# hila-chefer/Transformer-MM-Explainability

Hardware: AMD Instinct MI355X
Metric: relevancy maps/sec (fwd+bwd+rollout), CLIP ViT-B/32 (higher is better)
Workload: dtype f32

## Files before the change

### include/mmx_relevancy.h

```cpp
#ifndef MMX_RELEVANCY_H
#define MMX_RELEVANCY_H

#include <stddef.h>
#include <stdint.h>

#ifdef __cplusplus
extern "C" {
#endif

#define MMX_ABI_VERSION 2
#define MMX_MAX_LAYERS 48

enum mmx_dtype { MMX_F32 = 0, MMX_F16 = 1, MMX_BF16 = 2 };
#define MMX_ATTN_MMA_BF16 0x100
#define MMX_ATTN_IO_BF16 0x200

enum mmx_status {
    MMX_OK = 0,
    MMX_EINVAL = -22,
    MMX_ENOTSUP = -95,
    MMX_EWORKSPACE = -105,
    MMX_EHIP = -1000
};

#define MMX_MM_NORMALIZE 1u
#define MMX_MM_SELF_IN_RULE10 2u
#define MMX_MM_NAN_TO_ZERO 4u

#define MMX_SCALE_Q_FIRST 0
#define MMX_SCALE_SCORES 1

int mmx_abi_version(void);
const char* mmx_last_error(void);
int mmx_set_option(const char* key, int value);

int mmx_avg_heads(const void* attn_dev, const void* grad_dev, void* out_dev,
                  int B, int H, int Nq, int Nk, int dtype, void* stream);
int mmx_avg_heads_ex(const void* attn_dev, const void* grad_dev, void* out_dev,
                     int B, int H, int Nq, int Nk, int dtype, int64_t attn_batch_stride, void* stream);

size_t mmx_self_chain_workspace_bytes(int n_layers, int B, int H, int N, int M, int dtype);
int mmx_relevancy_self_chain(const void* const* attn_layers, const void* const* grad_layers, int n_layers,
                             int B, int H, int N, int dtype,
                             const void* R_init_dev, void* R_out_dev,
                             const void* Rsq_init_dev, void* Rsq_out_dev, int M,
                             void* workspace_dev, size_t workspace_bytes, void* stream);

int mmx_relevancy_self_chain_ex(const void* const* attn_layers, const void* const* grad_layers, int n_layers,
                                int B, int H, int N, int dtype, int64_t attn_batch_stride,
                                const void* R_init_dev, void* R_out_dev,
                                const void* Rsq_init_dev, void* Rsq_out_dev, int M,
                                void* workspace_dev, size_t workspace_bytes, void* stream);

#define MMX_CHAIN_CAUSAL 1u
int mmx_relevancy_self_chain_flags(const void* const* attn_layers, const void* const* grad_layers, int n_layers,
                                   int B, int H, int N, int dtype, int64_t attn_batch_stride,
                                   const void* R_init_dev, void* R_out_dev,
                                   const void* Rsq_init_dev, void* Rsq_out_dev, int M, unsigned flags,
                                   void* workspace_dev, size_t workspace_bytes, void* stream);

int mmx_relevancy_self_chain_half(const void* const* attn_layers, const void* const* grad_layers, int n_layers,
                                  int B, int H, int N, int dtype, int64_t attn_batch_stride, void* R_out_dev,
                                  void* workspace_dev, size_t workspace_bytes, void* stream);

int mmx_bmm_f32(const void* A_dev, const void* B_dev, const void* Cin_dev, void* C_dev,
                int batch, int M, int N, int K, int trans_a,
                int64_t stride_a, int64_t stride_b, int64_t stride_c,
                int nan_to_zero, void* stream);

int mmx_linear_f32(const void* x_dev, const void* wt_dev, const void* bias_dev, void* out_dev, int M, int N, int K, void* stream);

int mmx_rows_to_dense(const void* vals_dev, const void* rows_dev, void* out_dev, int B, int N, int E, void* stream);
int mmx_rows_add(void* dense_dev, const void* rows_dev, const void* vals_dev, int B, int N, int E, void* stream);

int mmx_live_rows(const void* eot_dev, int B, int N, void* rows_dev, void* count_dev, void* stream);
int mmx_gemm_rows_f32(const void* a_dev, const void* w_dev, void* c_dev, const void* rows_dev, const void* count_dev,
                      int cap_rows, int N, int K, void* stream);
int mmx_quick_gelu_bwd_rows(const void* x_dev, const void* dy_dev, void* dx_dev, const void* rows_dev, const void* count_dev,
                            int cap_rows, int row_elems, void* stream);
int mmx_layernorm_bwd_add_rows(const void* dy_dev, const void* x_dev, const void* mean_dev, const void* rstd_dev,
                               const void* gamma_dev, const void* d_res_dev, void* dx_dev, const void* rows_dev,
                               const void* count_dev, int cap_rows, int E, void* stream);
int mmx_gemm_rows_bias_f32(const void* a_dev, const void* wt_dev, const void* bias_dev, void* c_dev, void* act_dev,
                           const void* rows_dev, const void* count_dev, int cap_rows, int N, int K, void* stream);
int mmx_add_layernorm_fwd_rows(const void* x_dev, const void* y_dev, const void* gamma_dev, const void* beta_dev,
                               void* sum_dev, void* h_dev, void* mean_dev, void* rstd_dev, const void* rows_dev,
                               const void* count_dev, int cap_rows, int E, float eps, void* stream);
int mmx_text_live_rows_fwd_enabled(void);

int mmx_chain_matvec(const void* A_dev, const void* y_dev, const void* base_dev, void* out_dev, int B, int N, void* stream);
size_t mmx_chain_vecmat_workspace_bytes(int B, int N);
int mmx_chain_vecmat(const void* A_dev, const void* x_dev, const void* base_dev, void* out_dev, int B, int N,
                     void* workspace_dev, size_t workspace_bytes, void* stream);

size_t mmx_avg_heads_vecmat_workspace_bytes(int B, int N);
int mmx_avg_heads_vecmat(const void* attn_dev, const void* grad_dev, const void* x_dev, const void* base_dev, void* out_dev,
                         int B, int H, int N, int dtype, int64_t attn_batch_stride, void* workspace_dev,
                         size_t workspace_bytes, void* stream);

int mmx_handle_residual(const void* R_dev, void* out_dev, int batch, int N, void* diag_min_dev, void* stream);

size_t mmx_mm_rules_workspace_bytes(int Ns, int Nq);
int mmx_mm_attention_rules(const void* R_ss_dev, const void* R_qq_dev, const void* R_qs_dev,
                           const void* cam_sq_dev, void* R_sq_add_dev, void* R_ss_add_dev,
                           int Ns, int Nq, unsigned flags, void* diag_min_dev,
                           void* workspace_dev, size_t workspace_bytes, void* stream);

size_t mmx_lxmert_schedule_workspace_bytes(int n_lang, int n_vis, int n_x, int B, int T, int I);
int mmx_lxmert_schedule(const void* const* lang_attn, const void* const* lang_grad, int n_lang,
                           const void* const* vis_attn, const void* const* vis_grad, int n_vis,
                           const void* const* x_lang_cross_attn, const void* const* x_lang_cross_grad,
                           const void* const* x_img_cross_attn, const void* const* x_img_cross_grad,
                           const void* const* x_lang_self_attn, const void* const* x_lang_self_grad,
                           const void* const* x_img_self_attn, const void* const* x_img_self_grad, int n_x,
                           int B, int H, int T, int I, unsigned flags, const void* text_len_dev,
                           void* R_tt_dev, void* R_ti_dev, void* R_ii_dev, void* R_it_dev,
                           void* diag_min_dev, void* workspace_dev, size_t workspace_bytes, void* stream);

size_t mmx_rollout_workspace_bytes(int B, int N);
int mmx_rollout_chain(const void* const* layers, int n_layers, int B, int N, int normalize,
                      void* out_dev, void* workspace_dev, size_t workspace_bytes, void* stream);

int mmx_heatmap_bilinear_minmax(const void* in_dev, void* out_dev, int B, int g, int S, void* stream);
int mmx_otsu_masks(const void* cam_dev, void* masks_dev, void* thresholds_dev, int K, int n, void* stream);

int mmx_attn_capture_fwd(const void* q_dev, const void* k_dev, const void* v_dev,
                         int64_t q_sb, int64_t q_sh, int64_t q_sn,
                         int64_t k_sb, int64_t k_sh, int64_t k_sn,
                         int64_t v_sb, int64_t v_sh, int64_t v_sn,
                         const void* mask_dev, int64_t mask_sb, int64_t mask_sq,
                         void* probs_dev, void* o_dev, int64_t o_sb, int64_t o_sh, int64_t o_sn,
                         int B, int H, int Nq, int Nk, int D, float scale, int scale_mode, void* stream);

size_t mmx_attn_capture_bwd_workspace_bytes(int B, int H, int Nq);
int mmx_attn_capture_bwd(const void* q_dev, const void* k_dev, const void* v_dev,
                         int64_t q_sb, int64_t q_sh, int64_t q_sn,
                         int64_t k_sb, int64_t k_sh, int64_t k_sn,
                         int64_t v_sb, int64_t v_sh, int64_t v_sn,
                         const void* probs_dev, int64_t probs_sb,
                         const void* do_dev, int64_t o_sb, int64_t o_sh, int64_t o_sn,
                         void* dprobs_dev,
                         void* dq_dev, void* dk_dev, void* dv_dev,
                         int64_t dq_sb, int64_t dq_sh, int64_t dq_sn,
                         int64_t dk_sb, int64_t dk_sh, int64_t dk_sn,
                         int64_t dv_sb, int64_t dv_sh, int64_t dv_sn,
                         int B, int H, int Nq, int Nk, int D, float scale, int scale_mode,
                         int need_dqkv, void* workspace_dev, size_t workspace_bytes, void* stream);

int mmx_attn_capture_fwd_ex(const void* q_dev, const void* k_dev, const void* v_dev,
                            int64_t q_sb, int64_t q_sh, int64_t q_sn,
                            int64_t k_sb, int64_t k_sh, int64_t k_sn,
                            int64_t v_sb, int64_t v_sh, int64_t v_sn,
                            const void* mask_dev, int64_t mask_sb, int64_t mask_sq,
                            void* probs_dev, int slab_dtype,
                            void* o_dev, int64_t o_sb, int64_t o_sh, int64_t o_sn,
                            int B, int H, int Nq, int Nk, int D, float scale, int scale_mode, void* stream);
int mmx_attn_capture_bwd_ex(const void* q_dev, const void* k_dev, const void* v_dev,
                            int64_t q_sb, int64_t q_sh, int64_t q_sn,
                            int64_t k_sb, int64_t k_sh, int64_t k_sn,
                            int64_t v_sb, int64_t v_sh, int64_t v_sn,
                            const void* probs_dev, int64_t probs_sb, int slab_dtype,
                            const void* do_dev, int64_t o_sb, int64_t o_sh, int64_t o_sn,
                            const void* fwd_o_dev, int64_t fo_sb, int64_t fo_sh, int64_t fo_sn,
                            void* dprobs_dev,
                            void* dq_dev, void* dk_dev, void* dv_dev,
                            int64_t dq_sb, int64_t dq_sh, int64_t dq_sn,
                            int64_t dk_sb, int64_t dk_sh, int64_t dk_sn,
                            int64_t dv_sb, int64_t dv_sh, int64_t dv_sn,
                            int B, int H, int Nq, int Nk, int D, float scale, int scale_mode,
                            int need_dqkv, void* workspace_dev, size_t workspace_bytes, void* stream);

int mmx_attn_fwd(const void* q_dev, const void* k_dev, const void* v_dev,
                 int64_t q_sb, int64_t q_sh, int64_t q_sn,
                 int64_t k_sb, int64_t k_sh, int64_t k_sn,
                 int64_t v_sb, int64_t v_sh, int64_t v_sn,
                 const void* mask_dev, int64_t mask_sb, int64_t mask_sq,
                 void* o_dev, int64_t o_sb, int64_t o_sh, int64_t o_sn,
                 int B, int H, int Nq, int Nk, int D, float scale, int scale_mode, void* stream);

int mmx_patch_ranks(const void* scores_dev, void* ranks_dev, int B, int P, void* stream);
int mmx_perturb_patches(const void* images_dev, const void* ranks_dev, const void* counts_dev, const void* fill_dev,
                        void* out_dev, int B, int C, int R, int patch, int S, void* stream);

size_t mmx_attn_capture_bwd_rowrel_workspace_bytes(int B, int H, int Nq, int Nk);
int mmx_attn_capture_bwd_rowrel(const void* q_dev, const void* k_dev, const void* v_dev,
                                int64_t q_sb, int64_t q_sh, int64_t q_sn,
                                int64_t k_sb, int64_t k_sh, int64_t k_sn,
                                int64_t v_sb, int64_t v_sh, int64_t v_sn,
                                const void* probs_dev, int64_t probs_sb, int slab_dtype,
                                const void* do_dev, int64_t o_sb, int64_t o_sh, int64_t o_sn,
                                const void* fwd_o_dev, int64_t fo_sb, int64_t fo_sh, int64_t fo_sn,
                                void* dprobs_dev,
                                void* dq_dev, void* dk_dev, void* dv_dev,
                                int64_t dq_sb, int64_t dq_sh, int64_t dq_sn,
                                int64_t dk_sb, int64_t dk_sh, int64_t dk_sn,
                                int64_t dv_sb, int64_t dv_sh, int64_t dv_sn,
                                int B, int H, int Nq, int Nk, int D, float scale, int scale_mode,
                                int need_dqkv, const void* rel_in_dev, void* rel_out_dev,
                                void* workspace_dev, size_t workspace_bytes, void* stream);

size_t mmx_attn_capture_bwd_rowrel_f32_workspace_bytes(int B, int H, int Nq, int Nk);
int mmx_attn_capture_bwd_rowrel_f32(const void* q_dev, const void* k_dev, const void* v_dev,
                                    int64_t q_sb, int64_t q_sh, int64_t q_sn,
                                    int64_t k_sb, int64_t k_sh, int64_t k_sn,
                                    int64_t v_sb, int64_t v_sh, int64_t v_sn,
                                    const void* probs_dev, int64_t probs_sb, int slab_dtype,
                                    const void* do_dev, int64_t o_sb, int64_t o_sh, int64_t o_sn,
                                    const void* fwd_o_dev, int64_t fo_sb, int64_t fo_sh, int64_t fo_sn,
                                    void* dprobs_dev,
                                    void* dq_dev, void* dk_dev, void* dv_dev,
                                    int64_t dq_sb, int64_t dq_sh, int64_t dq_sn,
                                    int64_t dk_sb, int64_t dk_sh, int64_t dk_sn,
                                    int64_t dv_sb, int64_t dv_sh, int64_t dv_sn,
                                    int B, int H, int Nq, int Nk, int D, float scale, int scale_mode,
                                    int need_dqkv, const void* rel_in_dev, void* rel_out_dev,
                                    void* workspace_dev, size_t workspace_bytes, void* stream);

size_t mmx_attn_capture_bwd_rowrel_f32_grouped_workspace_bytes(int B, int H, int Nq, int Nk);
int mmx_attn_capture_bwd_rowrel_f32_grouped(const void* q_dev, const void* k_dev, const void* v_dev,
                                            int64_t q_sb, int64_t q_sh, int64_t q_sn,
                                            int64_t k_sb, int64_t k_sh, int64_t k_sn,
                                            int64_t v_sb, int64_t v_sh, int64_t v_sn,
                                            const void* probs_dev, int64_t probs_sb, int slab_dtype,
                                            const void* do_dev, int64_t o_sb, int64_t o_sh, int64_t o_sn,
                                            const void* fwd_o_dev, int64_t fo_sb, int64_t fo_sh, int64_t fo_sn,
                                            void* dprobs_dev,
                                            void* dq_dev, void* dk_dev, void* dv_dev,
                                            int64_t dq_sb, int64_t dq_sh, int64_t dq_sn,
                                            int64_t dk_sb, int64_t dk_sh, int64_t dk_sn,
                                            int64_t dv_sb, int64_t dv_sh, int64_t dv_sn,
                                            int B, int H, int Nq, int Nk, int D, float scale, int scale_mode,
                                            int need_dqkv, const void* rel_in_dev, void* rel_out_dev, int n_images,
                                            void* workspace_dev, size_t workspace_bytes, void* stream);

size_t mmx_detr_decoder_rows_workspace_bytes(int n_layers, int K, int Q, int Ni);
int mmx_detr_decoder_rows(const void* const* self_attn, const void* const* self_grad, const void* const* cross_attn,
                          const void* const* cross_grad, int n_layers, int K, int H, int Q, int Ni,
                          int64_t self_attn_bstride, int64_t cross_attn_bstride, const void* targets_dev,
                          void* s_out_dev, void* diag_min_dev, void* workspace_dev, size_t workspace_bytes, void* stream);

int mmx_attn_relprop(const void* q_dev, const void* k_dev, const void* v_dev, const void* o_dev, const void* cam_o_dev,
                     int64_t q_sb, int64_t q_sh, int64_t q_sn, int64_t k_sb, int64_t k_sh, int64_t k_sn,
                     int64_t v_sb, int64_t v_sh, int64_t v_sn, int64_t o_sb, int64_t o_sh, int64_t o_sn,
                     int64_t co_sb, int64_t co_sh, int64_t co_sn,
                     const void* probs_dev, void* cam_probs_dev, void* cam_q_dev, void* cam_k_dev, void* cam_v_dev,
                     int64_t cq_sb, int64_t cq_sh, int64_t cq_sn, int64_t ck_sb, int64_t ck_sh, int64_t ck_sn,
                     int64_t cv_sb, int64_t cv_sh, int64_t cv_sn,
                     int B, int H, int Nq, int Nk, int D, float scale, int scale_mode, void* stream);

#define MMX_LRP_VALUES 1
#define MMX_LRP_SCORES 2
int mmx_attn_relprop_phase(const void* q_dev, const void* k_dev, const void* v_dev, const void* o_dev, const void* cam_o_dev,
                           int64_t q_sb, int64_t q_sh, int64_t q_sn, int64_t k_sb, int64_t k_sh, int64_t k_sn,
                           int64_t v_sb, int64_t v_sh, int64_t v_sn, int64_t o_sb, int64_t o_sh, int64_t o_sn,
                           int64_t co_sb, int64_t co_sh, int64_t co_sn,
                           const void* probs_dev, void* cam_probs_dev, void* cam_q_dev, void* cam_k_dev, void* cam_v_dev,
                           int64_t cq_sb, int64_t cq_sh, int64_t cq_sn, int64_t ck_sb, int64_t ck_sh, int64_t ck_sn,
                           int64_t cv_sb, int64_t cv_sh, int64_t cv_sn,
                           int B, int H, int Nq, int Nk, int D, float scale, int scale_mode,
                           const void* cam_scores_dev, int phase, void* stream);

size_t mmx_lrp_workspace_bytes(void);
int mmx_lrp_split_signs(const void* x_dev, void* out_dev, int64_t rows, int n, void* stream);
int mmx_lrp_safe_divide(const void* a_dev, const void* b_dev, void* out_dev, int64_t n, void* stream);
int mmx_lrp_linear_combine(const void* xx_dev, const void* y_dev, void* out_dev, int64_t rows, int n,
                           const void* r_dev, int64_t r_numel, void* workspace_dev, void* stream);
int mmx_lrp_add_relprop(const void* r_dev, const void* a_dev, const void* b_dev, void* ra_dev, void* rb_dev,
                        int batch, int64_t per, void* workspace_dev, void* stream);
int mmx_lrp_clone_relprop(const void* const* r_list, int n_r, const void* x_dev, void* out_dev, int64_t n, void* stream);
int mmx_lrp_mha_rescale(const void* v_pre_dev, int64_t n_vpre, const void* v_post_dev, int64_t n_vpost, void* cam_k_dev,
                        int64_t n_k, void* cam_q_dev, int64_t n_q, const void* cam_o_dev, int64_t n_o,
                        void* workspace_dev, void* stream);


int mmx_quick_gelu_fwd(const void* x_dev, void* y_dev, int64_t n, void* stream);
int mmx_quick_gelu_fwd_bf16(const void* x_dev, void* y_dev, int64_t n, void* stream);
int mmx_quick_gelu_bwd(const void* x_dev, const void* dy_dev, void* dx_dev, int64_t n, void* stream);
int mmx_quick_gelu_bwd_bcast_bf16(const void* x_dev, const void* dy_dev, void* dx_dev, int64_t n, int64_t x_n, void* stream);
int mmx_layernorm_bwd_add_bf16(const void* dy_dev, const void* x_dev, const void* mean_dev, const void* rstd_dev,
                               const void* gamma_dev, const void* d_res_dev, void* dx_dev, void* dx_bf16_dev,
                               int64_t rows, int x_rows, int E, void* stream);
int mmx_quick_gelu_bwd_bcast(const void* x_dev, const void* dy_dev, void* dx_dev, int64_t n, int64_t x_n, void* stream);

int mmx_layernorm_bwd_add(const void* dy_dev, const void* x_dev, const void* mean_dev, const void* rstd_dev,
                          const void* gamma_dev, const void* d_res_dev, void* dx_dev, int64_t rows, int x_rows, int E,
                          void* stream);

int mmx_add_layernorm_fwd(const void* x_dev, const void* y_dev, const void* gamma_dev, const void* beta_dev,
                          void* sum_dev, void* h_dev, void* mean_dev, void* rstd_dev, int64_t rows, int E, float eps,
                          void* stream);
int mmx_add_layernorm_fwd_ex(const void* x_dev, const void* y_dev, const void* gamma_dev, const void* beta_dev,
                             void* sum_dev, void* h_dev, void* mean_dev, void* rstd_dev, int64_t rows, int E,
                             float eps, int h_dtype, void* stream);

int mmx_event_create(void** event_out);
int mmx_event_destroy(void* event);
int mmx_event_record(void* event, void* stream);
int mmx_event_elapsed_ms(void* start, void* stop, float* ms_out);

#ifdef __cplusplus
}
#endif
#endif
```

### transformer-mm-explainability_amd/_lib.py

```python
from __future__ import annotations

import ctypes as C
import os
import re

_HERE = os.path.dirname(os.path.abspath(__file__))
LIB_PATH = os.environ.get("MMX_LIB_PATH") or os.path.join(_HERE, "csrc", "libmmx_hip.so")
HEADER_PATH = os.path.join(os.path.dirname(_HERE), "include", "mmx_relevancy.h")

ABI_VERSION = 2
MMX_F32, MMX_F16, MMX_BF16 = 0, 1, 2
MMX_ENOTSUP = -95
MMX_ATTN_IO_BF16 = 0x200
MMX_ATTN_MMA_BF16 = 0x100
MM_NORMALIZE, MM_SELF_IN_RULE10, MM_NAN_TO_ZERO = 1, 2, 4
CHAIN_CAUSAL = 1
SCALE_Q_FIRST, SCALE_SCORES = 0, 1
LRP_VALUES, LRP_SCORES = 1, 2
MAX_LAYERS = 48

_vp, _i, _i64, _sz, _f, _u = C.c_void_p, C.c_int, C.c_int64, C.c_size_t, C.c_float, C.c_uint
_vpp = C.POINTER(C.c_void_p)

_PROTOTYPES = {
    "mmx_abi_version": (_i, []),
    "mmx_last_error": (C.c_char_p, []),
    "mmx_set_option": (_i, [C.c_char_p, _i]),
    "mmx_avg_heads": (_i, [_vp, _vp, _vp, _i, _i, _i, _i, _i, _vp]),
    "mmx_avg_heads_ex": (_i, [_vp, _vp, _vp, _i, _i, _i, _i, _i, _i64, _vp]),
    "mmx_self_chain_workspace_bytes": (_sz, [_i, _i, _i, _i, _i, _i]),
    "mmx_relevancy_self_chain": (_i, [_vpp, _vpp, _i, _i, _i, _i, _i, _vp, _vp, _vp, _vp, _i, _vp, _sz, _vp]),
    "mmx_relevancy_self_chain_ex": (_i, [_vpp, _vpp, _i, _i, _i, _i, _i, _i64, _vp, _vp, _vp, _vp, _i, _vp, _sz, _vp]),
    "mmx_relevancy_self_chain_flags": (_i, [_vpp, _vpp, _i, _i, _i, _i, _i, _i64, _vp, _vp, _vp, _vp, _i, _u, _vp, _sz, _vp]),
    "mmx_relevancy_self_chain_half": (_i, [_vpp, _vpp, _i, _i, _i, _i, _i, _i64, _vp, _vp, _sz, _vp]),
    "mmx_bmm_f32": (_i, [_vp, _vp, _vp, _vp, _i, _i, _i, _i, _i, _i64, _i64, _i64, _i, _vp]),
    "mmx_handle_residual": (_i, [_vp, _vp, _i, _i, _vp, _vp]),
    "mmx_mm_rules_workspace_bytes": (_sz, [_i, _i]),
    "mmx_mm_attention_rules": (_i, [_vp, _vp, _vp, _vp, _vp, _vp, _i, _i, _u, _vp, _vp, _sz, _vp]),
    "mmx_lxmert_schedule_workspace_bytes": (_sz, [_i, _i, _i, _i, _i, _i]),
    "mmx_lxmert_schedule": (_i, [_vpp, _vpp, _i, _vpp, _vpp, _i] + [_vpp] * 8 + [_i, _i, _i, _i, _i, _u, _vp,
                                    _vp, _vp, _vp, _vp, _vp, _vp, _sz, _vp]),
    "mmx_lrp_workspace_bytes": (_sz, []),
    "mmx_lrp_split_signs": (_i, [_vp, _vp, _i64, _i, _vp]),
    "mmx_lrp_safe_divide": (_i, [_vp, _vp, _vp, _i64, _vp]),
    "mmx_lrp_linear_combine": (_i, [_vp, _vp, _vp, _i64, _i, _vp, _i64, _vp, _vp]),
    "mmx_lrp_add_relprop": (_i, [_vp, _vp, _vp, _vp, _vp, _i, _i64, _vp, _vp]),
    "mmx_lrp_clone_relprop": (_i, [_vpp, _i, _vp, _vp, _i64, _vp]),
    "mmx_lrp_mha_rescale": (_i, [_vp, _i64, _vp, _i64, _vp, _i64, _vp, _i64, _vp, _i64, _vp, _vp]),
    "mmx_heatmap_bilinear_minmax": (_i, [_vp, _vp, _i, _i, _i, _vp]),
    "mmx_otsu_masks": (_i, [_vp, _vp, _vp, _i, _i, _vp]),
    "mmx_rollout_workspace_bytes": (_sz, [_i, _i]),
    "mmx_rollout_chain": (_i, [_vpp, _i, _i, _i, _i, _vp, _vp, _sz, _vp]),
    "mmx_attn_capture_fwd": (_i, [_vp, _vp, _vp] + [_i64] * 9 + [_vp, _i64, _i64, _vp, _vp, _i64, _i64, _i64,
                                  _i, _i, _i, _i, _i, _f, _i, _vp]),
    "mmx_attn_capture_fwd_ex": (_i, [_vp, _vp, _vp] + [_i64] * 9 + [_vp, _i64, _i64, _vp, _i, _vp, _i64, _i64, _i64,
                                     _i, _i, _i, _i, _i, _f, _i, _vp]),
    "mmx_attn_fwd": (_i, [_vp, _vp, _vp] + [_i64] * 9 + [_vp, _i64, _i64, _vp, _i64, _i64, _i64, _i, _i, _i, _i, _i, _f, _i, _vp]),
    "mmx_patch_ranks": (_i, [_vp, _vp, _i, _i, _vp]),
    "mmx_perturb_patches": (_i, [_vp, _vp, _vp, _vp, _vp, _i, _i, _i, _i, _i, _vp]),
    "mmx_attn_capture_bwd_ex": (_i, [_vp, _vp, _vp] + [_i64] * 9 + [_vp, _i64, _i, _vp, _i64, _i64, _i64, _vp, _i64, _i64, _i64,
                                     _vp, _vp, _vp, _vp]
                                + [_i64] * 9 + [_i, _i, _i, _i, _i, _f, _i, _i, _vp, _sz, _vp]),
    "mmx_attn_capture_bwd_rowrel": (_i, [_vp, _vp, _vp] + [_i64] * 9 + [_vp, _i64, _i, _vp, _i64, _i64, _i64, _vp, _i64, _i64,
                                         _i64, _vp, _vp, _vp, _vp]
                                    + [_i64] * 9 + [_i, _i, _i, _i, _i, _f, _i, _i, _vp, _vp, _vp, _sz, _vp]),
    "mmx_attn_capture_bwd_rowrel_workspace_bytes": (_sz, [_i, _i, _i, _i]),
    "mmx_attn_capture_bwd_rowrel_f32": (_i, [_vp, _vp, _vp] + [_i64] * 9 + [_vp, _i64, _i, _vp, _i64, _i64, _i64, _vp, _i64,
                                             _i64, _i64, _vp, _vp, _vp, _vp]
                                        + [_i64] * 9 + [_i, _i, _i, _i, _i, _f, _i, _i, _vp, _vp, _vp, _sz, _vp]),
    "mmx_attn_capture_bwd_rowrel_f32_workspace_bytes": (_sz, [_i, _i, _i, _i]),
    "mmx_attn_capture_bwd_rowrel_f32_grouped": (_i, [_vp, _vp, _vp] + [_i64] * 9 + [_vp, _i64, _i, _vp, _i64, _i64, _i64, _vp,
                                                     _i64, _i64, _i64, _vp, _vp, _vp, _vp]
                                                + [_i64] * 9 + [_i, _i, _i, _i, _i, _f, _i, _i, _vp, _vp, _i, _vp, _sz, _vp]),
    "mmx_attn_capture_bwd_rowrel_f32_grouped_workspace_bytes": (_sz, [_i, _i, _i, _i]),
    "mmx_attn_capture_bwd_workspace_bytes": (_sz, [_i, _i, _i]),
    "mmx_attn_capture_bwd": (_i, [_vp, _vp, _vp] + [_i64] * 9 + [_vp, _i64, _vp, _i64, _i64, _i64, _vp, _vp, _vp, _vp]
                             + [_i64] * 9 + [_i, _i, _i, _i, _i, _f, _i, _i, _vp, _sz, _vp]),
    "mmx_attn_relprop": (_i, [_vp] * 5 + [_i64] * 15 + [_vp] * 5 + [_i64] * 9 + [_i, _i, _i, _i, _i, _f, _i, _vp]),
    "mmx_attn_relprop_phase": (_i, [_vp] * 5 + [_i64] * 15 + [_vp] * 5 + [_i64] * 9 + [_i, _i, _i, _i, _i, _f, _i, _vp, _i, _vp]),
    "mmx_detr_decoder_rows_workspace_bytes": (_sz, [_i, _i, _i, _i]),
    "mmx_detr_decoder_rows": (_i, [_vpp] * 4 + [_i] * 5 + [_i64, _i64, _vp, _vp, _vp, _vp, _sz, _vp]),
    "mmx_linear_f32": (_i, [_vp, _vp, _vp, _vp, _i, _i, _i, _vp]),
    "mmx_rows_to_dense": (_i, [_vp, _vp, _vp, _i, _i, _i, _vp]),
    "mmx_rows_add": (_i, [_vp, _vp, _vp, _i, _i, _i, _vp]),
    "mmx_live_rows": (_i, [_vp, _i, _i, _vp, _vp, _vp]),
    "mmx_gemm_rows_f32": (_i, [_vp, _vp, _vp, _vp, _vp, _i, _i, _i, _vp]),
    "mmx_quick_gelu_bwd_rows": (_i, [_vp, _vp, _vp, _vp, _vp, _i, _i, _vp]),
    "mmx_layernorm_bwd_add_rows": (_i, [_vp, _vp, _vp, _vp, _vp, _vp, _vp, _vp, _vp, _i, _i, _vp]),
    "mmx_gemm_rows_bias_f32": (_i, [_vp, _vp, _vp, _vp, _vp, _vp, _vp, _i, _i, _i, _vp]),
    "mmx_add_layernorm_fwd_rows": (_i, [_vp, _vp, _vp, _vp, _vp, _vp, _vp, _vp, _vp, _vp, _i, _i, _f, _vp]),
    "mmx_text_live_rows_fwd_enabled": (_i, []),
    "mmx_chain_matvec": (_i, [_vp, _vp, _vp, _vp, _i, _i, _vp]),
    "mmx_chain_vecmat_workspace_bytes": (_sz, [_i, _i]),
    "mmx_chain_vecmat": (_i, [_vp, _vp, _vp, _vp, _i, _i, _vp, _sz, _vp]),
    "mmx_avg_heads_vecmat_workspace_bytes": (_sz, [_i, _i]),
    "mmx_avg_heads_vecmat": (_i, [_vp, _vp, _vp, _vp, _vp, _i, _i, _i, _i, _i64, _vp, _sz, _vp]),
    "mmx_quick_gelu_fwd": (_i, [_vp, _vp, _i64, _vp]),
    "mmx_quick_gelu_fwd_bf16": (_i, [_vp, _vp, _i64, _vp]),
    "mmx_quick_gelu_bwd": (_i, [_vp, _vp, _vp, _i64, _vp]),
    "mmx_quick_gelu_bwd_bcast": (_i, [_vp, _vp, _vp, _i64, _i64, _vp]),
    "mmx_quick_gelu_bwd_bcast_bf16": (_i, [_vp, _vp, _vp, _i64, _i64, _vp]),
    "mmx_layernorm_bwd_add_bf16": (_i, [_vp, _vp, _vp, _vp, _vp, _vp, _vp, _vp, _i64, _i, _i, _vp]),
    "mmx_layernorm_bwd_add": (_i, [_vp, _vp, _vp, _vp, _vp, _vp, _vp, _i64, _i, _i, _vp]),
    "mmx_add_layernorm_fwd": (_i, [_vp, _vp, _vp, _vp, _vp, _vp, _vp, _vp, _i64, _i, _f, _vp]),
    "mmx_add_layernorm_fwd_ex": (_i, [_vp, _vp, _vp, _vp, _vp, _vp, _vp, _vp, _i64, _i, _f, _i, _vp]),
    "mmx_event_create": (_i, [_vpp]),
    "mmx_event_destroy": (_i, [_vp]),
    "mmx_event_record": (_i, [_vp, _vp]),
    "mmx_event_elapsed_ms": (_i, [_vp, _vp, C.POINTER(C.c_float)]),
}


class MMXError(RuntimeError):
    pass


_lib = None


def header_symbols():
    with open(HEADER_PATH) as f:
        text = re.sub(r"/\*.*?\*/", "", f.read(), flags=re.S)
    return sorted(set(re.findall(r"\b(mmx_[a-z0-9_]+)\s*\(", text)))


def lib():
    global _lib
    if _lib is None:
        if not os.path.exists(LIB_PATH):
            raise MMXError(
                "libmmx_hip.so is not built (%s). Run `python -c 'import __graft_entry__ as g; g.build()'` "
                "or `make -C transformer-mm-explainability_amd/csrc`. There is no CPU fallback." % LIB_PATH)
        handle = C.CDLL(LIB_PATH)
        for name, (res, args) in _PROTOTYPES.items():
            fn = getattr(handle, name)
            fn.restype, fn.argtypes = res, args
        if handle.mmx_abi_version() != ABI_VERSION:
            raise MMXError("libmmx_hip.so ABI version %d != %d (stale build? `make -C transformer-mm-explainability_amd/csrc`)"
                           % (handle.mmx_abi_version(), ABI_VERSION))
        _lib = handle
    return _lib


def check(rc, what):
    if rc != 0:
        msg = lib().mmx_last_error().decode("utf-8", "replace")
        raise MMXError("%s failed (rc=%d): %s" % (what, rc, msg))


def ptr_table(ptrs):
    arr = (C.c_void_p * len(ptrs))(*ptrs)
    return C.cast(arr, _vpp), arr
```

### transformer-mm-explainability_amd/clip_model.py

```python
from __future__ import annotations

from collections import OrderedDict

import numpy as np
import torch
import torch.nn as nn
import torch.nn.functional as F

from . import _lib, ops
from .capture import CaptureBuffers, attention_capture_packed


class QuickGELU(nn.Module):
    def forward(self, x):
        if x.is_cuda and x.dtype == torch.float32:
            return ops.quick_gelu(x)
        return x * torch.sigmoid(1.702 * x)


class _OutProj(nn.Linear):
    """``attn.out_proj`` (name kept for state-dict compatibility)."""


class CapturedSelfAttention(nn.Module):

    def __init__(self, embed_dim, num_heads):
        super().__init__()
        if embed_dim % num_heads:
            raise ValueError("embed_dim must be divisible by num_heads")
        self.embed_dim, self.num_heads, self.head_dim = embed_dim, num_heads, embed_dim // num_heads
        self.in_proj_weight = nn.Parameter(torch.empty(3 * embed_dim, embed_dim))
        self.in_proj_bias = nn.Parameter(torch.zeros(3 * embed_dim))
        self.out_proj = _OutProj(embed_dim, embed_dim)
        nn.init.xavier_uniform_(self.in_proj_weight)
        nn.init.zeros_(self.out_proj.bias)

    def forward(self, x, probs_slab, grads_slab, mask=None, need_dqkv=True, grad_hook=None):
        B, N, E = x.shape
        qkv = F.linear(x, self.in_proj_weight, self.in_proj_bias).view(B, N, 3, self.num_heads, self.head_dim)
        o = attention_capture_packed(qkv, probs_slab, grads_slab, self.head_dim ** -0.5, mask=mask,
                                     scale_mode=_lib.SCALE_Q_FIRST, need_dqkv=need_dqkv, grad_hook=grad_hook)
        return self.out_proj(o.view(B, N, E))


class ResidualAttentionBlock(nn.Module):

    def __init__(self, d_model, n_head, attn_mask=None):
        super().__init__()
        self.attn = CapturedSelfAttention(d_model, n_head)
        self.ln_1 = nn.LayerNorm(d_model)
        self.mlp = nn.Sequential(OrderedDict([
            ("c_fc", nn.Linear(d_model, d_model * 4)),
            ("gelu", QuickGELU()),
            ("c_proj", nn.Linear(d_model * 4, d_model)),
        ]))
        self.ln_2 = nn.LayerNorm(d_model)
        self.attn_mask = attn_mask
        self.attn_probs = None
        self.attn_grad = None

    def _slab_view(self, name):
        owner = self.__dict__.get("_probs_owner")
        if owner is not None:
            owner[0].complete_attn_probs()
        return self.__dict__.get(name)

    @property
    def attn_probs(self):
        return self._slab_view("_attn_probs")

    @attn_probs.setter
    def attn_probs(self, value):
        self.__dict__["_attn_probs"] = value

    @property
    def attn_grad(self):
        return self._slab_view("_attn_grad")

    @attn_grad.setter
    def attn_grad(self, value):
        self.__dict__["_attn_grad"] = value

    def set_attn_probs(self, attn_probs):
        self.attn_probs = attn_probs

    def set_attn_grad(self, attn_grad):
        self.attn_grad = attn_grad

    def forward(self, x, buffers, layer, need_dqkv=True):
        if self.attn_mask is not None and (self.attn_mask.device != x.device):
            self.attn_mask = self.attn_mask.to(device=x.device, dtype=torch.float32)
        probs, grads = buffers.probs[layer], buffers.grads[layer]
        self.attn_probs = buffers.layer_probs(layer)
        self.attn_grad = buffers.layer_grads(layer)
        mask = self.attn_mask
        if mask is not None and mask.shape[-1] != x.shape[1]:
            mask = mask[: x.shape[1], : x.shape[1]].contiguous()
        x = x + self.attn(self.ln_1(x), probs, grads, mask=mask, need_dqkv=need_dqkv)
        x = x + self.mlp(self.ln_2(x))
        return x


class Transformer(nn.Module):
    def __init__(self, width, layers, heads, attn_mask=None):
        super().__init__()
        self.width, self.layers, self.heads = width, layers, heads
        self.resblocks = nn.Sequential(*[ResidualAttentionBlock(width, heads, attn_mask) for _ in range(layers)])
        self.buffers = None
        self.capture_dtype = torch.float32
        self.backward_gemm_dtype = torch.float32
        self.forward_gemm_dtype = torch.float32
        self.attention_mma_bf16 = False
        self._long_sequence_slabs_follow_body = attn_mask is None
        self._probs_pending = None

    def set_body_dtype(self, dtype):
        if dtype not in (torch.float32, torch.bfloat16, torch.float16):
            raise ValueError("body dtype must be torch.float32, torch.bfloat16 or torch.float16")
        half = dtype == torch.bfloat16
        self.backward_gemm_dtype = self.forward_gemm_dtype = dtype
        self.attention_mma_bf16 = half
        self.half_chain = dtype == torch.float16
        if self._long_sequence_slabs_follow_body:
            self.capture_dtype = dtype
            self.buffers = None

    def _linear(self, x, lin_weight, lin_bias):
        return ops.linear(x, lin_weight, lin_bias, getattr(self, "forward_gemm_dtype", torch.float32))

    def _gemm(self, x, weight):
        return ops.backward_gemm(x, weight, getattr(self, "backward_gemm_dtype", torch.float32))

    def _ensure_buffers(self, batch, n_tokens, device, shared_probs=False, grads=True):
        if self.buffers is None or not self.buffers.matches(self.layers, batch, self.heads, n_tokens, n_tokens, device,
                                                            shared_probs, self.capture_dtype, grads):
            self.buffers = CaptureBuffers(self.layers, batch, self.heads, n_tokens, n_tokens, device=device,
                                          shared_probs=shared_probs, dtype=self.capture_dtype, grads=grads)
        return self.buffers

    def _mask_for(self, blk, n_tokens, device):
        mask = blk.attn_mask
        if mask is None:
            return None
        if mask.device != device:
            blk.attn_mask = mask = mask.to(device=device, dtype=torch.float32)
        if mask.shape[-1] != n_tokens:
            mask = mask[:n_tokens, :n_tokens].contiguous()
        return mask

    def is_causal(self):
        masks = [getattr(blk, "attn_mask", None) for blk in self.resblocks]
        if not masks or any(m is None for m in masks):
            return False
        key = tuple(id(m) for m in masks)
        cached = self.__dict__.get("_causal_mask_check")
        if cached is None or cached[0] != key:
            ok = True
            for m in {id(m): m for m in masks}.values():
                n = m.shape[-1]
                upper = torch.ones(n, n, dtype=torch.bool, device=m.device).triu_(1)
                ok = ok and m.dim() == 2 and m.shape[0] == n and bool(torch.isneginf(m[upper]).all())
            self.__dict__["_causal_mask_check"] = cached = (key, ok)
        return cached[1]

    def _row_gemm_weights_ok(self):
        for blk in self.resblocks:
            if not ops.gemm_rows_eligible(blk.mlp.c_proj.weight, blk.mlp.c_fc.weight, blk.attn.out_proj.weight, blk.attn.in_proj_weight):
                return False
        return True

    def live_rows_for_forward(self, x, out_rows):
        if out_rows is None or x.dim() != 3 or x.dtype != torch.float32 or x.shape[-1] % 4 or not x.is_cuda:
            return None
        for what in ("forward_gemm_dtype", "backward_gemm_dtype", "capture_dtype"):
            if getattr(self, what, torch.float32) != torch.float32:
                return None
        if self.layers < 1 or not ops.live_rows_forward_enabled() or not self.is_causal() or not self._row_gemm_weights_ok():
            return None
        if x.shape[1] < self.resblocks[0].attn_mask.shape[-1]:
            return None
        for blk in self.resblocks:
            for bias in (blk.attn.in_proj_bias, blk.attn.out_proj.bias, blk.mlp.c_fc.bias, blk.mlp.c_proj.bias):
                if bias is None or bias.dtype != torch.float32:
                    return None
        return ops.live_rows(out_rows, x.shape[1])

    @torch.no_grad()
    def complete_attn_probs(self):
        pending = self.__dict__.get("_probs_pending")
        if pending is None:
            return
        if torch.cuda.is_current_stream_capturing():
            raise _lib.MMXError("attn_probs / attn_grad: the slabs of a row-list forward cannot be completed inside a stream capture "
                                "(read them outside it, or set option text_live_rows_fwd to 0)")
        self._probs_pending = None
        keep, self.buffers = self.buffers, pending["buffers"]
        try:
            _, tape = self.forward_tape(pending["x"], first_grad_layer=pending["first_grad_layer"],
                                        grads=pending["buffers"].grads is not None, out_rows=pending["out_rows"])
            if pending["dy_row_values"] is not None:
                self.backward_tape(tape, None, pending["backward_first_grad_layer"], dy_rows=pending["out_rows"],
                                   dy_row_values=pending["dy_row_values"])
        finally:
            self.buffers = keep

    def _live_rows_route(self, tape, B, N, E, first_grad_layer, dy_rows, dy_row_values, rel_row, grouped):
        top = self.layers - 1
        if dy_rows is None or dy_row_values is None or rel_row is not None or grouped or top <= first_grad_layer:
            return None
        if getattr(self, "backward_gemm_dtype", torch.float32) != torch.float32 or dy_row_values.dtype != torch.float32:
            return None
        if tape[top][0].shape[0] != B or E % 4 or not self.is_causal() or not self._row_gemm_weights_ok():
            return None
        return ops.live_rows(dy_rows, N)

    @torch.no_grad()
    def forward_tape(self, x, batch=None, first_grad_layer=0, grads=True, out_rows=None, live=None):
        if not x.is_cuda:
            raise _lib.MMXError("the CLIP body runs its attention on the HIP capture op: move the model and "
                                "inputs to the MI355X (there is no CPU attention path)")
        Bx, N, E = x.shape
        batch = Bx if batch is None else batch
        shared = Bx == 1 and batch > 1
        if not shared and Bx != batch:
            raise ValueError("forward_tape: %d inputs for %d upstream gradients (only a single input can be shared)" % (Bx, batch))
        buffers = self._ensure_buffers(batch, N, x.device, shared_probs=shared, grads=grads)
        blocks = list(self.resblocks)
        mask = self._mask_for(blocks[0], N, x.device) if blocks else None
        tape = []
        self._probs_pending = None
        if live is not None:
            if out_rows is None or shared or live.cap != Bx * N:
                raise ValueError("forward_tape: the row-list forward needs out_rows, one input per gradient and a list over %d rows"
                                 % (Bx * N))
            self._probs_pending = {"x": x, "buffers": buffers, "live": live, "out_rows": out_rows, "first_grad_layer": first_grad_layer,
                                   "dy_row_values": None, "backward_first_grad_layer": None}
            for blk in blocks:
                blk.__dict__["_probs_owner"] = (self,)

        def ln(res, y, norm):
            if live is not None:
                return ops.add_layernorm_rows(res, y, norm.weight, norm.bias, norm.eps, live)
            return ops.add_layernorm(res, y, norm.weight, norm.bias, norm.eps, h_dtype=hd)
        mma = bool(getattr(self, "attention_mma_bf16", False)) and N > 128
        first = blocks[0].ln_1
        hd = torch.bfloat16 if getattr(self, "forward_gemm_dtype", torch.float32) == torch.bfloat16 else torch.float32
        _, h1, mean1, rstd1 = ln(x, None, first)
        for l, blk in enumerate(blocks):
            at = blk.attn
            if live is not None:
                qkv = ops.linear_rows(h1, at.in_proj_weight, at.in_proj_bias, live,
                                      out=torch.zeros(Bx, N, 3 * E, dtype=torch.float32, device=x.device))
            else:
                qkv = self._linear(h1, at.in_proj_weight, at.in_proj_bias)
            qkv = qkv.view(Bx, N, 3, at.num_heads, at.head_dim)
            o = ops.attn_capture_fwd(qkv[:, :, 0], qkv[:, :, 1], qkv[:, :, 2], buffers.probs[l], at.head_dim ** -0.5,
                                     _lib.SCALE_Q_FIRST, mask, layout="bnhd", mma_bf16=mma)
            if out_rows is not None and l + 1 == len(blocks):
                ar = torch.arange(Bx, device=x.device)
                x1, h2, mean2, rstd2 = ops.add_layernorm(
                    x[ar, out_rows], self._linear(o.view(Bx, N, E)[ar, out_rows], at.out_proj.weight, at.out_proj.bias),
                    blk.ln_2.weight, blk.ln_2.bias, blk.ln_2.eps, h_dtype=hd)
                m = self._linear(h2, blk.mlp.c_fc.weight, blk.mlp.c_fc.bias)
                mlp_out = self._linear(ops.quick_gelu_fwd(m, hd), blk.mlp.c_proj.weight, blk.mlp.c_proj.bias)
                tape.append((x, mean1, rstd1, qkv, x1, mean2, rstd2, m, o, out_rows) if l >= first_grad_layer else None)
                blk.attn_probs, blk.attn_grad = buffers.layer_probs(l), buffers.layer_grads(l)
                return x1 + mlp_out, tape
            if live is not None:
                x1, h2, mean2, rstd2 = ln(x, ops.linear_rows(o.view(Bx, N, E), at.out_proj.weight, at.out_proj.bias, live), blk.ln_2)
                m, act = ops.linear_rows(h2, blk.mlp.c_fc.weight, blk.mlp.c_fc.bias, live, gelu=True)
                mlp_out = ops.linear_rows(act, blk.mlp.c_proj.weight, blk.mlp.c_proj.bias, live)
            else:
                x1, h2, mean2, rstd2 = ln(x, self._linear(o.view(Bx, N, E), at.out_proj.weight, at.out_proj.bias), blk.ln_2)
                m = self._linear(h2, blk.mlp.c_fc.weight, blk.mlp.c_fc.bias)
                mlp_out = self._linear(ops.quick_gelu_fwd(m, hd), blk.mlp.c_proj.weight, blk.mlp.c_proj.bias)
            tape.append((x, mean1, rstd1, qkv, x1, mean2, rstd2, m, o) if l >= first_grad_layer else None)
            blk.attn_probs, blk.attn_grad = buffers.layer_probs(l), buffers.layer_grads(l)
            if l + 1 < len(blocks):
                x, h1, mean1, rstd1 = ln(x1, mlp_out, blocks[l + 1].ln_1)
            else:
                x = x1 + mlp_out
        return x, tape

    @torch.no_grad()
    def forward_nocapture(self, x, out_rows=None):
        for what in ("forward_gemm_dtype", "capture_dtype"):
            dt = getattr(self, what, torch.float32)
            if dt != torch.float32:
                raise _lib.MMXError("forward_nocapture: fp32 bodies only (the no-capture attention is exact fp32); this tower's "
                                    "%s is %s" % (what, str(dt).replace("torch.", "")))
        if x.dtype != torch.float32:
            raise _lib.MMXError("forward_nocapture: fp32 bodies only; the input is %s" % str(x.dtype).replace("torch.", ""))
        if not x.is_cuda:
            raise _lib.MMXError("the CLIP body runs its attention on the HIP kernels: move the model and inputs to the GPU")
        B, N, E = x.shape
        blocks = list(self.resblocks)
        mask = self._mask_for(blocks[0], N, x.device) if blocks else None
        first = blocks[0].ln_1
        _, h1, _, _ = ops.add_layernorm(x, None, first.weight, first.bias, first.eps)
        for l, blk in enumerate(blocks):
            at = blk.attn
            top = out_rows is not None and l + 1 == len(blocks)
            one = top and isinstance(out_rows, int)
            qkv = self._linear(h1, at.in_proj_weight, at.in_proj_bias).view(B, N, 3, at.num_heads, at.head_dim)
            q = qkv[:, out_rows:out_rows + 1, 0] if one else qkv[:, :, 0]
            m_l = mask[out_rows:out_rows + 1] if (one and mask is not None) else mask
            o = ops.attn_fwd(q, qkv[:, :, 1], qkv[:, :, 2], at.head_dim ** -0.5, _lib.SCALE_Q_FIRST, m_l, layout="bnhd")
            if one:
                xr, orows = x[:, out_rows], o.view(B, E)
            elif top:
                ar = torch.arange(B, device=x.device)
                xr, orows = x[ar, out_rows], o.view(B, N, E)[ar, out_rows]
            else:
                xr, orows = x, o.view(B, N, E)
            x1, h2, _, _ = ops.add_layernorm(xr, self._linear(orows, at.out_proj.weight, at.out_proj.bias), blk.ln_2.weight,
                                             blk.ln_2.bias, blk.ln_2.eps)
            mlp_out = self._linear(ops.quick_gelu_fwd(self._linear(h2, blk.mlp.c_fc.weight, blk.mlp.c_fc.bias)),
                                   blk.mlp.c_proj.weight, blk.mlp.c_proj.bias)
            if l + 1 < len(blocks):
                nxt = blocks[l + 1].ln_1
                x, h1, _, _ = ops.add_layernorm(x1, mlp_out, nxt.weight, nxt.bias, nxt.eps)
            else:
                x = x1 + mlp_out
        return x

    def forward_shared(self, x, batch):
        if x.shape[0] != 1:
            raise ValueError("forward_shared takes the single shared sample")
        return self.forward_tape(x, batch)

    @torch.no_grad()
    def backward_tape(self, tape, dy, first_grad_layer=0, dy_rows=None, rel_row=None, dy_row_values=None, targets_per_image=1,
                      live=None):
        if dy is None:
            if dy_rows is None or dy_row_values is None:
                raise ValueError("backward_tape: dy=None needs dy_rows and dy_row_values")
            if self.layers - 1 < first_grad_layer:
                return rel_row
            B, N, E = dy_row_values.shape[0], tape[-1][0].shape[1], dy_row_values.shape[1]
        else:
            B, N, E = dy.shape
        buffers = self.buffers
        top = self.layers - 1
        dx = dy
        top_rows = None
        mma = bool(getattr(self, "attention_mma_bf16", False)) and N > 128
        grouped = int(targets_per_image) > 1
        stream16 = getattr(self, "backward_gemm_dtype", torch.float32) == torch.bfloat16
        head = self.resblocks[0].attn
        att16 = stream16 and (mma or (self.capture_dtype == torch.float32 and
                                      ops.head_kernel_shape(N, N, head.head_dim) and head.head_dim % 8 == 0))
        if grouped and (rel_row is None or stream16 or mma or B % int(targets_per_image)):
            raise ValueError("backward_tape: targets_per_image=%d needs an fp32 body in the row mode and a multiple of it "
                             "upstream gradients (got %d)" % (int(targets_per_image), B))
        dx_h = None
        if live is None:
            live = self._live_rows_route(tape, B, N, E, first_grad_layer, dy_rows, dy_row_values, rel_row, grouped)
        elif dy_rows is None or dy_row_values is None or rel_row is not None or grouped or live.cap != B * N:
            raise ValueError("backward_tape: the tape of a row-list forward needs the row-list backward (dy_rows and dy_row_values, "
                             "no rel_row, one target per sample)")
        else:
            pending = self.__dict__.get("_probs_pending")
            if pending is not None and pending["live"] is live:
                pending["dy_row_values"], pending["backward_first_grad_layer"] = dy_row_values, first_grad_layer
        d_o_dense = None
        for l in range(top, first_grad_layer - 1, -1):
            blk = self.resblocks[l]
            at = blk.attn
            x, mean1, rstd1, qkv, x1, mean2, rstd2, m, o_fwd = tape[l][:9]
            shared = x.shape[0] != B and not grouped
            if grouped and x.shape[0] * int(targets_per_image) != B:
                raise ValueError("backward_tape: %d upstream gradients for %d samples x %d targets"
                                 % (B, x.shape[0], int(targets_per_image)))
            if len(tape[l]) > 9 and (l != top or dy_rows is None):
                raise ValueError("backward_tape: the forward kept only the output rows of the top block (out_rows): "
                                 "pass the same rows as dy_rows")
            if l == top and dy_rows is not None:
                g = dy_row_values if dy_row_values is not None else dy[torch.arange(B, device=dy_rows.device), dy_rows]
                d_x1_r, d_o = self._top_block_rows(blk, tape[l], g, dy_rows, shared, N, x.shape[0] if grouped else None)
                d_x1, top_rows = None, (dy_rows, d_x1_r)
                d_o_dense = d_o
                if att16:
                    d_o = d_o.to(torch.bfloat16)
            elif live is not None:
                d_a = ops.gemm_rows(dx, blk.mlp.c_proj.weight, live)
                d_m = ops.quick_gelu_bwd_rows(m, d_a, live)
                d_h2 = ops.gemm_rows(d_m, blk.mlp.c_fc.weight, live)
                d_x1 = ops.layernorm_bwd_add_rows(d_h2, x1, mean2, rstd2, blk.ln_2.weight, dx, live)
                d_o = ops.gemm_rows(d_x1, at.out_proj.weight, live, out=d_o_dense)
            elif stream16:
                if dx_h is None:
                    dx_h = dx.to(torch.bfloat16)
                d_a = ops.backward_gemm_bf16(dx_h, blk.mlp.c_proj.weight)
                d_m = ops.quick_gelu_bwd(m, d_a)
                d_h2 = ops.backward_gemm_bf16(d_m, blk.mlp.c_fc.weight)
                d_x1, d_x1_h = ops.layernorm_bwd_add_bf16(d_h2, x1, mean2, rstd2, blk.ln_2.weight, dx)
                d_o = ops.backward_gemm_bf16(d_x1_h, at.out_proj.weight)
            else:
                d_a = self._gemm(dx, blk.mlp.c_proj.weight)
                d_m = ops.quick_gelu_bwd(m, d_a)
                d_h2 = self._gemm(d_m, blk.mlp.c_fc.weight)
                d_x1 = ops.layernorm_bwd_add(d_h2, x1, mean2, rstd2, blk.ln_2.weight, dx)
                d_o = self._gemm(d_x1, at.out_proj.weight)
            if stream16 and not att16 and d_o.dtype != torch.float32:
                d_o = d_o.float()
            d_o = d_o.view(B, N, at.num_heads, at.head_dim)
            need = l > first_grad_layer
            dqkv = torch.empty(B, N, 3, at.num_heads, at.head_dim, dtype=d_o.dtype, device=d_o.device) if need else None
            out = (dqkv[:, :, 0], dqkv[:, :, 1], dqkv[:, :, 2]) if need else None
            res = ops.attn_capture_bwd(qkv[:, :, 0], qkv[:, :, 1], qkv[:, :, 2], buffers.probs[l], d_o,
                                       buffers.grads[l] if buffers.grads is not None else None,
                                       at.head_dim ** -0.5, _lib.SCALE_Q_FIRST, need_dqkv=need, layout="bnhd", out=out,
                                       batch=B if shared else None, o=o_fwd, mma_bf16=mma, rel_row=rel_row,
                                       images=x.shape[0] if grouped else None)
            if rel_row is not None:
                rel_row = res[3]
            if not need:
                break
            if stream16:
                dq_in = dqkv.view(B, N, 3 * E)
                d_h1 = ops.backward_gemm_bf16(dq_in if att16 else dq_in.to(torch.bfloat16), at.in_proj_weight)
                dx, dx_h = ops.layernorm_bwd_add_bf16(d_h1, x, mean1, rstd1, blk.ln_1.weight, d_x1)
            elif live is not None:
                d_h1 = ops.gemm_rows(dqkv.view(B, N, 3 * E), at.in_proj_weight, live)
                dx = ops.layernorm_bwd_add_rows(d_h1, x, mean1, rstd1, blk.ln_1.weight, d_x1, live)
            else:
                d_h1 = self._gemm(dqkv.view(B, N, 3 * E), at.in_proj_weight)
                dx = ops.layernorm_bwd_add(d_h1, x, mean1, rstd1, blk.ln_1.weight, d_x1)
            if l == top and top_rows is not None:
                ops.rows_add_(dx, *top_rows)
                if stream16:
                    dx_h = dx.to(torch.bfloat16)
        return rel_row

    def _top_block_rows(self, blk, entry, g, rows, shared, N, images=None):
        x, mean1, rstd1, qkv, x1, mean2, rstd2, m, o_fwd = entry[:9]
        B = g.shape[0]
        ar = torch.arange(B, device=g.device)
        src = torch.zeros_like(rows) if shared else ar
        if images is not None:
            src = ar % images
        if len(entry) > 9:
            m_r, x1_r, mean2_r, rstd2_r = m[src], x1[src], mean2.reshape(-1)[src], rstd2.reshape(-1)[src]
        else:
            flat = src * N + rows
            m_r, x1_r, mean2_r, rstd2_r = m[src, rows], x1[src, rows], mean2.reshape(-1)[flat], rstd2.reshape(-1)[flat]
        d_a = self._gemm(g, blk.mlp.c_proj.weight)
        d_m = ops.quick_gelu_bwd(m_r, d_a) if d_a.dtype == torch.float32 and m_r.numel() % 4 == 0 else \
            d_a * (torch.sigmoid(1.702 * m_r) * (1 + 1.702 * m_r * (1 - torch.sigmoid(1.702 * m_r))))
        d_h2 = self._gemm(d_m, blk.mlp.c_fc.weight)
        d_x1_r = ops.layernorm_bwd_add(d_h2, x1_r, mean2_r, rstd2_r, blk.ln_2.weight, g)
        return d_x1_r, ops.rows_to_dense(self._gemm(d_x1_r, blk.attn.out_proj.weight), rows, N)

    def backward_shared(self, tape, dy, first_grad_layer=0):
        return self.backward_tape(tape, dy, first_grad_layer)

    def forward(self, x, capture_only=False, first_grad_layer=0):
        if not x.is_cuda:
            raise _lib.MMXError("the CLIP body runs its attention on the HIP capture op: move the model and "
                                "inputs to the MI355X (there is no CPU attention path)")
        buffers = self._ensure_buffers(x.shape[0], x.shape[1], x.device)
        self._probs_pending = None
        if not capture_only:
            for l, blk in enumerate(self.resblocks):
                x = blk(x, buffers, l)
            return x
        with torch.no_grad():
            for l in range(first_grad_layer):
                x = self.resblocks[l](x, buffers, l)
        x = x.detach().requires_grad_(True)
        for l in range(first_grad_layer, self.layers):
            x = self.resblocks[l](x, buffers, l, need_dqkv=(l != first_grad_layer))
        return x


class VisualTransformer(nn.Module):

    def __init__(self, input_resolution, patch_size, width, layers, heads, output_dim):
        super().__init__()
        self.input_resolution, self.output_dim = input_resolution, output_dim
        self.conv1 = nn.Conv2d(3, width, kernel_size=patch_size, stride=patch_size, bias=False)
        scale = width ** -0.5
        self.class_embedding = nn.Parameter(scale * torch.randn(width))
        self.positional_embedding = nn.Parameter(scale * torch.randn((input_resolution // patch_size) ** 2 + 1, width))
        self.ln_pre = nn.LayerNorm(width)
        self.transformer = Transformer(width, layers, heads)
        self.ln_post = nn.LayerNorm(width)
        self.proj = nn.Parameter(scale * torch.randn(width, output_dim))

    def _patchify(self, x):
        B, C, Hh, Ww = x.shape
        p = self.conv1.kernel_size[0]
        gh, gw = Hh // p, Ww // p
        patches = x.reshape(B, C, gh, p, gw, p).permute(0, 2, 4, 1, 3, 5).reshape(B, gh * gw, C * p * p)
        return F.linear(patches, self.conv1.weight.reshape(self.conv1.out_channels, -1))

    def _embed(self, x):
        x = self._patchify(x)
        cls = self.class_embedding.to(x.dtype).expand(x.shape[0], 1, -1)
        return self.ln_pre(torch.cat([cls, x], dim=1) + self.positional_embedding.to(x.dtype))

    def forward(self, x, capture_only=False, first_grad_layer=0):
        x = self.transformer(self._embed(x), capture_only=capture_only, first_grad_layer=first_grad_layer)
        x = self.ln_post(x[:, 0, :])
        return x @ self.proj if self.proj is not None else x

    def row_relevancy_ok(self):
        t = self.transformer
        n_tokens = self.positional_embedding.shape[0]
        return bool(getattr(t, "attention_mma_bf16", False)) and n_tokens > 128

    @torch.no_grad()
    def forward_tape(self, image, batch=None, first_grad_layer=0, grads=True):
        x = self._embed(image)
        y, tape = self.transformer.forward_tape(x, batch, first_grad_layer, grads=grads,
                                                out_rows=torch.zeros(x.shape[0], dtype=torch.long, device=x.device))
        cls = y
        _, f, mean, rstd = ops.add_layernorm(cls, None, self.ln_post.weight, self.ln_post.bias, self.ln_post.eps)
        return f @ self.proj, (tape, x.shape, cls, mean, rstd)

    def forward_shared(self, image, batch):
        return self.forward_tape(image, batch)

    @torch.no_grad()
    def encode_nocapture(self, images=None, tokens=None):
        if (images is None) == (tokens is None):
            raise ValueError("encode_nocapture takes images or tokens (exactly one of them)")
        if self.conv1.weight.dtype != torch.float32:
            raise _lib.MMXError("encode_nocapture: fp32 bodies only; the parameters are %s"
                                % str(self.conv1.weight.dtype).replace("torch.", ""))
        x = self._embed(images) if tokens is None else tokens
        cls = self.transformer.forward_nocapture(x, out_rows=0)
        _, f, _, _ = ops.add_layernorm(cls, None, self.ln_post.weight, self.ln_post.bias, self.ln_post.eps)
        return f @ self.proj

    @torch.no_grad()
    def backward_tape(self, state, d_features, first_grad_layer=0, cls_row=False, targets_per_image=1):
        tape, y_shape, cls, mean, rstd = state
        B = d_features.shape[0]
        if int(targets_per_image) > 1 and not cls_row:
            raise ValueError("backward_tape: targets_per_image needs cls_row=True (the grouped mode is a row mode)")
        d_f = torch.matmul(d_features, self.proj.t())
        d_cls = ops.layernorm_bwd_add(d_f, cls, mean, rstd, self.ln_post.weight)
        rel_row = None
        if cls_row:
            rel_row = torch.zeros(B, y_shape[1], dtype=torch.float32, device=d_f.device)
            rel_row[:, 0] = 1.0
        return self.transformer.backward_tape(tape, None, first_grad_layer,
                                              dy_rows=torch.zeros(B, dtype=torch.long, device=d_f.device), rel_row=rel_row,
                                              dy_row_values=d_cls, targets_per_image=targets_per_image)

    def backward_shared(self, state, d_features, first_grad_layer=0):
        return self.backward_tape(state, d_features, first_grad_layer)


class CLIP(nn.Module):

    def __init__(self, embed_dim, image_resolution, vision_layers, vision_width, vision_patch_size,
                 context_length, vocab_size, transformer_width, transformer_heads, transformer_layers):
        super().__init__()
        if isinstance(vision_layers, (tuple, list)):
            raise NotImplementedError("ModifiedResNet towers have no attention stack; use a ViT config")
        self.context_length = context_length
        self.visual = VisualTransformer(image_resolution, vision_patch_size, vision_width, vision_layers,
                                        vision_width // 64, embed_dim)
        self.transformer = Transformer(transformer_width, transformer_layers, transformer_heads,
                                       attn_mask=self.build_attention_mask())
        self.vocab_size = vocab_size
        self.token_embedding = nn.Embedding(vocab_size, transformer_width)
        self.positional_embedding = nn.Parameter(torch.empty(context_length, transformer_width))
        self.ln_final = nn.LayerNorm(transformer_width)
        self.text_projection = nn.Parameter(torch.empty(transformer_width, embed_dim))
        self.logit_scale = nn.Parameter(torch.ones([]) * np.log(1 / 0.07))
        self.capture_only = False
        self.first_grad_layers = (0, 0)
        self.initialize_parameters()

    def initialize_parameters(self):
        nn.init.normal_(self.token_embedding.weight, std=0.02)
        nn.init.normal_(self.positional_embedding, std=0.01)
        w, n = self.transformer.width, self.transformer.layers
        proj_std, attn_std, fc_std = (w ** -0.5) * ((2 * n) ** -0.5), w ** -0.5, (2 * w) ** -0.5
        for blk in self.transformer.resblocks:
            nn.init.normal_(blk.attn.in_proj_weight, std=attn_std)
            nn.init.normal_(blk.attn.out_proj.weight, std=proj_std)
            nn.init.normal_(blk.mlp.c_fc.weight, std=fc_std)
            nn.init.normal_(blk.mlp.c_proj.weight, std=proj_std)
        nn.init.normal_(self.text_projection, std=w ** -0.5)

    def set_body_dtype(self, dtype):
        self.visual.transformer.set_body_dtype(dtype)
        self.transformer.set_body_dtype(dtype)

    def build_attention_mask(self):
        return torch.full((self.context_length, self.context_length), float("-inf")).triu_(1)

    @property
    def dtype(self):
        return self.visual.conv1.weight.dtype

    def encode_image(self, image):
        return self.visual(image.type(self.dtype), capture_only=self.capture_only,
                           first_grad_layer=self.first_grad_layers[0])

    def encode_text(self, text, n_tokens=None):
        if n_tokens is not None and n_tokens < text.shape[1]:
            text = text[:, :n_tokens]
        n = text.shape[1]
        x = self.token_embedding(text).type(self.dtype) + self.positional_embedding[:n].type(self.dtype)
        x = self.transformer(x, capture_only=self.capture_only, first_grad_layer=self.first_grad_layers[1])
        x = self.ln_final(x)
        return x[torch.arange(x.shape[0], device=x.device), text.argmax(dim=-1)] @ self.text_projection

    @torch.no_grad()
    def encode_text_tape(self, text, n_tokens=None, first_grad_layer=0):
        if n_tokens is not None and n_tokens < text.shape[1]:
            text = text[:, :n_tokens]
        n = text.shape[1]
        x = self.token_embedding(text).type(self.dtype) + self.positional_embedding[:n].type(self.dtype)
        eot = text.argmax(dim=-1)
        live = self.transformer.live_rows_for_forward(x, eot)
        rows, tape = self.transformer.forward_tape(x, first_grad_layer=first_grad_layer, out_rows=eot, live=live)
        _, f, mean, rstd = ops.add_layernorm(rows, None, self.ln_final.weight, self.ln_final.bias, self.ln_final.eps)
        return f @ self.text_projection, (tape, x.shape, rows, mean, rstd, eot, live)

    @torch.no_grad()
    def encode_text_nocapture(self, text):
        x = self.token_embedding(text).type(self.dtype) + self.positional_embedding[:text.shape[1]].type(self.dtype)
        rows = self.transformer.forward_nocapture(x, out_rows=text.argmax(dim=-1))
        _, f, _, _ = ops.add_layernorm(rows, None, self.ln_final.weight, self.ln_final.bias, self.ln_final.eps)
        return f @ self.text_projection

    @torch.no_grad()
    def backward_text_tape(self, state, d_features, first_grad_layer=0):
        tape, y_shape, rows, mean, rstd, eot, live = state
        d_f = torch.matmul(d_features, self.text_projection.t())
        d_rows = ops.layernorm_bwd_add(d_f, rows, mean, rstd, self.ln_final.weight)
        self.transformer.backward_tape(tape, None, first_grad_layer, dy_rows=eot, dy_row_values=d_rows,
                                       live=live)

    def forward(self, image, text):
        return self.logits(self.encode_image(image), self.encode_text(text))

    def logits(self, image_features, text_features):
        image_features = image_features / image_features.norm(dim=-1, keepdim=True)
        text_features = text_features / text_features.norm(dim=-1, keepdim=True)
        logit_scale = self.logit_scale.exp()
        logits_per_image = logit_scale * image_features @ text_features.t()
        logits_per_text = logit_scale * text_features @ image_features.t()
        return logits_per_image, logits_per_text


def build_model(state_dict):
    if "visual.proj" not in state_dict:
        raise NotImplementedError("only ViT CLIP checkpoints carry an attention stack to explain")
    vision_width = state_dict["visual.conv1.weight"].shape[0]
    vision_layers = len([k for k in state_dict if k.startswith("visual.") and k.endswith(".attn.in_proj_weight")])
    vision_patch_size = state_dict["visual.conv1.weight"].shape[-1]
    grid_size = round((state_dict["visual.positional_embedding"].shape[0] - 1) ** 0.5)
    embed_dim = state_dict["text_projection"].shape[1]
    context_length = state_dict["positional_embedding"].shape[0]
    vocab_size = state_dict["token_embedding.weight"].shape[0]
    transformer_width = state_dict["ln_final.weight"].shape[0]
    transformer_layers = len({k.split(".")[2] for k in state_dict if k.startswith("transformer.resblocks")})
    model = CLIP(embed_dim, vision_patch_size * grid_size, vision_layers, vision_width, vision_patch_size,
                 context_length, vocab_size, transformer_width, transformer_width // 64, transformer_layers)
    sd = {k: v.float() for k, v in state_dict.items() if k not in ("input_resolution", "context_length", "vocab_size")}
    model.load_state_dict(sd)
    return model.eval()


CONFIGS = {
    "ViT-B/32": (512, 224, 12, 768, 32, 77, 49408, 512, 8, 12),
    "ViT-B/16": (512, 224, 12, 768, 16, 77, 49408, 512, 8, 12),
    "ViT-L/14@336": (768, 336, 24, 1024, 14, 77, 49408, 768, 12, 12),
}


def random_init(name="ViT-B/32", seed=0):
    torch.manual_seed(seed)
    return CLIP(*CONFIGS[name]).float().eval()
```

### transformer-mm-explainability_amd/csrc/elementwise_kernels.hip

```cpp
#include "mmx_common.h"

namespace mmx {

typedef unsigned u32x2 __attribute__((ext_vector_type(2)));
__device__ __forceinline__ unsigned bf_pack(float a, float b) {
    typedef __bf16 bf2 __attribute__((ext_vector_type(2)));
    bf2 r;
    r[0] = static_cast<__bf16>(a);
    r[1] = static_cast<__bf16>(b);
    return __builtin_bit_cast(unsigned, r);
}

__global__ __launch_bounds__(256) void quick_gelu_fwd_kernel(const f32x4* __restrict__ x, f32x4* __restrict__ y, int64_t n4,
                                                             const float* xt, float* yt, int tail) {
    for (int64_t i = static_cast<int64_t>(blockIdx.x) * 256 + threadIdx.x; i < n4; i += static_cast<int64_t>(gridDim.x) * 256) {
        const f32x4 v = x[i];
        f32x4 o;
#pragma unroll
        for (int e = 0; e < 4; ++e) o[e] = quick_gelu_f(v[e]);
        y[i] = o;
    }
    if (blockIdx.x == 0 && threadIdx.x < tail) yt[threadIdx.x] = quick_gelu_f(xt[threadIdx.x]);
}

__global__ __launch_bounds__(256) void quick_gelu_fwd_bf16_kernel(const f32x4* __restrict__ x, u32x2* __restrict__ y, int64_t n4) {
    for (int64_t i = static_cast<int64_t>(blockIdx.x) * 256 + threadIdx.x; i < n4; i += static_cast<int64_t>(gridDim.x) * 256) {
        const f32x4 v = x[i];
        f32x4 o;
#pragma unroll
        for (int e = 0; e < 4; ++e) o[e] = quick_gelu_f(v[e]);
        y[i] = u32x2{bf_pack(o[0], o[1]), bf_pack(o[2], o[3])};
    }
}

template <bool ROWS>
__global__ __launch_bounds__(256) void quick_gelu_bwd_kernel(const f32x4* __restrict__ x, const f32x4* __restrict__ dy,
                                                             f32x4* __restrict__ dx, int64_t n4, int64_t x_n4, const float* xt,
                                                             const float* dyt, float* dxt, int tail, const int* __restrict__ rows,
                                                             const int* __restrict__ count, int row4) {
    const int64_t cap = ROWS ? n4 / row4 : 0;
    const int64_t total = ROWS ? (*count < cap ? *count : cap) * row4 : n4;
    for (int64_t j = static_cast<int64_t>(blockIdx.x) * 256 + threadIdx.x; j < total; j += static_cast<int64_t>(gridDim.x) * 256) {
        int64_t i = j;
        if constexpr (ROWS) {
            const int64_t r = rows[j / row4];
            if (r < 0 || r >= cap) continue;
            i = r * row4 + j % row4;
        }
        const f32x4 v = x[x_n4 == n4 ? i : i % x_n4];
        const f32x4 g = dy[i];
        f32x4 o;
#pragma unroll
        for (int e = 0; e < 4; ++e) {
            const float s = sigmoid_f(1.702f * v[e]);
            o[e] = g[e] * (s + 1.702f * v[e] * s * (1.f - s));
        }
        dx[i] = o;
    }
    if (!ROWS && blockIdx.x == 0 && threadIdx.x < tail) {
        const float v = xt[threadIdx.x], s = sigmoid_f(1.702f * v);
        dxt[threadIdx.x] = dyt[threadIdx.x] * (s + 1.702f * v * s * (1.f - s));
    }
}

}

using namespace mmx;

static int gelu_grid(int64_t n4) {
    const int64_t blocks = (n4 + 255) / 256;
    return static_cast<int>(blocks < 1 ? 1 : (blocks > 4096 ? 4096 : blocks));
}

extern "C" int mmx_quick_gelu_fwd(const void* x_dev, void* y_dev, int64_t n, void* stream) {
    MMX_CHECK_ARG(x_dev && y_dev && n > 0, "mmx_quick_gelu_fwd: bad argument");
    MMX_CHECK_ARG(((reinterpret_cast<uintptr_t>(x_dev) | reinterpret_cast<uintptr_t>(y_dev)) & 15u) == 0,
                  "mmx_quick_gelu_fwd: pointers must be 16-byte aligned");
    const int64_t n4 = n / 4;
    const float* x = static_cast<const float*>(x_dev);
    float* y = static_cast<float*>(y_dev);
    quick_gelu_fwd_kernel<<<gelu_grid(n4), 256, 0, static_cast<hipStream_t>(stream)>>>(
        reinterpret_cast<const f32x4*>(x), reinterpret_cast<f32x4*>(y), n4, x + n4 * 4, y + n4 * 4, static_cast<int>(n - n4 * 4));
    MMX_LAUNCH_CHECK("quick_gelu_fwd_kernel");
    return MMX_OK;
}

extern "C" int mmx_quick_gelu_bwd_bcast(const void* x_dev, const void* dy_dev, void* dx_dev, int64_t n, int64_t x_n,
                                        void* stream) {
    MMX_CHECK_ARG(x_dev && dy_dev && dx_dev && n > 0 && x_n > 0, "mmx_quick_gelu_bwd_bcast: bad argument");
    MMX_CHECK_ARG(n % x_n == 0 && x_n % 4 == 0, "mmx_quick_gelu_bwd_bcast: n=%ld must be a multiple of x_n=%ld, x_n %% 4 == 0",
                  static_cast<long>(n), static_cast<long>(x_n));
    MMX_CHECK_ARG(((reinterpret_cast<uintptr_t>(x_dev) | reinterpret_cast<uintptr_t>(dy_dev) |
                    reinterpret_cast<uintptr_t>(dx_dev)) & 15u) == 0, "mmx_quick_gelu_bwd_bcast: pointers must be 16-byte aligned");
    const int64_t n4 = n / 4;
    quick_gelu_bwd_kernel<false><<<gelu_grid(n4), 256, 0, static_cast<hipStream_t>(stream)>>>(
        static_cast<const f32x4*>(x_dev), static_cast<const f32x4*>(dy_dev), static_cast<f32x4*>(dx_dev), n4, x_n / 4, nullptr,
        nullptr, nullptr, 0, nullptr, nullptr, 1);
    MMX_LAUNCH_CHECK("quick_gelu_bwd_kernel");
    return MMX_OK;
}

extern "C" int mmx_quick_gelu_bwd(const void* x_dev, const void* dy_dev, void* dx_dev, int64_t n, void* stream) {
    MMX_CHECK_ARG(x_dev && dy_dev && dx_dev && n > 0, "mmx_quick_gelu_bwd: bad argument");
    MMX_CHECK_ARG(((reinterpret_cast<uintptr_t>(x_dev) | reinterpret_cast<uintptr_t>(dy_dev) |
                    reinterpret_cast<uintptr_t>(dx_dev)) & 15u) == 0, "mmx_quick_gelu_bwd: pointers must be 16-byte aligned");
    const int64_t n4 = n / 4;
    const float* x = static_cast<const float*>(x_dev);
    const float* dy = static_cast<const float*>(dy_dev);
    float* dx = static_cast<float*>(dx_dev);
    quick_gelu_bwd_kernel<false><<<gelu_grid(n4), 256, 0, static_cast<hipStream_t>(stream)>>>(
        reinterpret_cast<const f32x4*>(x), reinterpret_cast<const f32x4*>(dy), reinterpret_cast<f32x4*>(dx), n4, n4, x + n4 * 4,
        dy + n4 * 4, dx + n4 * 4, static_cast<int>(n - n4 * 4), nullptr, nullptr, 1);
    MMX_LAUNCH_CHECK("quick_gelu_bwd_kernel");
    return MMX_OK;
}

extern "C" int mmx_quick_gelu_bwd_rows(const void* x_dev, const void* dy_dev, void* dx_dev, const void* rows_dev, const void* count_dev,
                                       int cap_rows, int row_elems, void* stream) {
    MMX_CHECK_ARG(x_dev && dy_dev && dx_dev && rows_dev && count_dev, "mmx_quick_gelu_bwd_rows: null pointer");
    MMX_CHECK_ARG(cap_rows > 0 && row_elems > 0 && row_elems % 4 == 0, "mmx_quick_gelu_bwd_rows: cap_rows=%d row_elems=%d (%% 4 must be 0)",
                  cap_rows, row_elems);
    MMX_CHECK_ARG(((reinterpret_cast<uintptr_t>(x_dev) | reinterpret_cast<uintptr_t>(dy_dev) |
                    reinterpret_cast<uintptr_t>(dx_dev)) & 15u) == 0, "mmx_quick_gelu_bwd_rows: pointers must be 16-byte aligned");
    const int64_t n4 = static_cast<int64_t>(cap_rows) * (row_elems / 4);
    quick_gelu_bwd_kernel<true><<<gelu_grid(n4), 256, 0, static_cast<hipStream_t>(stream)>>>(
        static_cast<const f32x4*>(x_dev), static_cast<const f32x4*>(dy_dev), static_cast<f32x4*>(dx_dev), n4, n4, nullptr, nullptr,
        nullptr, 0, static_cast<const int*>(rows_dev), static_cast<const int*>(count_dev), row_elems / 4);
    MMX_LAUNCH_CHECK("quick_gelu_bwd_kernel<rows>");
    return MMX_OK;
}

namespace mmx {

template <bool ROWS>
__global__ __launch_bounds__(256) void layernorm_bwd_add_kernel(const float* __restrict__ dy, const float* __restrict__ x,
                                                                const float* __restrict__ mean, const float* __restrict__ rstd,
                                                                const float* __restrict__ gamma, const float* d_res,
                                                                float* __restrict__ dx, int64_t rows, int x_rows, int E,
                                                                const int* __restrict__ list, const int* __restrict__ count) {
    int64_t r = static_cast<int64_t>(blockIdx.x) * 4 + (threadIdx.x >> 6);
    if (r >= rows) return;
    if constexpr (ROWS) {
        if (r >= *count) return;
        r = list[r];
        if (r < 0 || r >= rows) return;
    }
    const int lane = threadIdx.x & 63;
    const int m = static_cast<int>(r % x_rows);
    const f32x4* dyr = reinterpret_cast<const f32x4*>(dy + r * E);
    const f32x4* xr = reinterpret_cast<const f32x4*>(x + static_cast<int64_t>(m) * E);
    const f32x4* gm = reinterpret_cast<const f32x4*>(gamma);
    const float mu = mean[m], rs = rstd[m];
    const int n4 = E >> 2;
    float a = 0.f, b = 0.f;
    for (int i = lane; i < n4; i += 64) {
        const f32x4 g = dyr[i] * gm[i];
        const f32x4 xh = (xr[i] - mu) * rs;
        a += g[0] + g[1] + g[2] + g[3];
        b += g[0] * xh[0] + g[1] * xh[1] + g[2] * xh[2] + g[3] * xh[3];
    }
#pragma unroll
    for (int off = 32; off > 0; off >>= 1) { a += __shfl_xor(a, off); b += __shfl_xor(b, off); }
    a /= static_cast<float>(E);
    b /= static_cast<float>(E);
    const f32x4* dr = d_res ? reinterpret_cast<const f32x4*>(d_res + r * E) : nullptr;
    f32x4* out = reinterpret_cast<f32x4*>(dx + r * E);
    for (int i = lane; i < n4; i += 64) {
        const f32x4 g = dyr[i] * gm[i];
        const f32x4 xh = (xr[i] - mu) * rs;
        f32x4 o = (g - a - xh * b) * rs;
        if (dr) o = o + dr[i];
        out[i] = o;
    }
}

}

extern "C" int mmx_layernorm_bwd_add(const void* dy_dev, const void* x_dev, const void* mean_dev, const void* rstd_dev,
                                     const void* gamma_dev, const void* d_res_dev, void* dx_dev, int64_t rows, int x_rows,
                                     int E, void* stream) {
    MMX_CHECK_ARG(dy_dev && x_dev && mean_dev && rstd_dev && gamma_dev && dx_dev, "mmx_layernorm_bwd_add: null pointer");
    MMX_CHECK_ARG(rows > 0 && x_rows > 0 && E > 0 && E % 4 == 0, "mmx_layernorm_bwd_add: rows=%ld x_rows=%d E=%d (E %% 4 must be 0)",
                  static_cast<long>(rows), x_rows, E);
    mmx::layernorm_bwd_add_kernel<false><<<static_cast<unsigned>((rows + 3) / 4), 256, 0, static_cast<hipStream_t>(stream)>>>(
        static_cast<const float*>(dy_dev), static_cast<const float*>(x_dev), static_cast<const float*>(mean_dev),
        static_cast<const float*>(rstd_dev), static_cast<const float*>(gamma_dev), static_cast<const float*>(d_res_dev),
        static_cast<float*>(dx_dev), rows, x_rows, E, nullptr, nullptr);
    MMX_LAUNCH_CHECK("layernorm_bwd_add_kernel");
    return MMX_OK;
}

extern "C" int mmx_layernorm_bwd_add_rows(const void* dy_dev, const void* x_dev, const void* mean_dev, const void* rstd_dev,
                                          const void* gamma_dev, const void* d_res_dev, void* dx_dev, const void* rows_dev,
                                          const void* count_dev, int cap_rows, int E, void* stream) {
    MMX_CHECK_ARG(dy_dev && x_dev && mean_dev && rstd_dev && gamma_dev && dx_dev && rows_dev && count_dev,
                  "mmx_layernorm_bwd_add_rows: null pointer");
    MMX_CHECK_ARG(cap_rows > 0 && E > 0 && E % 4 == 0, "mmx_layernorm_bwd_add_rows: cap_rows=%d E=%d (E %% 4 must be 0)", cap_rows, E);
    mmx::layernorm_bwd_add_kernel<true><<<static_cast<unsigned>((cap_rows + 3) / 4), 256, 0, static_cast<hipStream_t>(stream)>>>(
        static_cast<const float*>(dy_dev), static_cast<const float*>(x_dev), static_cast<const float*>(mean_dev),
        static_cast<const float*>(rstd_dev), static_cast<const float*>(gamma_dev), static_cast<const float*>(d_res_dev),
        static_cast<float*>(dx_dev), cap_rows, cap_rows, E, static_cast<const int*>(rows_dev), static_cast<const int*>(count_dev));
    MMX_LAUNCH_CHECK("layernorm_bwd_add_kernel<rows>");
    return MMX_OK;
}

namespace mmx {

template <int NV, bool ROWS>
__global__ __launch_bounds__(256) void add_layernorm_fwd_kernel(const float* __restrict__ x, const float* __restrict__ y,
                                                                const float* __restrict__ gamma, const float* __restrict__ beta,
                                                                float* __restrict__ sum_out, float* __restrict__ h_out,
                                                                float* __restrict__ mean_out, float* __restrict__ rstd_out,
                                                                int64_t rows, int E, float eps, unsigned short* __restrict__ h_bf16,
                                                                const int* __restrict__ list, const int* __restrict__ count) {
    int64_t r = static_cast<int64_t>(blockIdx.x) * 4 + (threadIdx.x >> 6);
    if (r >= rows) return;
    if constexpr (ROWS) {
        if (r >= *count) return;
        r = list[r];
        if (r < 0 || r >= rows) return;
    }
    const int lane = threadIdx.x & 63, n4 = E >> 2;
    const f32x4* xr = reinterpret_cast<const f32x4*>(x + r * E);
    const f32x4* yr = y ? reinterpret_cast<const f32x4*>(y + r * E) : nullptr;
    f32x4 v[NV];
    float s = 0.f;
#pragma unroll
    for (int j = 0; j < NV; ++j) {
        const int i = lane + 64 * j;
        v[j] = f32x4{0.f, 0.f, 0.f, 0.f};
        if (i < n4) {
            v[j] = xr[i];
            if (yr) v[j] = v[j] + yr[i];
            s += v[j][0] + v[j][1] + v[j][2] + v[j][3];
        }
    }
#pragma unroll
    for (int off = 32; off > 0; off >>= 1) s += __shfl_xor(s, off);
    const float mu = s / static_cast<float>(E);
    float q = 0.f;
#pragma unroll
    for (int j = 0; j < NV; ++j)
        if (lane + 64 * j < n4) {
            const f32x4 d = v[j] - mu;
            q += d[0] * d[0] + d[1] * d[1] + d[2] * d[2] + d[3] * d[3];
        }
#pragma unroll
    for (int off = 32; off > 0; off >>= 1) q += __shfl_xor(q, off);
    const float rs = rsqrtf(q / static_cast<float>(E) + eps);
    if (lane == 0) {
        mean_out[r] = mu;
        rstd_out[r] = rs;
    }
    const f32x4* gm = reinterpret_cast<const f32x4*>(gamma);
    const f32x4* bt = reinterpret_cast<const f32x4*>(beta);
    f32x4* so = (sum_out && yr) ? reinterpret_cast<f32x4*>(sum_out + r * E) : nullptr;
    f32x4* ho = h_bf16 ? nullptr : reinterpret_cast<f32x4*>(h_out + r * E);
    u32x2* hb = h_bf16 ? reinterpret_cast<u32x2*>(h_bf16 + r * E) : nullptr;
#pragma unroll
    for (int j = 0; j < NV; ++j) {
        const int i = lane + 64 * j;
        if (i < n4) {
            if (so) so[i] = v[j];
            const f32x4 h = (v[j] - mu) * rs * gm[i] + bt[i];
            if (hb) hb[i] = u32x2{bf_pack(h[0], h[1]), bf_pack(h[2], h[3])};
            else ho[i] = h;
        }
    }
}

}

extern "C" int mmx_add_layernorm_fwd_ex(const void* x_dev, const void* y_dev, const void* gamma_dev, const void* beta_dev,
                                        void* sum_dev, void* h_dev, void* mean_dev, void* rstd_dev, int64_t rows, int E,
                                        float eps, int h_dtype, void* stream) {
    MMX_CHECK_ARG(x_dev && gamma_dev && beta_dev && h_dev && mean_dev && rstd_dev, "mmx_add_layernorm_fwd: null pointer");
    MMX_CHECK_ARG(!y_dev || sum_dev, "mmx_add_layernorm_fwd: the sum x + y needs an output buffer");
    MMX_CHECK_ARG(rows > 0 && E > 0 && E % 4 == 0 && E <= 4096, "mmx_add_layernorm_fwd: rows=%ld E=%d (E %% 4 == 0, E <= 4096)",
                  static_cast<long>(rows), E);
    MMX_CHECK_ARG(h_dtype == MMX_F32 || h_dtype == MMX_BF16, "mmx_add_layernorm_fwd: h is fp32 or bf16");
    const unsigned grid = static_cast<unsigned>((rows + 3) / 4);
    hipStream_t s = static_cast<hipStream_t>(stream);
    const float *x = static_cast<const float*>(x_dev), *y = static_cast<const float*>(y_dev);
    const float *g = static_cast<const float*>(gamma_dev), *b = static_cast<const float*>(beta_dev);
    float *so = static_cast<float*>(sum_dev), *ho = h_dtype == MMX_F32 ? static_cast<float*>(h_dev) : nullptr;
    unsigned short* hb = h_dtype == MMX_BF16 ? static_cast<unsigned short*>(h_dev) : nullptr;
    float *mo = static_cast<float*>(mean_dev), *ro = static_cast<float*>(rstd_dev);
    if (E <= 256) mmx::add_layernorm_fwd_kernel<1, false><<<grid, 256, 0, s>>>(x, y, g, b, so, ho, mo, ro, rows, E, eps, hb, nullptr, nullptr);
    else if (E <= 512) mmx::add_layernorm_fwd_kernel<2, false><<<grid, 256, 0, s>>>(x, y, g, b, so, ho, mo, ro, rows, E, eps, hb, nullptr, nullptr);
    else if (E <= 1024) mmx::add_layernorm_fwd_kernel<4, false><<<grid, 256, 0, s>>>(x, y, g, b, so, ho, mo, ro, rows, E, eps, hb, nullptr, nullptr);
    else if (E <= 2048) mmx::add_layernorm_fwd_kernel<8, false><<<grid, 256, 0, s>>>(x, y, g, b, so, ho, mo, ro, rows, E, eps, hb, nullptr, nullptr);
    else mmx::add_layernorm_fwd_kernel<16, false><<<grid, 256, 0, s>>>(x, y, g, b, so, ho, mo, ro, rows, E, eps, hb, nullptr, nullptr);
    MMX_LAUNCH_CHECK("add_layernorm_fwd_kernel");
    return MMX_OK;
}

extern "C" int mmx_add_layernorm_fwd_rows(const void* x_dev, const void* y_dev, const void* gamma_dev, const void* beta_dev,
                                          void* sum_dev, void* h_dev, void* mean_dev, void* rstd_dev, const void* rows_dev,
                                          const void* count_dev, int cap_rows, int E, float eps, void* stream) {
    MMX_CHECK_ARG(x_dev && gamma_dev && beta_dev && h_dev && mean_dev && rstd_dev && rows_dev && count_dev,
                  "mmx_add_layernorm_fwd_rows: null pointer");
    MMX_CHECK_ARG(!y_dev || sum_dev, "mmx_add_layernorm_fwd_rows: the sum x + y needs an output buffer");
    MMX_CHECK_ARG(cap_rows > 0 && E > 0 && E % 4 == 0 && E <= 4096, "mmx_add_layernorm_fwd_rows: cap_rows=%d E=%d (E %% 4 == 0, E <= 4096)",
                  cap_rows, E);
    const unsigned grid = static_cast<unsigned>((cap_rows + 3) / 4);
    hipStream_t s = static_cast<hipStream_t>(stream);
    const float *x = static_cast<const float*>(x_dev), *y = static_cast<const float*>(y_dev);
    const float *g = static_cast<const float*>(gamma_dev), *b = static_cast<const float*>(beta_dev);
    float *so = static_cast<float*>(sum_dev), *ho = static_cast<float*>(h_dev);
    float *mo = static_cast<float*>(mean_dev), *ro = static_cast<float*>(rstd_dev);
    const int *list = static_cast<const int*>(rows_dev), *count = static_cast<const int*>(count_dev);
    if (E <= 256) mmx::add_layernorm_fwd_kernel<1, true><<<grid, 256, 0, s>>>(x, y, g, b, so, ho, mo, ro, cap_rows, E, eps, nullptr, list, count);
    else if (E <= 512) mmx::add_layernorm_fwd_kernel<2, true><<<grid, 256, 0, s>>>(x, y, g, b, so, ho, mo, ro, cap_rows, E, eps, nullptr, list, count);
    else if (E <= 1024) mmx::add_layernorm_fwd_kernel<4, true><<<grid, 256, 0, s>>>(x, y, g, b, so, ho, mo, ro, cap_rows, E, eps, nullptr, list, count);
    else if (E <= 2048) mmx::add_layernorm_fwd_kernel<8, true><<<grid, 256, 0, s>>>(x, y, g, b, so, ho, mo, ro, cap_rows, E, eps, nullptr, list, count);
    else mmx::add_layernorm_fwd_kernel<16, true><<<grid, 256, 0, s>>>(x, y, g, b, so, ho, mo, ro, cap_rows, E, eps, nullptr, list, count);
    MMX_LAUNCH_CHECK("add_layernorm_fwd_kernel<rows>");
    return MMX_OK;
}

extern "C" int mmx_add_layernorm_fwd(const void* x_dev, const void* y_dev, const void* gamma_dev, const void* beta_dev,
                                     void* sum_dev, void* h_dev, void* mean_dev, void* rstd_dev, int64_t rows, int E,
                                     float eps, void* stream) {
    return mmx_add_layernorm_fwd_ex(x_dev, y_dev, gamma_dev, beta_dev, sum_dev, h_dev, mean_dev, rstd_dev, rows, E, eps, MMX_F32,
                                    stream);
}

extern "C" int mmx_quick_gelu_fwd_bf16(const void* x_dev, void* y_dev, int64_t n, void* stream) {
    MMX_CHECK_ARG(x_dev && y_dev && n > 0 && n % 4 == 0, "mmx_quick_gelu_fwd_bf16: bad argument (n %% 4 == 0)");
    MMX_CHECK_ARG((reinterpret_cast<uintptr_t>(x_dev) & 15u) == 0 && (reinterpret_cast<uintptr_t>(y_dev) & 7u) == 0,
                  "mmx_quick_gelu_fwd_bf16: x must be 16-byte, y 8-byte aligned");
    mmx::quick_gelu_fwd_bf16_kernel<<<gelu_grid(n / 4), 256, 0, static_cast<hipStream_t>(stream)>>>(
        static_cast<const mmx::f32x4*>(x_dev), static_cast<mmx::u32x2*>(y_dev), n / 4);
    MMX_LAUNCH_CHECK("quick_gelu_fwd_bf16_kernel");
    return MMX_OK;
}

namespace mmx {

typedef unsigned u32x4 __attribute__((ext_vector_type(4)));


__device__ __forceinline__ float bf_lo(unsigned u) { return __uint_as_float(u << 16); }
__device__ __forceinline__ float bf_hi(unsigned u) { return __uint_as_float(u & 0xffff0000u); }

__global__ __launch_bounds__(256) void quick_gelu_bwd_bf16_kernel(const f32x4* __restrict__ x, const u32x4* __restrict__ dy,
                                                                  u32x4* __restrict__ dx, int64_t n8, int64_t x_n8) {
    for (int64_t i = static_cast<int64_t>(blockIdx.x) * 256 + threadIdx.x; i < n8; i += static_cast<int64_t>(gridDim.x) * 256) {
        const int64_t xi = (x_n8 == n8 ? i : i % x_n8) * 2;
        const f32x4 v0 = x[xi], v1 = x[xi + 1];
        const u32x4 g = dy[i];
        float gv[8], xv[8] = {v0[0], v0[1], v0[2], v0[3], v1[0], v1[1], v1[2], v1[3]};
#pragma unroll
        for (int e = 0; e < 4; ++e) { gv[2 * e] = bf_lo(g[e]); gv[2 * e + 1] = bf_hi(g[e]); }
        float o[8];
#pragma unroll
        for (int e = 0; e < 8; ++e) {
            const float sg = sigmoid_f(1.702f * xv[e]);
            o[e] = gv[e] * (sg + 1.702f * xv[e] * sg * (1.f - sg));
        }
        dx[i] = u32x4{bf_pack(o[0], o[1]), bf_pack(o[2], o[3]), bf_pack(o[4], o[5]), bf_pack(o[6], o[7])};
    }
}

__global__ __launch_bounds__(256) void quick_gelu_bwd_bf16_sweep_kernel(const f32x4* __restrict__ x, const u32x4* __restrict__ dy,
                                                                        u32x4* __restrict__ dx, int64_t x_n8, int batch, int per) {
    const int64_t p = static_cast<int64_t>(blockIdx.x) * 256 + threadIdx.x;
    if (p >= x_n8) return;
    const f32x4 v0 = x[2 * p], v1 = x[2 * p + 1];
    const float xv[8] = {v0[0], v0[1], v0[2], v0[3], v1[0], v1[1], v1[2], v1[3]};
    float d[8];
#pragma unroll
    for (int e = 0; e < 8; ++e) {
        const float sg = sigmoid_f(1.702f * xv[e]);
        d[e] = sg + 1.702f * xv[e] * sg * (1.f - sg);
    }
    const int b0 = blockIdx.y * per, b1 = min(batch, b0 + per);
    const u32x4* src = dy + static_cast<int64_t>(b0) * x_n8 + p;
    u32x4* dst = dx + static_cast<int64_t>(b0) * x_n8 + p;
    int b = b0;
    for (; b + 4 <= b1; b += 4) {
        u32x4 g[4];
#pragma unroll
        for (int u = 0; u < 4; ++u) g[u] = __builtin_nontemporal_load(src + u * x_n8);
#pragma unroll
        for (int u = 0; u < 4; ++u) {
            u32x4 o;
#pragma unroll
            for (int e = 0; e < 4; ++e) o[e] = bf_pack(bf_lo(g[u][e]) * d[2 * e], bf_hi(g[u][e]) * d[2 * e + 1]);
            __builtin_nontemporal_store(o, dst + u * x_n8);
        }
        src += 4 * x_n8;
        dst += 4 * x_n8;
    }
    for (; b < b1; ++b) {
        const u32x4 g = *src;
        u32x4 o;
#pragma unroll
        for (int e = 0; e < 4; ++e) o[e] = bf_pack(bf_lo(g[e]) * d[2 * e], bf_hi(g[e]) * d[2 * e + 1]);
        *dst = o;
        src += x_n8;
        dst += x_n8;
    }
}

template <int ITER>
__global__ __launch_bounds__(256) void layernorm_bwd_add_bf16_row_kernel(const unsigned short* __restrict__ dy,
                                                                         const float* __restrict__ x, const float* __restrict__ mean,
                                                                         const float* __restrict__ rstd, const float* __restrict__ gamma,
                                                                         const float* d_res, float* __restrict__ dx,
                                                                         unsigned short* __restrict__ dx_h, int64_t rows, int x_rows) {
    constexpr int E = 256 * ITER;
    const int64_t r = static_cast<int64_t>(blockIdx.x) * 4 + (threadIdx.x >> 6);
    if (r >= rows) return;
    const int lane = threadIdx.x & 63;
    const int m = static_cast<int>(r % x_rows);
    const u32x2* dyr = reinterpret_cast<const u32x2*>(dy + r * E);
    const f32x4* xr = reinterpret_cast<const f32x4*>(x + static_cast<int64_t>(m) * E);
    const f32x4* gm = reinterpret_cast<const f32x4*>(gamma);
    const f32x4* dr = d_res ? reinterpret_cast<const f32x4*>(d_res + r * E) : nullptr;
    u32x2 raw[ITER];
    f32x4 xh[ITER], res[ITER], g[ITER];
#pragma unroll
    for (int k = 0; k < ITER; ++k) raw[k] = __builtin_nontemporal_load(dyr + lane + 64 * k);
#pragma unroll
    for (int k = 0; k < ITER; ++k) xh[k] = xr[lane + 64 * k];
    if (dr) {
#pragma unroll
        for (int k = 0; k < ITER; ++k) res[k] = __builtin_nontemporal_load(dr + lane + 64 * k);
    }
    const float mu = mean[m], rs = rstd[m];
    float a = 0.f, b = 0.f;
#pragma unroll
    for (int k = 0; k < ITER; ++k) {
        g[k] = f32x4{bf_lo(raw[k][0]), bf_hi(raw[k][0]), bf_lo(raw[k][1]), bf_hi(raw[k][1])} * gm[lane + 64 * k];
        xh[k] = (xh[k] - mu) * rs;
        a += g[k][0] + g[k][1] + g[k][2] + g[k][3];
        b += g[k][0] * xh[k][0] + g[k][1] * xh[k][1] + g[k][2] * xh[k][2] + g[k][3] * xh[k][3];
    }
#pragma unroll
    for (int off = 32; off > 0; off >>= 1) { a += __shfl_xor(a, off); b += __shfl_xor(b, off); }
    a /= static_cast<float>(E);
    b /= static_cast<float>(E);
    f32x4* out = dx ? reinterpret_cast<f32x4*>(dx + r * E) : nullptr;
    u32x2* out_h = dx_h ? reinterpret_cast<u32x2*>(dx_h + r * E) : nullptr;
#pragma unroll
    for (int k = 0; k < ITER; ++k) {
        f32x4 o = (g[k] - a - xh[k] * b) * rs;
        if (dr) o = o + res[k];
        if (out) out[lane + 64 * k] = o;
        if (out_h) out_h[lane + 64 * k] = u32x2{bf_pack(o[0], o[1]), bf_pack(o[2], o[3])};
    }
}

__global__ __launch_bounds__(256) void layernorm_bwd_add_bf16_kernel(const unsigned short* __restrict__ dy,
                                                                     const float* __restrict__ x, const float* __restrict__ mean,
                                                                     const float* __restrict__ rstd, const float* __restrict__ gamma,
                                                                     const float* d_res, float* __restrict__ dx,
                                                                     unsigned short* __restrict__ dx_h, int64_t rows, int x_rows,
                                                                     int E) {
    const int64_t r = static_cast<int64_t>(blockIdx.x) * 4 + (threadIdx.x >> 6);
    if (r >= rows) return;
    const int lane = threadIdx.x & 63;
    const int m = static_cast<int>(r % x_rows);
    const u32x2* dyr = reinterpret_cast<const u32x2*>(dy + r * E);
    const f32x4* xr = reinterpret_cast<const f32x4*>(x + static_cast<int64_t>(m) * E);
    const f32x4* gm = reinterpret_cast<const f32x4*>(gamma);
    const float mu = mean[m], rs = rstd[m];
    const int n4 = E >> 2;
    float a = 0.f, b = 0.f;
    for (int i = lane; i < n4; i += 64) {
        const u32x2 raw = dyr[i];
        const f32x4 g = f32x4{bf_lo(raw[0]), bf_hi(raw[0]), bf_lo(raw[1]), bf_hi(raw[1])} * gm[i];
        const f32x4 xh = (xr[i] - mu) * rs;
        a += g[0] + g[1] + g[2] + g[3];
        b += g[0] * xh[0] + g[1] * xh[1] + g[2] * xh[2] + g[3] * xh[3];
    }
#pragma unroll
    for (int off = 32; off > 0; off >>= 1) { a += __shfl_xor(a, off); b += __shfl_xor(b, off); }
    a /= static_cast<float>(E);
    b /= static_cast<float>(E);
    const f32x4* dr = d_res ? reinterpret_cast<const f32x4*>(d_res + r * E) : nullptr;
    f32x4* out = dx ? reinterpret_cast<f32x4*>(dx + r * E) : nullptr;
    u32x2* out_h = dx_h ? reinterpret_cast<u32x2*>(dx_h + r * E) : nullptr;
    for (int i = lane; i < n4; i += 64) {
        const u32x2 raw = dyr[i];
        const f32x4 g = f32x4{bf_lo(raw[0]), bf_hi(raw[0]), bf_lo(raw[1]), bf_hi(raw[1])} * gm[i];
        const f32x4 xh = (xr[i] - mu) * rs;
        f32x4 o = (g - a - xh * b) * rs;
        if (dr) o = o + dr[i];
        if (out) out[i] = o;
        if (out_h) out_h[i] = u32x2{bf_pack(o[0], o[1]), bf_pack(o[2], o[3])};
    }
}

__global__ __launch_bounds__(256) void rows_to_dense_kernel(const f32x4* __restrict__ vals, const long long* __restrict__ rows,
                                                            f32x4* __restrict__ out, int N, int E4) {
    const int b = blockIdx.y;
    const long long row = rows[b];
    const int64_t per = static_cast<int64_t>(N) * E4;
    for (int64_t i = static_cast<int64_t>(blockIdx.x) * 256 + threadIdx.x; i < per; i += static_cast<int64_t>(gridDim.x) * 256) {
        const int n = static_cast<int>(i / E4), e = static_cast<int>(i - static_cast<int64_t>(n) * E4);
        out[b * per + i] = n == row ? vals[static_cast<int64_t>(b) * E4 + e] : f32x4{0.f, 0.f, 0.f, 0.f};
    }
}

__global__ __launch_bounds__(256) void rows_add_kernel(f32x4* __restrict__ dense, const long long* __restrict__ rows,
                                                       const f32x4* __restrict__ vals, int N, int E4) {
    const int b = blockIdx.y;
    const long long row = rows[b];
    if (row < 0 || row >= N) return;
    f32x4* dst = dense + (static_cast<int64_t>(b) * N + row) * E4;
    for (int e = blockIdx.x * 256 + threadIdx.x; e < E4; e += gridDim.x * 256) dst[e] = dst[e] + vals[static_cast<int64_t>(b) * E4 + e];
}

}

extern "C" int mmx_rows_to_dense(const void* vals_dev, const void* rows_dev, void* out_dev, int B, int N, int E, void* stream) {
    MMX_CHECK_ARG(vals_dev && rows_dev && out_dev && B > 0 && N > 0 && E > 0 && E % 4 == 0 && B <= 65535,
                  "mmx_rows_to_dense: bad argument (B=%d N=%d E=%d, E %% 4 must be 0)", B, N, E);
    const int64_t per = static_cast<int64_t>(N) * (E / 4);
    const dim3 grid(static_cast<unsigned>(per / 256 + 1 > 64 ? 64 : per / 256 + 1), B);
    mmx::rows_to_dense_kernel<<<grid, 256, 0, static_cast<hipStream_t>(stream)>>>(
        static_cast<const f32x4*>(vals_dev), static_cast<const long long*>(rows_dev), static_cast<f32x4*>(out_dev), N, E / 4);
    MMX_LAUNCH_CHECK("rows_to_dense_kernel");
    return MMX_OK;
}

extern "C" int mmx_rows_add(void* dense_dev, const void* rows_dev, const void* vals_dev, int B, int N, int E, void* stream) {
    MMX_CHECK_ARG(dense_dev && rows_dev && vals_dev && B > 0 && N > 0 && E > 0 && E % 4 == 0 && B <= 65535,
                  "mmx_rows_add: bad argument (B=%d N=%d E=%d, E %% 4 must be 0)", B, N, E);
    mmx::rows_add_kernel<<<dim3((E / 4 + 255) / 256, B), 256, 0, static_cast<hipStream_t>(stream)>>>(
        static_cast<f32x4*>(dense_dev), static_cast<const long long*>(rows_dev), static_cast<const f32x4*>(vals_dev), N, E / 4);
    MMX_LAUNCH_CHECK("rows_add_kernel");
    return MMX_OK;
}

extern "C" int mmx_quick_gelu_bwd_bcast_bf16(const void* x_dev, const void* dy_dev, void* dx_dev, int64_t n, int64_t x_n,
                                             void* stream) {
    MMX_CHECK_ARG(x_dev && dy_dev && dx_dev && n > 0 && x_n > 0, "mmx_quick_gelu_bwd_bcast_bf16: bad argument");
    MMX_CHECK_ARG(n % x_n == 0 && x_n % 8 == 0, "mmx_quick_gelu_bwd_bcast_bf16: n=%ld must be a multiple of x_n=%ld, x_n %% 8 == 0",
                  static_cast<long>(n), static_cast<long>(x_n));
    MMX_CHECK_ARG(((reinterpret_cast<uintptr_t>(x_dev) | reinterpret_cast<uintptr_t>(dy_dev) |
                    reinterpret_cast<uintptr_t>(dx_dev)) & 15u) == 0, "mmx_quick_gelu_bwd_bcast_bf16: pointers must be 16-byte aligned");
    const int64_t n8 = n / 8;
    if (n / x_n >= 4 && n / x_n <= 65535 * 8) {
        const int batch = static_cast<int>(n / x_n), per = 8;
        const dim3 grid(static_cast<unsigned>((x_n / 8 + 255) / 256), static_cast<unsigned>((batch + per - 1) / per));
        quick_gelu_bwd_bf16_sweep_kernel<<<grid, 256, 0, static_cast<hipStream_t>(stream)>>>(
            static_cast<const f32x4*>(x_dev), static_cast<const u32x4*>(dy_dev), static_cast<u32x4*>(dx_dev), x_n / 8, batch, per);
        MMX_LAUNCH_CHECK("quick_gelu_bwd_bf16_sweep_kernel");
        return MMX_OK;
    }
    quick_gelu_bwd_bf16_kernel<<<gelu_grid(n8), 256, 0, static_cast<hipStream_t>(stream)>>>(
        static_cast<const f32x4*>(x_dev), static_cast<const u32x4*>(dy_dev), static_cast<u32x4*>(dx_dev), n8, x_n / 8);
    MMX_LAUNCH_CHECK("quick_gelu_bwd_bf16_kernel");
    return MMX_OK;
}

extern "C" int mmx_layernorm_bwd_add_bf16(const void* dy_dev, const void* x_dev, const void* mean_dev, const void* rstd_dev,
                                          const void* gamma_dev, const void* d_res_dev, void* dx_dev, void* dx_bf16_dev,
                                          int64_t rows, int x_rows, int E, void* stream) {
    MMX_CHECK_ARG(dy_dev && x_dev && mean_dev && rstd_dev && gamma_dev && (dx_dev || dx_bf16_dev),
                  "mmx_layernorm_bwd_add_bf16: null pointer");
    MMX_CHECK_ARG(rows > 0 && x_rows > 0 && E > 0 && E % 4 == 0, "mmx_layernorm_bwd_add_bf16: rows=%ld x_rows=%d E=%d (E %% 4 must be 0)",
                  static_cast<long>(rows), x_rows, E);
    const bool aligned = ((reinterpret_cast<uintptr_t>(dy_dev) | reinterpret_cast<uintptr_t>(x_dev) | reinterpret_cast<uintptr_t>(gamma_dev) |
                           reinterpret_cast<uintptr_t>(d_res_dev) | reinterpret_cast<uintptr_t>(dx_dev) |
                           reinterpret_cast<uintptr_t>(dx_bf16_dev)) & 15u) == 0;
#define MMX_LN_ROW(ITER)                                                                                                          \
    if (aligned && E == 256 * ITER) {                                                                                            \
        mmx::layernorm_bwd_add_bf16_row_kernel<ITER><<<static_cast<unsigned>((rows + 3) / 4), 256, 0,                             \
                                                       static_cast<hipStream_t>(stream)>>>(                                      \
            static_cast<const unsigned short*>(dy_dev), static_cast<const float*>(x_dev), static_cast<const float*>(mean_dev),   \
            static_cast<const float*>(rstd_dev), static_cast<const float*>(gamma_dev), static_cast<const float*>(d_res_dev),     \
            static_cast<float*>(dx_dev), static_cast<unsigned short*>(dx_bf16_dev), rows, x_rows);                               \
        MMX_LAUNCH_CHECK("layernorm_bwd_add_bf16_row_kernel");                                                                   \
        return MMX_OK;                                                                                                           \
    }
    MMX_LN_ROW(2) MMX_LN_ROW(3) MMX_LN_ROW(4) MMX_LN_ROW(5)
#undef MMX_LN_ROW
    mmx::layernorm_bwd_add_bf16_kernel<<<static_cast<unsigned>((rows + 3) / 4), 256, 0, static_cast<hipStream_t>(stream)>>>(
        static_cast<const unsigned short*>(dy_dev), static_cast<const float*>(x_dev), static_cast<const float*>(mean_dev),
        static_cast<const float*>(rstd_dev), static_cast<const float*>(gamma_dev), static_cast<const float*>(d_res_dev),
        static_cast<float*>(dx_dev), static_cast<unsigned short*>(dx_bf16_dev), rows, x_rows, E);
    MMX_LAUNCH_CHECK("layernorm_bwd_add_bf16_kernel");
    return MMX_OK;
}
```

### transformer-mm-explainability_amd/csrc/gemm_rows_f32.hip

```cpp
#include "mmx_common.h"

namespace mmx {

typedef float f32x16 __attribute__((ext_vector_type(16)));

static int g_text_live_rows = 1;
static int g_gemm_rows_tm = 32;
static int g_gemm_rows_tn = 0;
static int g_text_live_rows_fwd = 1;
bool text_live_rows_option(const char* key, int value) {
    if (strcmp(key, "text_live_rows") == 0 && value >= 0 && value <= 1) { g_text_live_rows = value; return true; }
    if (strcmp(key, "text_live_rows_fwd") == 0 && value >= 0 && value <= 1) { g_text_live_rows_fwd = value; return true; }
    if (strcmp(key, "gemm_rows_tm") == 0 && (value == 32 || value == 64)) { g_gemm_rows_tm = value; return true; }
    if (strcmp(key, "gemm_rows_tn") == 0 && (value == 0 || value == 32 || value == 64)) { g_gemm_rows_tn = value; return true; }
    return false;
}

__global__ __launch_bounds__(256) void live_rows_kernel(const long long* __restrict__ eot, int B, int N, int* __restrict__ rows,
                                                        int* __restrict__ count) {
    __shared__ int len[256], off[256];
    __shared__ int base;
    if (threadIdx.x == 0) base = 0;
    for (int b0 = 0; b0 < B; b0 += 256) {
        const int b = b0 + threadIdx.x;
        if (b < B) {
            const long long e = eot[b];
            len[threadIdx.x] = static_cast<int>(e < 0 ? 0 : (e > N - 1 ? N - 1 : e)) + 1;
        }
        __syncthreads();
        if (threadIdx.x == 0) {
            int run = base;
            const int n = min(256, B - b0);
            for (int i = 0; i < n; ++i) { off[i] = run; run += len[i]; }
            base = run;
        }
        __syncthreads();
        const int n = min(256, B - b0);
        for (int i = 0; i < n; ++i)
            for (int p = threadIdx.x; p < len[i]; p += 256) rows[off[i] + p] = (b0 + i) * N + p;
        __syncthreads();
    }
    if (threadIdx.x == 0) *count = base;
}

template <int TM, int TN, int BK, int PF, int EPI>
__global__ __launch_bounds__(256, 2) void gemm_rows_f32_kernel(const float* __restrict__ A, const float* __restrict__ W,
                                                               float* __restrict__ C, const int* __restrict__ rows,
                                                               const int* __restrict__ count, int cap, int N, int K,
                                                               const float* __restrict__ bias, float* __restrict__ C2) {
    constexpr int WR = TM / 32, WC = TN / 32;
    constexpr int WK = 4 / (WR * WC);
    constexpr int NG = BK / 8 / WK;
    constexpr int LA = BK + 4;
    constexpr int LB = TN + 4;
    constexpr int CA = TM * BK / 1024, CB = BK * TN / 1024;
    constexpr int RA = 1024 / BK, RB = 1024 / TN;
    static_assert(WR * WC * WK == 4 && NG >= 2 && NG % 2 == 0 && CA >= 1 && CB >= 1 && PF >= 2, "tile shape");
    __shared__ __attribute__((aligned(16))) float As[2][TM * LA];
    __shared__ __attribute__((aligned(16))) float Bs[2][BK * LB];
    __shared__ __attribute__((aligned(16))) float red[WK > 1 ? (WK - 1) * WR * WC * 16 * 64 : 4];
    __shared__ int rid[TM];

    const int tid = threadIdx.x, lane = tid & 63, wave = tid >> 6;
    const int wc = wave % WC, wr = (wave / WC) % WR, wk = wave / (WC * WR);
    const int M = min(*count, cap);
    const int tiles_n = (N + TN - 1) / TN;
    const int bx = blockIdx.x % tiles_n, by = blockIdx.x / tiles_n;
    const int m0 = by * TM, n0 = bx * TN;
    if (m0 >= M) return;

    auto dense_row = [&](int gm) {
        const int r = gm < M ? rows[gm] : -1;
        return static_cast<unsigned>(r) < static_cast<unsigned>(cap) ? r : -1;
    };
    if (tid < TM) rid[tid] = dense_row(m0 + tid);

    f32x16 acc;
#pragma unroll
    for (int v = 0; v < 16; ++v) acc[v] = 0.f;

    const int ar = tid / (BK / 4), ka = (tid % (BK / 4)) * 4;
    bool oka[CA];
    const float* pa[CA];
#pragma unroll
    for (int i = 0; i < CA; ++i) {
        const int arow = dense_row(m0 + ar + i * RA);
        oka[i] = arow >= 0;
        pa[i] = A + static_cast<int64_t>(oka[i] ? arow : 0) * K;
    }
    const int kb = tid / (TN / 4), nbl = (tid % (TN / 4)) * 4;
    const bool okb = n0 + nbl < N;
    const float* pb = W + (okb ? n0 + nbl : 0);
    struct Slab { f32x4 a[CA], b[CB]; };
    Slab ring[PF];
    auto fetch = [&](int t, Slab& x) {
        const int k0 = t * BK;
#pragma unroll
        for (int i = 0; i < CA; ++i) x.a[i] = ldg4_u(pa[i] + min(k0 + ka, K - 4));
#pragma unroll
        for (int i = 0; i < CB; ++i) x.b[i] = ldg4_u(pb + static_cast<int64_t>(min(k0 + kb + i * RB, K - 1)) * N);
    };
    auto stash = [&](int stage, int t, const Slab& x) {
        const f32x4 z = {0.f, 0.f, 0.f, 0.f};
        const int k0 = t * BK;
#pragma unroll
        for (int i = 0; i < CA; ++i)
            *reinterpret_cast<f32x4*>(&As[stage][(ar + i * RA) * LA + ka]) = (oka[i] && k0 + ka < K) ? x.a[i] : z;
#pragma unroll
        for (int i = 0; i < CB; ++i)
            *reinterpret_cast<f32x4*>(&Bs[stage][(kb + i * RB) * LB + nbl]) = (okb && k0 + kb + i * RB < K) ? x.b[i] : z;
    };

    const int li = lane & 31, lg = lane >> 5;
    struct Frag { f32x4 a[NG]; float b[NG][4]; };
    auto read_frag = [&](Frag& f, int stage) {
        const float* Asl = &As[stage][(wr * 32 + li) * LA + 4 * lg];
        const float* Bsl = &Bs[stage][(4 * lg) * LB + wc * 32 + li];
#pragma unroll
        for (int g = 0; g < NG; ++g) {
            const int jj = wk + g * WK;
            f.a[g] = *reinterpret_cast<const f32x4*>(Asl + 8 * jj);
#pragma unroll
            for (int t = 0; t < 4; ++t) f.b[g][t] = Bsl[(8 * jj + t) * LB];
        }
    };
    auto mfma_half = [&](const Frag& f, int h) {
#pragma unroll
        for (int g = h * (NG / 2); g < (h + 1) * (NG / 2); ++g)
#pragma unroll
            for (int t = 0; t < 4; ++t) acc = __builtin_amdgcn_mfma_f32_32x32x2f32(f.a[g][t], f.b[g][t], acc, 0, 0, 0);
    };

    const int nslab = (K + BK - 1) / BK;
    fetch(0, ring[0]);
    stash(0, 0, ring[0]);
#pragma unroll
    for (int j = 1; j <= PF; ++j) fetch(j, ring[j % PF]);
    lds_barrier();
    Frag cur;
    read_frag(cur, 0);
    auto step = [&](int s, Slab& x, bool refill) {
        stash((s + 1) & 1, s + 1, x);
        if (refill) fetch(s + 1 + PF, x);
        mfma_half(cur, 0);
        lds_barrier();
        Frag nxt;
        read_frag(nxt, (s + 1) & 1);
        mfma_half(cur, 1);
        cur = nxt;
    };
    int s = 0;
    for (; s + PF < nslab; s += PF)
#pragma unroll
        for (int j = 0; j < PF; ++j) step(s + j, ring[(j + 1) % PF], true);
#pragma unroll
    for (int j = 0; j < PF - 1; ++j) {
        if (s + j + 1 >= nslab) break;
        step(s + j, ring[(j + 1) % PF], false);
    }
    mfma_half(cur, 0);
    mfma_half(cur, 1);
    if constexpr (WK > 1) {
        const int tile = wr * WC + wc;
        if (wk > 0)
#pragma unroll
            for (int v = 0; v < 16; ++v) red[(((wk - 1) * WR * WC + tile) * 16 + v) * 64 + lane] = acc[v];
        lds_barrier();
        if (wk > 0) return;
#pragma unroll
        for (int q = 0; q < WK - 1; ++q)
#pragma unroll
            for (int v = 0; v < 16; ++v) acc[v] += red[((q * WR * WC + tile) * 16 + v) * 64 + lane];
    }
    const int gn = n0 + wc * 32 + li;
    if (m0 + wr * 32 >= M || gn >= N) return;
    float bv = 0.f;
    if constexpr (EPI != 0) bv = bias[gn];
#pragma unroll
    for (int v = 0; v < 16; ++v) {
        const int r = rid[wr * 32 + (v >> 2) * 8 + lg * 4 + (v & 3)];
        if (r < 0) continue;
        if constexpr (EPI == 0) {
            C[static_cast<int64_t>(r) * N + gn] = acc[v];
        } else {
            const float m = acc[v] + bv;
            C[static_cast<int64_t>(r) * N + gn] = m;
            if constexpr (EPI == 2) C2[static_cast<int64_t>(r) * N + gn] = quick_gelu_f(m);
        }
    }
}

struct RowsTile { int tm, tn; };
static RowsTile rows_tile(int N, int K) {
    if (g_gemm_rows_tm == 64) return {64, 64};
    const int tn = g_gemm_rows_tn ? g_gemm_rows_tn : 64;
    return {32, tn};
}
static int64_t rows_grid(RowsTile t, int cap_rows, int N) {
    return static_cast<int64_t>((N + t.tn - 1) / t.tn) * ((cap_rows + t.tm - 1) / t.tm);
}

template <int EPI>
static void launch_gemm_rows(RowsTile t, int64_t wgs, hipStream_t s, const float* A, const float* W, float* C, const int* rows,
                             const int* count, int cap_rows, int N, int K, const float* bias, float* C2) {
    const unsigned g = static_cast<unsigned>(wgs);
    if (t.tm == 64)
        gemm_rows_f32_kernel<64, 64, 32, 3, EPI><<<g, 256, 0, s>>>(A, W, C, rows, count, cap_rows, N, K, bias, C2);
    else if (t.tn == 32)
        gemm_rows_f32_kernel<32, 32, 64, 3, EPI><<<g, 256, 0, s>>>(A, W, C, rows, count, cap_rows, N, K, bias, C2);
    else
        gemm_rows_f32_kernel<32, 64, 32, 3, EPI><<<g, 256, 0, s>>>(A, W, C, rows, count, cap_rows, N, K, bias, C2);
}

}

using namespace mmx;

extern "C" int mmx_live_rows(const void* eot_dev, int B, int N, void* rows_dev, void* count_dev, void* stream) {
    MMX_CHECK_ARG(eot_dev && rows_dev && count_dev, "mmx_live_rows: null pointer");
    MMX_CHECK_ARG(B > 0 && N > 0 && static_cast<int64_t>(B) * N < (1ll << 31), "mmx_live_rows: B=%d N=%d (B * N must fit an int)", B, N);
    if (!g_text_live_rows) {
        set_error("mmx_live_rows: the row-list route is switched off (option text_live_rows = 0)");
        return MMX_ENOTSUP;
    }
    live_rows_kernel<<<1, 256, 0, static_cast<hipStream_t>(stream)>>>(static_cast<const long long*>(eot_dev), B, N,
                                                                      static_cast<int*>(rows_dev), static_cast<int*>(count_dev));
    MMX_LAUNCH_CHECK("live_rows_kernel");
    return MMX_OK;
}

extern "C" int mmx_gemm_rows_f32(const void* a_dev, const void* w_dev, void* c_dev, const void* rows_dev, const void* count_dev,
                                 int cap_rows, int N, int K, void* stream) {
    MMX_CHECK_ARG(a_dev && w_dev && c_dev && rows_dev && count_dev, "mmx_gemm_rows_f32: null pointer");
    MMX_CHECK_ARG(cap_rows > 0 && N > 0 && K > 0, "mmx_gemm_rows_f32: cap_rows=%d N=%d K=%d", cap_rows, N, K);
    if (N % 4 || K % 4 ||
        ((reinterpret_cast<uintptr_t>(a_dev) | reinterpret_cast<uintptr_t>(w_dev) | reinterpret_cast<uintptr_t>(c_dev)) & 15u)) {
        set_error("mmx_gemm_rows_f32: N=%d and K=%d must be multiples of 4 and the operands 16-byte aligned", N, K);
        return MMX_ENOTSUP;
    }
    const RowsTile tm = rows_tile(N, K);
    const int64_t wgs = rows_grid(tm, cap_rows, N);
    MMX_CHECK_ARG(wgs < (1ll << 31), "mmx_gemm_rows_f32: cap_rows=%d x N=%d is too large a grid", cap_rows, N);
    launch_gemm_rows<0>(tm, wgs, static_cast<hipStream_t>(stream), static_cast<const float*>(a_dev), static_cast<const float*>(w_dev),
                        static_cast<float*>(c_dev), static_cast<const int*>(rows_dev), static_cast<const int*>(count_dev), cap_rows, N, K,
                        nullptr, nullptr);
    MMX_LAUNCH_CHECK("gemm_rows_f32_kernel");
    return MMX_OK;
}

extern "C" int mmx_text_live_rows_fwd_enabled(void) { return g_text_live_rows && g_text_live_rows_fwd; }

extern "C" int mmx_gemm_rows_bias_f32(const void* a_dev, const void* wt_dev, const void* bias_dev, void* c_dev, void* act_dev,
                                      const void* rows_dev, const void* count_dev, int cap_rows, int N, int K, void* stream) {
    MMX_CHECK_ARG(a_dev && wt_dev && bias_dev && c_dev && rows_dev && count_dev, "mmx_gemm_rows_bias_f32: null pointer");
    MMX_CHECK_ARG(cap_rows > 0 && N > 0 && K > 0, "mmx_gemm_rows_bias_f32: cap_rows=%d N=%d K=%d", cap_rows, N, K);
    MMX_CHECK_ARG(act_dev != c_dev, "mmx_gemm_rows_bias_f32: the activation needs a buffer of its own");
    if (N % 4 || K % 4 ||
        ((reinterpret_cast<uintptr_t>(a_dev) | reinterpret_cast<uintptr_t>(wt_dev) | reinterpret_cast<uintptr_t>(c_dev)) & 15u)) {
        set_error("mmx_gemm_rows_bias_f32: N=%d and K=%d must be multiples of 4 and the operands 16-byte aligned", N, K);
        return MMX_ENOTSUP;
    }
    const RowsTile tm = rows_tile(N, K);
    const int64_t wgs = rows_grid(tm, cap_rows, N);
    MMX_CHECK_ARG(wgs < (1ll << 31), "mmx_gemm_rows_bias_f32: cap_rows=%d x N=%d is too large a grid", cap_rows, N);
    const float *A = static_cast<const float*>(a_dev), *W = static_cast<const float*>(wt_dev), *bias = static_cast<const float*>(bias_dev);
    const int *rows = static_cast<const int*>(rows_dev), *count = static_cast<const int*>(count_dev);
    hipStream_t s = static_cast<hipStream_t>(stream);
    if (act_dev)
        launch_gemm_rows<2>(tm, wgs, s, A, W, static_cast<float*>(c_dev), rows, count, cap_rows, N, K, bias, static_cast<float*>(act_dev));
    else
        launch_gemm_rows<1>(tm, wgs, s, A, W, static_cast<float*>(c_dev), rows, count, cap_rows, N, K, bias, nullptr);
    MMX_LAUNCH_CHECK("gemm_rows_f32_kernel<bias>");
    return MMX_OK;
}
```

### transformer-mm-explainability_amd/csrc/mmx_common.h

```cpp
#pragma once
#include <hip/hip_runtime.h>
#include <hip/hip_bf16.h>
#include <hip/hip_fp16.h>
#include <stdint.h>
#include <stdio.h>
#include <string.h>

#include "../../include/mmx_relevancy.h"

namespace mmx {

typedef float f32x4 __attribute__((ext_vector_type(4)));
typedef float f32x2 __attribute__((ext_vector_type(2)));

struct __attribute__((packed, aligned(4))) f32x4_u { f32x4 v; };
__device__ __forceinline__ f32x4 ldg4_u(const float* p) { return reinterpret_cast<const f32x4_u*>(p)->v; }

__device__ __forceinline__ const char* sgpr_ptr(const void* p) {
    const uint64_t u = reinterpret_cast<uint64_t>(p);
    const uint32_t lo = __builtin_amdgcn_readfirstlane(static_cast<uint32_t>(u));
    const uint32_t hi = __builtin_amdgcn_readfirstlane(static_cast<uint32_t>(u >> 32));
    return reinterpret_cast<const char*>((static_cast<uint64_t>(hi) << 32) | lo);
}
typedef unsigned u32x4 __attribute__((ext_vector_type(4)));
constexpr int kRawBufferFlags = 0x00020000;

struct __attribute__((packed, aligned(2))) u16x4_u { unsigned short v[4]; };

__device__ __forceinline__ float bf16_bits_to_f32(unsigned short b) {
    return __uint_as_float(static_cast<unsigned int>(b) << 16);
}
__device__ __forceinline__ float f16_bits_to_f32(unsigned short b) {
    return __half2float(__ushort_as_half(b));
}

template <int DT>
__device__ __forceinline__ f32x4 load4_as_f32(const void* base, int64_t idx);
template <>
__device__ __forceinline__ f32x4 load4_as_f32<MMX_F32>(const void* base, int64_t idx) {
    return ldg4_u(static_cast<const float*>(base) + idx);
}
template <>
__device__ __forceinline__ f32x4 load4_as_f32<MMX_BF16>(const void* base, int64_t idx) {
    u16x4_u r = *reinterpret_cast<const u16x4_u*>(static_cast<const unsigned short*>(base) + idx);
    f32x4 o;
    o[0] = bf16_bits_to_f32(r.v[0]); o[1] = bf16_bits_to_f32(r.v[1]);
    o[2] = bf16_bits_to_f32(r.v[2]); o[3] = bf16_bits_to_f32(r.v[3]);
    return o;
}
template <>
__device__ __forceinline__ f32x4 load4_as_f32<MMX_F16>(const void* base, int64_t idx) {
    u16x4_u r = *reinterpret_cast<const u16x4_u*>(static_cast<const unsigned short*>(base) + idx);
    f32x4 o;
    o[0] = f16_bits_to_f32(r.v[0]); o[1] = f16_bits_to_f32(r.v[1]);
    o[2] = f16_bits_to_f32(r.v[2]); o[3] = f16_bits_to_f32(r.v[3]);
    return o;
}
typedef unsigned u32x3 __attribute__((ext_vector_type(3)));
struct __attribute__((packed, aligned(4))) u32x3_u { u32x3 v; };
template <int DT> struct stream_raw { u32x3 v; };
template <> struct stream_raw<MMX_F32> { f32x4 v; };
template <int DT>
__device__ __forceinline__ stream_raw<DT> load4_stream_raw(const void* base, int64_t idx) {
    stream_raw<DT> r;
    if constexpr (DT == MMX_F32) {
        r.v = ldg4_u(static_cast<const float*>(base) + idx);
    } else {
        const unsigned short* p = static_cast<const unsigned short*>(base) + (idx & ~static_cast<int64_t>(1));
        r.v = reinterpret_cast<const u32x3_u*>(p)->v;
    }
    return r;
}
template <int DT>
__device__ __forceinline__ f32x4 stream_cvt(const stream_raw<DT>& r, int64_t idx) {
    if constexpr (DT == MMX_F32) {
        return r.v;
    } else {
        const unsigned sh = (idx & 1) ? 2u : 0u;
        const unsigned lo = __builtin_amdgcn_alignbyte(r.v[1], r.v[0], sh);
        const unsigned hi = __builtin_amdgcn_alignbyte(r.v[2], r.v[1], sh);
        f32x4 o;
        if constexpr (DT == MMX_BF16) {
            o[0] = __uint_as_float(lo << 16); o[1] = __uint_as_float(lo & 0xffff0000u);
            o[2] = __uint_as_float(hi << 16); o[3] = __uint_as_float(hi & 0xffff0000u);
        } else {
            o[0] = f16_bits_to_f32(static_cast<unsigned short>(lo)); o[1] = f16_bits_to_f32(static_cast<unsigned short>(lo >> 16));
            o[2] = f16_bits_to_f32(static_cast<unsigned short>(hi)); o[3] = f16_bits_to_f32(static_cast<unsigned short>(hi >> 16));
        }
        return o;
    }
}
template <int DT>
__device__ __forceinline__ f32x4 load4_stream(const void* base, int64_t idx) {
    return stream_cvt<DT>(load4_stream_raw<DT>(base, idx), idx);
}

template <int DT>
__device__ __forceinline__ float load1_as_f32(const void* base, int64_t idx);
template <>
__device__ __forceinline__ float load1_as_f32<MMX_F32>(const void* base, int64_t idx) {
    return static_cast<const float*>(base)[idx];
}
template <>
__device__ __forceinline__ float load1_as_f32<MMX_BF16>(const void* base, int64_t idx) {
    return bf16_bits_to_f32(static_cast<const unsigned short*>(base)[idx]);
}
template <>
__device__ __forceinline__ float load1_as_f32<MMX_F16>(const void* base, int64_t idx) {
    return f16_bits_to_f32(static_cast<const unsigned short*>(base)[idx]);
}

template <int DT> struct slab_elem { typedef unsigned short type; };
template <> struct slab_elem<MMX_F32> { typedef float type; };
template <int DT>
__device__ __forceinline__ float slab_load(const typename slab_elem<DT>::type* p) {
    if constexpr (DT == MMX_F32) return *p;
    else if constexpr (DT == MMX_BF16) return bf16_bits_to_f32(*p);
    else return f16_bits_to_f32(*p);
}
template <int DT>
__device__ __forceinline__ void slab_store(typename slab_elem<DT>::type* p, float v) {
    if constexpr (DT == MMX_F32) {
        *p = v;
    } else if constexpr (DT == MMX_BF16) {
        const unsigned u = __float_as_uint(v);
        *p = (v != v) ? static_cast<unsigned short>(0x7FC0)
                      : static_cast<unsigned short>((u + 0x7FFFu + ((u >> 16) & 1u)) >> 16);
    } else {
        *p = __half_as_ushort(__float2half(v));
    }
}

__device__ __forceinline__ float relu_nan(float x) { return (x < 0.0f) ? 0.0f : x; }

__device__ __forceinline__ float sigmoid_f(float z) { return 1.f / (1.f + expf(-z)); }
__device__ __forceinline__ float quick_gelu_f(float v) { return v * sigmoid_f(1.702f * v); }

__device__ __forceinline__ f32x4 mfma16x16x4(float a, float b, f32x4 acc) {
    return __builtin_amdgcn_mfma_f32_16x16x4f32(a, b, acc, 0, 0, 0);
}

typedef __bf16 bf16x8 __attribute__((ext_vector_type(8)));
__device__ __forceinline__ bf16x8 pack_bf16(f32x4 lo, f32x4 hi) {
    bf16x8 r;
    r[0] = static_cast<__bf16>(lo[0]); r[1] = static_cast<__bf16>(lo[1]); r[2] = static_cast<__bf16>(lo[2]);
    r[3] = static_cast<__bf16>(lo[3]); r[4] = static_cast<__bf16>(hi[0]); r[5] = static_cast<__bf16>(hi[1]);
    r[6] = static_cast<__bf16>(hi[2]); r[7] = static_cast<__bf16>(hi[3]);
    return r;
}
__device__ __forceinline__ f32x4 mfma16x16x32_bf16(bf16x8 a, bf16x8 b, f32x4 acc) {
    return __builtin_amdgcn_mfma_f32_16x16x32_bf16(a, b, acc, 0, 0, 0);
}

__device__ __forceinline__ void lds_barrier() { asm volatile("s_waitcnt lgkmcnt(0)\n\ts_barrier" ::: "memory"); }

template <int CTRL>
__device__ __forceinline__ float dpp_row(float x) {
    return __int_as_float(__builtin_amdgcn_update_dpp(0, __float_as_int(x), CTRL, 0xF, 0xF, false));
}
__device__ __forceinline__ float group16_max(float x) {
    x = fmaxf(x, dpp_row<0x128>(x)); x = fmaxf(x, dpp_row<0x124>(x));
    x = fmaxf(x, dpp_row<0x122>(x)); x = fmaxf(x, dpp_row<0x121>(x));
    return x;
}
__device__ __forceinline__ float group16_sum(float x) {
    x += dpp_row<0x128>(x); x += dpp_row<0x124>(x); x += dpp_row<0x122>(x); x += dpp_row<0x121>(x);
    return x;
}

__device__ __forceinline__ int xcd_contiguous_id(int w, int total) {
    constexpr int X = 8;
    const int xcd = w % X, local = w / X, per = total / X, rem = total % X;
    return xcd < rem ? xcd * (per + 1) + local : rem * (per + 1) + (xcd - rem) * per + local;
}

inline size_t dtype_size(int dt) { return dt == MMX_F32 ? 4 : 2; }

void set_error(const char* fmt, ...);
void attn_head_enable(int on);
void attn_head_tile_skip(int on);
bool self_chain_cols_applies(int n_layers, int B, int H, int N);
int self_chain_cols_launch(const void* const* attn_layers, const void* const* grad_layers, int n_layers, int B, int H, int N,
                           int64_t attn_bstride, const void* R_init, void* R_out, int nt_policy, int debug, hipStream_t s);
void chain_cols_options(int c, int nb);
bool self_chain_groups_applies(int n_layers, int G, int H, int N);
int self_chain_groups_launch(const void* const* attn_layers, const void* const* grad_layers, int n_layers, int B, int H, int N, int G,
                             int64_t attn_bstride, const void* R_init, void* R_out, unsigned* counters, float* parts, int nt_policy,
                             int debug, hipStream_t s);
void attn_stream_enable(int on);
void attn_fwd_split_enable(int on);
void attn_bf16_v2_enable(int on);
void attn_bf16_v3_enable(int mode);
int hip_fail(hipError_t e, const char* what);
int zero_async(void* dst, size_t bytes, hipStream_t s);
bool chain_rows_layer_applies(int N);
int chain_rows_layer_launch(const void* attn, const void* grad, const float* R_in, float* R_out, int B, int H, int N, int dtype,
                            int64_t attn_bstride, hipStream_t s, int debug = 0);
bool bmm_f32_tiles_try(const float* A, const float* B, const float* Cin, float* C, int batch, int M, int N, int K, int trans_a,
                       int64_t sa, int64_t sb, int64_t sc, int nan_to_zero, int cin_is_row, hipStream_t s);
bool text_live_rows_option(const char* key, int value);
int device_cu_count();
int identity_async(float* R, int batch, int N, hipStream_t s);

}

#define MMX_CHECK_ARG(cond, ...)            \
    do {                                    \
        if (!(cond)) {                      \
            mmx::set_error(__VA_ARGS__);    \
            return MMX_EINVAL;              \
        }                                   \
    } while (0)

#define MMX_LAUNCH_CHECK(what)                                  \
    do {                                                        \
        hipError_t e__ = hipGetLastError();                     \
        if (e__ != hipSuccess) return mmx::hip_fail(e__, what); \
    } while (0)
```

### transformer-mm-explainability_amd/ops.py

```python
from __future__ import annotations

import contextlib
import threading
import ctypes as C
import gc
import os
import weakref

import torch

from . import _lib
from ._lib import MMXError, check, lib

_DTYPES = {torch.float32: _lib.MMX_F32, torch.float16: _lib.MMX_F16, torch.bfloat16: _lib.MMX_BF16}


def _stream():
    return C.c_void_p(torch.cuda.current_stream().cuda_stream)


def _dev(*tensors):
    for t in tensors:
        if t is not None and not t.is_cuda:
            raise MMXError("mmx ops need HIP-device tensors (got %s); there is no CPU path" % t.device)
# ... 212 lines not shown
    x, dy = _f32c(x), _f32c(dy)
    dx = torch.empty_like(dy)
    if x.shape == dy.shape:
        check(lib().mmx_quick_gelu_bwd(_p(x), _p(dy), _p(dx), x.numel(), _stream()), "mmx_quick_gelu_bwd")
    elif x.shape[1:] == dy.shape[1:] and dy.shape[0] % x.shape[0] == 0 and x.numel() % 4 == 0:
        check(lib().mmx_quick_gelu_bwd_bcast(_p(x), _p(dy), _p(dx), dy.numel(), x.numel(), _stream()),
              "mmx_quick_gelu_bwd_bcast")
    else:
        raise MMXError("quick_gelu_bwd: x %s vs dy %s" % (tuple(x.shape), tuple(dy.shape)))
    return dx


def add_layernorm(x, y, gamma, beta, eps=1e-5, h_dtype=torch.float32):
    _dev(x, y, gamma, beta)
    x = _f32c(x)
    E = x.shape[-1]
    rows = x.numel() // E
    if y is not None:
        y = _f32c(y)
        if y.shape != x.shape:
            raise MMXError("add_layernorm: x %s vs y %s" % (tuple(x.shape), tuple(y.shape)))
    s = torch.empty_like(x) if y is not None else x
    h = torch.empty(x.shape, dtype=h_dtype, device=x.device)
    mean = torch.empty(rows, dtype=torch.float32, device=x.device)
    rstd = torch.empty(rows, dtype=torch.float32, device=x.device)
    check(lib().mmx_add_layernorm_fwd_ex(_p(x), _p(y), _p(_f32c(gamma)), _p(_f32c(beta)), _p(s) if y is not None else _p(None),
                                         _p(h), _p(mean), _p(rstd), rows, E, float(eps), _DTYPES[h_dtype], _stream()),
          "mmx_add_layernorm_fwd")
    return s, h, mean, rstd


def layernorm_bwd_add(dy, x, mean, rstd, gamma, d_res=None):
    _dev(dy, x, mean, rstd, gamma, d_res)
    dy, x = _f32c(dy), _f32c(x)
    E = dy.shape[-1]
    rows, x_rows = dy.numel() // E, x.numel() // E
    dx = torch.empty_like(dy)
    check(lib().mmx_layernorm_bwd_add(_p(dy), _p(x), _p(_f32c(mean)), _p(_f32c(rstd)), _p(_f32c(gamma)),
                                      _p(_f32c(d_res)) if d_res is not None else _p(None), _p(dx), rows, x_rows, E,
                                      _stream()), "mmx_layernorm_bwd_add")
    return dx


def layernorm_bwd_add_bf16(dy, x, mean, rstd, gamma, d_res=None, want_f32=True):
    _dev(dy, x, mean, rstd, gamma, d_res)
    if dy.dtype != torch.bfloat16:
        raise MMXError("layernorm_bwd_add_bf16: dy must be bf16")
    dy, x = dy.contiguous(), _f32c(x)
    E = dy.shape[-1]
    rows, x_rows = dy.numel() // E, x.numel() // E
    dx = torch.empty(dy.shape, dtype=torch.float32, device=dy.device) if want_f32 else None
    dx_h = torch.empty_like(dy)
    check(lib().mmx_layernorm_bwd_add_bf16(_p(dy), _p(x), _p(_f32c(mean)), _p(_f32c(rstd)), _p(_f32c(gamma)),
                                           _p(_f32c(d_res)) if d_res is not None else _p(None), _p(dx), _p(dx_h), rows,
                                           x_rows, E, _stream()), "mmx_layernorm_bwd_add_bf16")
    return dx, dx_h


_GEMM_WEIGHTS = {}


def _converted(weight, dtype):
    per_weight = _GEMM_WEIGHTS.get(id(weight))
    if per_weight is None:
        per_weight = _GEMM_WEIGHTS[id(weight)] = {}
        weakref.finalize(weight, _GEMM_WEIGHTS.pop, id(weight), None)
    hit = per_weight.get(dtype)
    if hit is None or hit[0] != weight._version or hit[1].device != weight.device:
        hit = per_weight[dtype] = (weight._version, weight.detach().to(dtype))
    return hit[1]


def transposed_weight(weight):
    per_weight = _GEMM_WEIGHTS.get(id(weight))
    if per_weight is None:
        per_weight = _GEMM_WEIGHTS[id(weight)] = {}
        weakref.finalize(weight, _GEMM_WEIGHTS.pop, id(weight), None)
    hit = per_weight.get("t")
    if hit is None or hit[0] != weight._version or hit[1].device != weight.device:
        hit = per_weight["t"] = (weight._version, weight.detach().t().contiguous())
    return hit[1]


def sign_split_weight(weight, transposed=False):
    per_weight = _GEMM_WEIGHTS.get(id(weight))
    if per_weight is None:
        per_weight = _GEMM_WEIGHTS[id(weight)] = {}
        weakref.finalize(weight, _GEMM_WEIGHTS.pop, id(weight), None)
    hit = per_weight.get("pn")
    if hit is None or hit[0] != weight._version or hit[1].device != weight.device:
        w = weight.detach().float()
        hit = per_weight["pn"] = (weight._version, torch.cat((w.clamp(min=0), w.clamp(max=0)), dim=1).contiguous())
        per_weight.pop("pnT", None)
    if not transposed:
        return hit[1]
    hit_t = per_weight.get("pnT")
    if hit_t is None or hit_t[0] != weight._version or hit_t[1].device != weight.device:
        hit_t = per_weight["pnT"] = (weight._version, hit[1].t().contiguous())
    return hit_t[1]


def lrp_fusable(*tensors):
    return all(t.is_cuda and t.dtype == torch.float32 for t in tensors)


def lrp_linear(R, X, weight, normalize):
    n_in, n_out = X.shape[-1], R.shape[-1]
    if tuple(R.shape[:-1]) != tuple(X.shape[:-1]) or tuple(weight.shape) != (n_out, n_in):
        raise MMXError("lrp_linear: R %s, X %s, weight %s do not describe Linear.relprop (R [..., out], X [..., in], weight "
                       "[out, in] with equal leading dimensions)" % (tuple(R.shape), tuple(X.shape), tuple(weight.shape)))
    Xc, Rc = X.contiguous(), R.contiguous()
    rows = Xc.numel() // n_in
    WW = sign_split_weight(weight)
    st = _stream()
    XX = torch.empty(rows, 2 * n_in, dtype=torch.float32, device=X.device)
    check(lib().mmx_lrp_split_signs(_p(Xc), _p(XX), rows, n_in, st), "mmx_lrp_split_signs")

    def mm(a, wt_of, k, n):
        if rows <= 128 and k <= 1024:
            out_ = torch.empty(rows, n, dtype=torch.float32, device=a.device)
            check(lib().mmx_linear_f32(_p(a), _p(wt_of()), None, _p(out_), rows, n, k, st), "mmx_linear_f32")
            return out_
        return torch.mm(a, wt_of())
    Z = mm(XX, lambda: sign_split_weight(weight, transposed=True) if rows <= 128 and 2 * n_in <= 1024 else WW.t(), 2 * n_in, n_out)
    S = torch.empty_like(Z)
    check(lib().mmx_lrp_safe_divide(_p(Rc), _p(Z), _p(S), Z.numel(), st), "mmx_lrp_safe_divide")
    Y = mm(S, lambda: WW, n_out, 2 * n_in)
    out = torch.empty(X.shape, dtype=torch.float32, device=X.device)
    ws = _workspace(lib().mmx_lrp_workspace_bytes(), X.device, tag="lrp") if normalize else None
    check(lib().mmx_lrp_linear_combine(_p(XX), _p(Y), _p(out), rows, n_in, _p(Rc) if normalize else None, Rc.numel(),
                                       _p(ws), st), "mmx_lrp_linear_combine")
    return out


def lrp_mha_rescale(cam_v_pre, cam_v_post, cam_k, cam_q, cam_o):
    vp, vq = cam_v_pre.contiguous(), cam_v_post.contiguous()
    ck, cq, co = cam_k.contiguous().clone(), cam_q.contiguous().clone(), cam_o.contiguous()
    ws = _workspace(lib().mmx_lrp_workspace_bytes(), cam_k.device, tag="lrp")
    check(lib().mmx_lrp_mha_rescale(_p(vp), vp.numel(), _p(vq), vq.numel(), _p(ck), ck.numel(), _p(cq), cq.numel(), _p(co),
                                    co.numel(), _p(ws), _stream()), "mmx_lrp_mha_rescale")
    return ck, cq


def lrp_add(R, a, b, per_sample):
    Rc, ac, bc = R.contiguous(), a.contiguous(), b.contiguous()
    batch = Rc.shape[0] if (per_sample and Rc.dim() > 1) else 1
    if batch > 64:
        return None
    ra, rb = torch.empty_like(Rc), torch.empty_like(Rc)
    ws = _workspace(lib().mmx_lrp_workspace_bytes(), R.device, tag="lrp")
    check(lib().mmx_lrp_add_relprop(_p(Rc), _p(ac), _p(bc), _p(ra), _p(rb), batch, Rc.numel() // batch, _p(ws), _stream()),
          "mmx_lrp_add_relprop")
    return ra, rb


def lrp_clone(Rs, X):
    Xc = X.contiguous()
    rc = [r.contiguous() for r in Rs]
    out = torch.empty_like(Xc)
    tbl, _k = _lib.ptr_table([r.data_ptr() for r in rc])
    check(lib().mmx_lrp_clone_relprop(tbl, len(rc), _p(Xc), _p(out), Xc.numel(), _stream()), "mmx_lrp_clone_relprop")
    return out


_MM_OUT_DTYPE = [None]


def _mm_f32_out(a, b):
    if _MM_OUT_DTYPE[0] is None:
        try:
            torch.mm(a[:1], b, out_dtype=torch.float32)
            _MM_OUT_DTYPE[0] = True
        except (RuntimeError, TypeError):
            _MM_OUT_DTYPE[0] = False
    if _MM_OUT_DTYPE[0]:
        return torch.mm(a, b, out_dtype=torch.float32)
    return torch.mm(a, b).float()


def backward_gemm_bf16(x, weight):
    w = _converted(weight, torch.bfloat16)
    return torch.mm(x.reshape(-1, x.shape[-1]), w).view(*x.shape[:-1], w.shape[-1])


def backward_gemm(x, weight, dtype=torch.float32):
    if dtype == torch.float32:
        return torch.matmul(x, weight)
    w = _converted(weight, dtype)
    return _mm_f32_out(x.reshape(-1, x.shape[-1]).to(dtype), w).view(*x.shape[:-1], w.shape[-1])


def linear(x, weight, bias=None, dtype=torch.float32):
    if dtype == torch.float32:
        return torch.nn.functional.linear(x, weight, bias)
    w = _converted(weight, dtype)
    y = _mm_f32_out(x.reshape(-1, x.shape[-1]).to(dtype), w.t()).view(*x.shape[:-1], w.shape[0])
    return y if bias is None else y.add_(bias)


class ChainPlan:

    def __init__(self, attn_layers, grad_layers, batch_size, shared_attn=False, half_chain=False, causal=False):
        _dev(*attn_layers, *grad_layers)
        self.half_chain = bool(half_chain)
        self.flags = _lib.CHAIN_CAUSAL if causal else 0
        self.attn = [_capture(a) for a in attn_layers]
        self.grad = [_capture(g) for g in grad_layers]
        if not self.attn or len(self.attn) != len(self.grad) or len(self.attn) > _lib.MAX_LAYERS:
            raise MMXError("ChainPlan: need 1..%d (attn, grad) layer pairs" % _lib.MAX_LAYERS)
        g0 = self.grad[0]
        self.n = g0.shape[-1]
        self.batch = batch_size
        self.heads = g0.numel() // (self.n * self.n) // batch_size
        self.dt = _DTYPES[g0.dtype]
        self.shared = 0 if shared_attn else -1
        for a, g in zip(self.attn, self.grad):
            if g.shape != g0.shape or g.dtype != g0.dtype or a.dtype != g0.dtype or \
                    a.numel() * (batch_size if shared_attn else 1) != g.numel():
                raise MMXError("ChainPlan: inconsistent layer shapes/dtypes")
        self.device = g0.device
        if self.half_chain and g0.dtype == torch.bfloat16:
            raise MMXError("ChainPlan: the fp16 chain reads fp32 or fp16 slabs")
        self.need = lib().mmx_self_chain_workspace_bytes(len(self.attn), batch_size, self.heads, self.n, 0, self.dt)
        if self.half_chain and self.n <= 128:
            self.need = 0
        self.ws = torch.empty(max(self.need, 1), dtype=torch.uint8, device=g0.device)
        self.at, self._k1 = _lib.ptr_table([a.data_ptr() for a in self.attn])
        self.gt, self._k2 = _lib.ptr_table([g.data_ptr() for g in self.grad])

    def launch(self, out=None):
        if out is None:
            out = torch.empty(self.batch, self.n, self.n, dtype=torch.float32, device=self.device)
        if self.half_chain:
            check(lib().mmx_relevancy_self_chain_half(self.at, self.gt, len(self.attn), self.batch, self.heads, self.n, self.dt,
                                                      self.shared, _p(out), _p(self.ws), self.need, _stream()),
                  "mmx_relevancy_self_chain_half")
            return out.to(torch.float16)
        check(lib().mmx_relevancy_self_chain_flags(self.at, self.gt, len(self.attn), self.batch, self.heads, self.n, self.dt,
                                                   self.shared, None, _p(out), None, None, 0, self.flags, _p(self.ws), self.need,
                                                   _stream()), "mmx_relevancy_self_chain_flags")
        return out


def matmul(a, b, add_to=None, trans_a=False, nan_to_zero=False):
    _dev(a, b, add_to)
    a, b = _f32c(a), _f32c(b)
    batch = 1
    for t in (a, b):
        if t.dim() == 3:
            batch = max(batch, t.shape[0])
    am, ak = (a.shape[-1], a.shape[-2]) if trans_a else (a.shape[-2], a.shape[-1])
    if b.shape[-2] != ak:
        raise MMXError("matmul: inner dims %d vs %d" % (ak, b.shape[-2]))
    n = b.shape[-1]
    sa = a.shape[-2] * a.shape[-1] if (a.dim() == 3 and a.shape[0] > 1) else 0
    sb = ak * n if (b.dim() == 3 and b.shape[0] > 1) else 0
    squeeze = a.dim() == 2 and b.dim() == 2
    out = torch.empty(batch, am, n, dtype=torch.float32, device=a.device)
    cin = None
    if add_to is not None:
        cin = _f32c(add_to).expand(batch, am, n).contiguous() if add_to.dim() == 2 or add_to.shape[0] != batch \
            else _f32c(add_to)
    check(lib().mmx_bmm_f32(_p(a), _p(b), _p(cin), _p(out), batch, am, n, ak, int(trans_a), sa, sb, am * n,
                            int(nan_to_zero), _stream()), "mmx_bmm_f32")
    return out[0] if squeeze else out


def rows_to_dense(vals, rows, n_tokens):
    _dev(vals, rows)
    vals, rows = _f32c(vals), rows.to(torch.long).contiguous()
    if vals.dim() != 2 or rows.numel() != vals.shape[0]:
        raise MMXError("rows_to_dense: vals [B, E] and rows [B] expected, got %s / %s" % (tuple(vals.shape), tuple(rows.shape)))
    B, E = vals.shape
    out = torch.empty(B, n_tokens, E, dtype=torch.float32, device=vals.device)
    check(lib().mmx_rows_to_dense(_p(vals), _p(rows), _p(out), B, n_tokens, E, _stream()), "mmx_rows_to_dense")
    return out


def rows_add_(dense, rows, vals):
    _dev(dense, rows, vals)
    if dense.dtype != torch.float32 or not dense.is_contiguous():
        raise MMXError("rows_add_: dense must be fp32 contiguous")
    B, N, E = dense.shape
    if tuple(vals.shape) != (B, E) or rows.numel() != B:
        raise MMXError("rows_add_: dense [B, N, E] needs vals [B, E] and rows [B], got %s / %s / %s"
                       % (tuple(dense.shape), tuple(vals.shape), tuple(rows.shape)))
    check(lib().mmx_rows_add(_p(dense), _p(rows.to(torch.long).contiguous()), _p(_f32c(vals)), B, N, E, _stream()), "mmx_rows_add")
    return dense


class LiveRows:
    poison = False

    def __init__(self, rows, count, batch, n_tokens):
        self.rows, self.count, self.batch, self.n_tokens = rows, count, batch, n_tokens
        self.cap = batch * n_tokens

    def _out(self, like, width):
        shape = tuple(like.shape[:-1]) + (width,)
        if LiveRows.poison:
            return torch.full(shape, float("nan"), dtype=torch.float32, device=like.device)
        return torch.empty(shape, dtype=torch.float32, device=like.device)

    def _check(self, what, *tensors):
        for t in tensors:
            if t.dtype != torch.float32 or not t.is_contiguous() or t.numel() // t.shape[-1] != self.cap:
                raise MMXError("%s: fp32 contiguous tensors of %d rows expected, got %s %s" % (what, self.cap, t.dtype, tuple(t.shape)))


def live_rows(eot, n_tokens):
    _dev(eot)
    eot = eot.to(torch.long).contiguous()
    B = eot.numel()
    buf = torch.empty(B * n_tokens + 1, dtype=torch.int32, device=eot.device)
    rc = lib().mmx_live_rows(_p(eot), B, n_tokens, _p(buf[1:]), _p(buf[:1]), _stream())
    if rc == _lib.MMX_ENOTSUP:
        return None
    check(rc, "mmx_live_rows")
    return LiveRows(buf[1:], buf[:1], B, n_tokens)


def gemm_rows_eligible(*weights):
    return all(w.dtype == torch.float32 and w.dim() == 2 and w.is_contiguous() and w.shape[0] % 4 == 0 and w.shape[1] % 4 == 0
               and w.data_ptr() % 16 == 0 for w in weights)


def gemm_rows(x, weight, live, out=None):
    _dev(x, weight, out)
    K, M = weight.shape
    if out is None:
        out = live._out(x, M)
    live._check("gemm_rows", x, out)
    if x.shape[-1] != K or out.shape[-1] != M or not gemm_rows_eligible(weight):
        raise MMXError("gemm_rows: x %s @ weight %s -> out %s" % (tuple(x.shape), tuple(weight.shape), tuple(out.shape)))
    check(lib().mmx_gemm_rows_f32(_p(x), _p(weight), _p(out), _p(live.rows), _p(live.count), live.cap, M, K, _stream()),
          "mmx_gemm_rows_f32")
    return out


def live_rows_forward_enabled():
    return bool(lib().mmx_text_live_rows_fwd_enabled())


def linear_rows(x, weight, bias, live, out=None, gelu=False, act_out=None):
    _dev(x, weight, bias, out, act_out)
    M, K = weight.shape
    if out is None:
        out = live._out(x, M)
    live._check("linear_rows", x, out)
    if x.shape[-1] != K or out.shape[-1] != M or not gemm_rows_eligible(weight) or bias is None or bias.numel() != M:
        raise MMXError("linear_rows: x %s @ weight %s^T + bias -> out %s" % (tuple(x.shape), tuple(weight.shape), tuple(out.shape)))
    act = (act_out if act_out is not None else live._out(x, M)) if gelu else None
    if act is not None:
        live._check("linear_rows", act)
        if act.shape[-1] != M or act.data_ptr() == out.data_ptr():
            raise MMXError("linear_rows: the activation needs a [.., %d] tensor of its own" % M)
    check(lib().mmx_gemm_rows_bias_f32(_p(x), _p(transposed_weight(weight)), _p(_f32c(bias.detach())), _p(out), _p(act), _p(live.rows),
                                       _p(live.count), live.cap, M, K, _stream()), "mmx_gemm_rows_bias_f32")
    return (out, act) if gelu else out


def add_layernorm_rows(x, y, gamma, beta, eps, live, out=None):
    _dev(x, y, gamma, beta)
    live._check("add_layernorm_rows", x, *([y] if y is not None else []))
    E = x.shape[-1]
    if out is not None:
        s, h, mean, rstd = out
        _dev(s, h, mean, rstd)
        s = s if y is not None else x
        live._check("add_layernorm_rows", h, *([s] if y is not None else []))
        if h.shape[-1] != E or (y is not None and s.shape[-1] != E) or mean.numel() != live.cap or rstd.numel() != live.cap or \
                not (mean.is_contiguous() and rstd.is_contiguous() and mean.dtype == rstd.dtype == torch.float32):
            raise MMXError("add_layernorm_rows: out must be (s, h [.., %d], mean, rstd [%d]) fp32 contiguous" % (E, live.cap))
    else:
        s = live._out(x, E) if y is not None else x
        h = live._out(x, E)
        mean, rstd = live._out(x, 1).view(-1), live._out(x, 1).view(-1)
    check(lib().mmx_add_layernorm_fwd_rows(_p(x), _p(y), _p(_f32c(gamma)), _p(_f32c(beta)), _p(s) if y is not None else _p(None), _p(h),
                                           _p(mean), _p(rstd), _p(live.rows), _p(live.count), live.cap, E, float(eps), _stream()),
          "mmx_add_layernorm_fwd_rows")
    return s, h, mean, rstd


def quick_gelu_bwd_rows(x, dy, live):
    _dev(x, dy)
    live._check("quick_gelu_bwd_rows", x, dy)
    dx = live._out(dy, dy.shape[-1])
    check(lib().mmx_quick_gelu_bwd_rows(_p(x), _p(dy), _p(dx), _p(live.rows), _p(live.count), live.cap, dy.shape[-1], _stream()),
          "mmx_quick_gelu_bwd_rows")
    return dx


def layernorm_bwd_add_rows(dy, x, mean, rstd, gamma, d_res, live):
    _dev(dy, x, mean, rstd, gamma, d_res)
    live._check("layernorm_bwd_add_rows", dy, x, *([d_res] if d_res is not None else []))
    mean, rstd = _f32c(mean), _f32c(rstd)
    if mean.numel() != live.cap or rstd.numel() != live.cap:
        raise MMXError("layernorm_bwd_add_rows: %d statistics for %d rows" % (mean.numel(), live.cap))
    dx = live._out(dy, dy.shape[-1])
    check(lib().mmx_layernorm_bwd_add_rows(_p(dy), _p(x), _p(mean), _p(rstd), _p(_f32c(gamma)), _p(d_res), _p(dx), _p(live.rows),
                                           _p(live.count), live.cap, dy.shape[-1], _stream()), "mmx_layernorm_bwd_add_rows")
    return dx


def small_linear(x, lin):
    rows = x.numel() // x.shape[-1]
    if not (x.is_cuda and x.dtype == torch.float32 and rows <= 128 and lin.in_features == lin.out_features <= 256) or \
            (torch.is_grad_enabled() and x.requires_grad):
        return lin(x)
    x2 = _f32c(x).view(rows, lin.in_features)
    out = torch.empty(rows, lin.out_features, dtype=torch.float32, device=x.device)
    check(lib().mmx_linear_f32(_p(x2), _p(transposed_weight(lin.weight)), _p(lin.bias.detach() if lin.bias is not None else None),
                               _p(out), rows, lin.out_features, lin.in_features, _stream()), "mmx_linear_f32")
    return out.view(*x.shape[:-1], lin.out_features)


def chain_matvec(A, y, base=None):
    _dev(A, y, base)
    A, y = _f32c(A), _f32c(y)
    base = y if base is None else _f32c(base)
    B, N = y.shape
    out = torch.empty_like(y)
    check(lib().mmx_chain_matvec(_p(A), _p(y), _p(base), _p(out), B, N, _stream()), "mmx_chain_matvec")
    return out


def chain_vecmat(x, A, base=None):
    _dev(A, x, base)
    A, x = _f32c(A), _f32c(x)
    base = x if base is None else _f32c(base)
    B, N = x.shape
    out = torch.empty_like(x)
    need = lib().mmx_chain_vecmat_workspace_bytes(B, N)
    ws = _workspace(need, x.device, "vecmat")
    check(lib().mmx_chain_vecmat(_p(A), _p(x), _p(base), _p(out), B, N, _p(ws), need, _stream()), "mmx_chain_vecmat")
    return out


def avg_heads_vecmat(x, cam, grad, batch_size=1, shared_attn=False, base=None):
    _dev(cam, grad, x, base)
    cam, grad, x = _capture(cam), _capture(grad), _f32c(x)
    base = x if base is None else _f32c(base)
    B, N = x.shape
    bh = grad.numel() // (N * N)
    ok = cam.numel() * batch_size == grad.numel() if shared_attn else cam.shape == grad.shape
    if not ok or B != batch_size or bh % B or tuple(grad.shape[-2:]) != (N, N) or cam.dtype != grad.dtype:
        raise MMXError("avg_heads_vecmat: x %s, cam %s/%s, grad %s/%s, batch %d" % (tuple(x.shape), tuple(cam.shape), cam.dtype,
                                                                                     tuple(grad.shape), grad.dtype, batch_size))
    out = torch.empty_like(x)
    need = lib().mmx_avg_heads_vecmat_workspace_bytes(B, N)
    ws = _workspace(need, x.device, "ahv")
    check(lib().mmx_avg_heads_vecmat(_p(cam), _p(grad), _p(x), _p(base), _p(out), B, bh // B, N, _DTYPES[cam.dtype],
                                     0 if shared_attn else -1, _p(ws), need, _stream()), "mmx_avg_heads_vecmat")
    return out


def handle_residual(R, check_diag=True):
    _dev(R)
    R = _f32c(R)
    n = R.shape[-1]
    batch = R.numel() // (n * n)
    out = torch.empty_like(R)
    dmin = torch.empty(1, dtype=torch.float32, device=R.device) if check_diag else None
    check(lib().mmx_handle_residual(_p(R), _p(out), batch, n, _p(dmin), _stream()), "mmx_handle_residual")
    if check_diag == "defer":
        return out, dmin
    if check_diag:
        assert dmin.item() >= 0
    return out


def mm_attention_rules(R_ss, R_qq, cam_sq, R_qs=None, apply_normalization=True, apply_self_in_rule_10=True,
                       nan_to_zero=False, check_diag=True):
    _dev(R_ss, R_qq, cam_sq, R_qs)
    R_ss, R_qq, cam_sq = _f32c(R_ss), _f32c(R_qq), _f32c(cam_sq)
    ns, nq = cam_sq.shape[-2], cam_sq.shape[-1]
    if R_ss.shape[-1] != ns or R_qq.shape[-1] != nq:
        raise MMXError("mm_attention_rules: R_ss %s, R_qq %s, cam_sq %s" % (tuple(R_ss.shape), tuple(R_qq.shape), tuple(cam_sq.shape)))
    flags = (_lib.MM_NORMALIZE if apply_normalization else 0) | (_lib.MM_SELF_IN_RULE10 if apply_self_in_rule_10 else 0) \
        | (_lib.MM_NAN_TO_ZERO if nan_to_zero else 0)
    sq_add = torch.empty(ns, nq, dtype=torch.float32, device=cam_sq.device)
    ss_add = None
    if R_qs is not None:
        R_qs = _f32c(R_qs)
        ss_add = torch.empty(ns, ns, dtype=torch.float32, device=cam_sq.device)
    want_diag = check_diag and apply_normalization
    dmin = torch.empty(1, dtype=torch.float32, device=cam_sq.device) if want_diag else None
    need = lib().mmx_mm_rules_workspace_bytes(ns, nq)
    ws = _workspace(need, cam_sq.device)
    check(lib().mmx_mm_attention_rules(_p(R_ss), _p(R_qq), _p(R_qs), _p(cam_sq), _p(sq_add), _p(ss_add), ns, nq,
                                       flags, _p(dmin), _p(ws), need, _stream()), "mmx_mm_attention_rules")
    if want_diag:
        assert dmin.item() >= 0
    return (sq_add, ss_add) if R_qs is not None else sq_add


LXMERT_FUSED_MAX_TOKENS = 48


def lxmert_schedule(lang, vis, x_lang_cross, x_img_cross, x_lang_self, x_img_self, apply_normalization=True,
                    apply_self_in_rule_10=True, check_diag=True, text_len=None):
    groups = [lang, vis, x_lang_cross, x_img_cross, x_lang_self, x_img_self]
    flat = [t for grp in groups for pair in grp for t in pair]
    _dev(*flat)
    if any(t.dtype != torch.float32 for t in flat):
        raise MMXError("lxmert_schedule: fp32 capture slabs only")
    keep = [[(a.contiguous(), g.contiguous()) for a, g in grp] for grp in groups]
    a0 = keep[2][0][0]
    B, H, T, I = a0.shape
    n_x = len(keep[2])
    if len(keep[4]) != n_x or len(keep[3]) < n_x - 1 or len(keep[5]) < n_x - 1:
        raise MMXError("lxmert_schedule: inconsistent cross-layer lists")
    dev = a0.device
    R_tt = torch.empty(B, T, T, dtype=torch.float32, device=dev)
    R_ti = torch.empty(B, T, I, dtype=torch.float32, device=dev)
    R_ii = torch.empty(B, I, I, dtype=torch.float32, device=dev)
    R_it = torch.empty(B, I, T, dtype=torch.float32, device=dev)
    want_diag = bool(check_diag) and apply_normalization and apply_self_in_rule_10
    dmin = torch.empty(1, dtype=torch.float32, device=dev) if want_diag else None
    if text_len is not None:
        _dev(text_len)
        text_len = text_len.to(dtype=torch.int32).contiguous()
        if text_len.numel() != B:
            raise MMXError("lxmert_schedule: text_len needs one entry per sample")
    tables, alive = [], []
    for grp in keep:
        for which in (0, 1):
            tbl, arr = _lib.ptr_table([pair[which].data_ptr() for pair in grp])
            tables.append(tbl)
            alive.append(arr)
    flags = (_lib.MM_NORMALIZE if apply_normalization else 0) | (_lib.MM_SELF_IN_RULE10 if apply_self_in_rule_10 else 0)
    la, lg, va, vg, xlca, xlcg, xica, xicg, xlsa, xlsg, xisa, xisg = tables
    need = lib().mmx_lxmert_schedule_workspace_bytes(len(keep[0]), len(keep[1]), n_x, B, T, I)
    ws = _workspace(need, dev, tag="lxmert_schedule")
    check(lib().mmx_lxmert_schedule(la, lg, len(keep[0]), va, vg, len(keep[1]), xlca, xlcg, xica, xicg, xlsa, xlsg,
                                    xisa, xisg, n_x, B, H, T, I, flags, _p(text_len), _p(R_tt), _p(R_ti), _p(R_ii),
                                    _p(R_it), _p(dmin), _p(ws), need, _stream()), "mmx_lxmert_schedule")
    if check_diag == "defer":
        return R_tt, R_ti, R_ii, R_it, dmin
    if want_diag:
        assert dmin.item() >= 0
    return R_tt, R_ti, R_ii, R_it


def rollout_chain(layers, normalize):
    _dev(*layers)
    mats = [_f32c(m) for m in layers]
    n = mats[0].shape[-1]
    batch = mats[0].numel() // (n * n)
    out = torch.empty(batch, n, n, dtype=torch.float32, device=mats[0].device)
    need = lib().mmx_rollout_workspace_bytes(batch, n)
    ws = _workspace(need, mats[0].device)
    tbl, _k = _lib.ptr_table([m.data_ptr() for m in mats])
    check(lib().mmx_rollout_chain(tbl, len(mats), batch, n, int(normalize), _p(out), _p(ws), need, _stream()),
          "mmx_rollout_chain")
    return out


def _bhnd_strides(t, layout):
    if t.stride(-1) != 1:
        raise MMXError("attention operands need a contiguous head_dim")
    if layout == "bnhd":
        return t.stride(0), t.stride(2), t.stride(1)
    if layout == "bhnd":
        return t.stride(0), t.stride(1), t.stride(2)
    raise MMXError("layout %r" % layout)


def _mask_strides(mask, Nk):
    if mask is None:
        return None, 0, 0
    mask = _f32c(mask)
    if mask.dim() == 2:
        return mask, 0, Nk
    if mask.dim() == 3:
        return mask, (mask.shape[1] * Nk if mask.shape[0] > 1 else 0), (Nk if mask.shape[1] > 1 else 0)
    raise MMXError("mask must be [Nq,Nk] or [B,Nq|1,Nk]")


def attn_capture_fwd(q, k, v, probs_out, scale, scale_mode=_lib.SCALE_Q_FIRST, mask=None, layout="bnhd", mma_bf16=False):
    _dev(q, k, v, probs_out, mask)
    if q.dtype != torch.float32 or k.dtype != torch.float32 or v.dtype != torch.float32:
        raise MMXError("attention capture op is fp32 in this ABI version")
    if layout == "bnhd":
        B, Nq, H, D = q.shape
        Nk = k.shape[1]
    else:
        B, H, Nq, D = q.shape
        Nk = k.shape[2]
    if probs_out.dtype not in _DTYPES or not probs_out.is_contiguous() or probs_out.numel() != B * H * Nq * Nk:
        raise MMXError("probs_out must be a contiguous fp32 / fp16 / bf16 [B,H,Nq,Nk] slab")
    o = torch.empty(q.shape, dtype=torch.float32, device=q.device)
    mask, msb, msq = _mask_strides(mask, Nk)
    check(lib().mmx_attn_capture_fwd_ex(_p(q), _p(k), _p(v), *_bhnd_strides(q, layout), *_bhnd_strides(k, layout),
                                        *_bhnd_strides(v, layout), _p(mask), msb, msq, _p(probs_out),
                                        _DTYPES[probs_out.dtype] | (_lib.MMX_ATTN_MMA_BF16 if mma_bf16 else 0),
                                        _p(o), *_bhnd_strides(o, layout), B, H, Nq, Nk, D,
                                        float(scale), scale_mode, _stream()), "mmx_attn_capture_fwd")
    return o


def attn_fwd(q, k, v, scale, scale_mode=_lib.SCALE_Q_FIRST, mask=None, layout="bnhd", out=None):
    _dev(q, k, v, mask, out)
    if q.dtype != torch.float32 or k.dtype != torch.float32 or v.dtype != torch.float32:
        raise MMXError("attn_fwd is exact fp32 (no bf16 / fp16 mode yet), got %s" % str(q.dtype).replace("torch.", ""))
    if layout == "bnhd":
        B, Nq, H, D = q.shape
        Nk = k.shape[1]
    else:
        B, H, Nq, D = q.shape
        Nk = k.shape[2]
    if out is not None and (out.dtype != torch.float32 or out.shape != q.shape):
        raise MMXError("attn_fwd: out must be fp32 of q's shape %s" % (tuple(q.shape),))
    o = out if out is not None else torch.empty(q.shape, dtype=torch.float32, device=q.device)
    mask, msb, msq = _mask_strides(mask, Nk)
    check(lib().mmx_attn_fwd(_p(q), _p(k), _p(v), *_bhnd_strides(q, layout), *_bhnd_strides(k, layout), *_bhnd_strides(v, layout),
                             _p(mask), msb, msq, _p(o), *_bhnd_strides(o, layout), B, H, Nq, Nk, D, float(scale), scale_mode,
                             _stream()), "mmx_attn_fwd")
    return o


def patch_ranks(scores, out=None):
    _dev(scores, out)
    if scores.dim() != 2 or scores.dtype != torch.float32:
        raise MMXError("patch_ranks: scores must be [B, P] fp32, got %s %s" % (tuple(scores.shape), scores.dtype))
    scores = scores.contiguous()
    if out is not None and (out.dtype != torch.int32 or out.shape != scores.shape or not out.is_contiguous()):
        raise MMXError("patch_ranks: out must be a contiguous int32 tensor of the scores' shape")
    ranks = out if out is not None else torch.empty(scores.shape, dtype=torch.int32, device=scores.device)
    check(lib().mmx_patch_ranks(_p(scores), _p(ranks), scores.shape[0], scores.shape[1], _stream()), "mmx_patch_ranks")
    return ranks


def perturb_patches(images, ranks, counts, fill, out=None):
    _dev(images, ranks, counts, fill, out)
    if images.dim() != 4 or images.shape[2] != images.shape[3] or images.dtype != torch.float32:
        raise MMXError("perturb_patches: images must be [B, C, R, R] fp32, got %s %s" % (tuple(images.shape), images.dtype))
    B, C, R, _ = images.shape
    if ranks.dtype != torch.int32 or ranks.dim() != 2 or ranks.shape[0] != B or counts.dtype != torch.int32 or counts.dim() != 1:
        raise MMXError("perturb_patches: ranks must be [B, P] int32 and counts [S] int32")
    grid = int(round(ranks.shape[1] ** 0.5))
    if grid < 1 or grid * grid != ranks.shape[1] or R % grid:
        raise MMXError("perturb_patches: %d patches are not a square grid that divides the resolution %d" % (ranks.shape[1], R))
    fill = _f32c(fill).reshape(-1)
    if fill.numel() != C:
        raise MMXError("perturb_patches: fill needs one value per channel (%d), got %d" % (C, fill.numel()))
    S = counts.shape[0]
    images, ranks, counts = images.contiguous(), ranks.contiguous(), counts.contiguous()
    if out is None:
        out = torch.empty(S, B, C, R, R, dtype=torch.float32, device=images.device)
    elif out.dtype != torch.float32 or not out.is_contiguous() or out.numel() != S * B * C * R * R:
        raise MMXError("perturb_patches: out must be a contiguous fp32 [S, B, C, R, R] tensor")
    check(lib().mmx_perturb_patches(_p(images), _p(ranks), _p(counts), _p(fill), _p(out), B, C, R, R // grid, S, _stream()),
          "mmx_perturb_patches")
    return out


def head_kernel_shape(n_q, n_k, head_dim, slab_dtype=torch.float32):
    if not (slab_dtype == torch.float32 and 1 <= n_k <= 128 and 1 <= n_q <= 256 and head_dim % 4 == 0 and head_dim <= 64):
        return False
    dp, ntk, ntq = (32 if head_dim <= 32 else 64), (n_k + 15) // 16, (n_q + 15) // 16
    lds = 4 * max(ntk * 16 * (2 * dp + 12), ntq * 16 * (ntk * 16 + 4 + dp + 4))
    return lds <= 160 * 1024 and not (ntk >= 7 and ntq > 8)


def _attn_capture_bwd_grouped(q, k, v, probs, d_o, dprobs_out, scale, scale_mode, need_dqkv, layout, out, o, mma_bf16,
                              rel_row, images):
    if rel_row is None or mma_bf16:
        raise MMXError("attn_capture_bwd: images= is the grouped exact-fp32 row mode: it needs rel_row and mma_bf16=False")
    if layout == "bnhd":
        M, Nq, H, D = q.shape
        Nk = k.shape[1]
    else:
        M, H, Nq, D = q.shape
        Nk = k.shape[2]
    T = d_o.shape[0]
    if images != M or probs.shape[0] != M or images < 1 or T % images:
        raise MMXError("attn_capture_bwd: images=%d needs q/k/v/probs of batch %d and a d_o batch that is a multiple of it "
                       "(q batch %d, probs batch %d, d_o batch %d)" % (images, images, M, probs.shape[0], T))
    if rel_row.dtype != torch.float32 or tuple(rel_row.shape) != (T, Nq) or Nq != Nk or probs.dtype != torch.float32:
        raise MMXError("attn_capture_bwd: grouped rel_row needs fp32 [T, N] rows and fp32 slabs of a self-attention")
    if d_o.dtype != torch.float32:
        raise MMXError("attn_capture_bwd: grouped rel_row needs an fp32 d_o")
    if dprobs_out is not None and (dprobs_out.dtype != torch.float32 or dprobs_out.shape[0] != T):
        raise MMXError("attn_capture_bwd: grouped dprobs_out must be fp32 with batch %d" % T)
    if d_o.stride(-1) != 1:
        d_o = d_o.contiguous()
    if probs.stride(-1) != 1 or not probs.is_contiguous():
        raise MMXError("attn_capture_bwd: grouped probs must be a contiguous [M, H, N, N] slab")
    dq = dk = dv = None
    zero3 = (0, 0, 0)
    if need_dqkv:
        if out is not None:
            dq, dk, dv = out
        else:
            dq, dk, dv = (torch.empty((T,) + tuple(t.shape[1:]), dtype=torch.float32, device=t.device) for t in (q, k, v))
    if o is not None and (o.dtype != torch.float32 or o.stride(-1) != 1):
        o = None
    rel_row = rel_row.contiguous()
    rel_out = torch.empty_like(rel_row)
    dprobs = dprobs_out
    if dprobs is None and need_dqkv and not head_kernel_shape(Nq, Nk, D, probs.dtype):
# ... 172 lines not shown
```

Measured before the change: 8129.

## Split-K live-row GEMMs into partial planes reduced inside consumer layernorm kernels

Adds a split-K form of the live-rows FP32 GEMM that writes S partial-sum planes whenever the row-tile grid is smaller than a threshold of dense workgroups. The add+LayerNorm forward and LayerNorm backward kernels sum those planes, plus the bias, as they read them, so no separate reduction kernel is launched. The goal is to fill the GPU when only a few text rows are live, as in the out_proj, c_proj, c_fc-backward and in_proj-backward products. The cost is extra plane memory traffic and redundant plane reads in the consumers, with the split factor decided by a plan and by runtime options.

```diff
diff --git a/include/mmx_relevancy.h b/include/mmx_relevancy.h
--- a/include/mmx_relevancy.h
+++ b/include/mmx_relevancy.h
@@ -87,6 +87,16 @@
                                void* sum_dev, void* h_dev, void* mean_dev, void* rstd_dev, const void* rows_dev,
                                const void* count_dev, int cap_rows, int E, float eps, void* stream);
 int mmx_text_live_rows_fwd_enabled(void);
+int mmx_gemm_rows_split_plan(int N, int K, int* plan);
+int mmx_gemm_rows_planes_f32(const void* a_dev, const void* w_dev, void* planes_dev, const void* rows_dev, const void* count_dev,
+                             int cap_rows, int N, int K, const int* plan, void* stream);
+int mmx_add_layernorm_fwd_rows_planes(const void* x_dev, const void* planes_dev, const void* bias_dev, const void* gamma_dev,
+                                      const void* beta_dev, void* sum_dev, void* h_dev, void* mean_dev, void* rstd_dev,
+                                      const void* rows_dev, const void* count_dev, int cap_rows, int E, float eps, const int* plan,
+                                      void* stream);
+int mmx_layernorm_bwd_add_rows_planes(const void* planes_dev, const void* x_dev, const void* mean_dev, const void* rstd_dev,
+                                      const void* gamma_dev, const void* d_res_dev, void* dx_dev, const void* rows_dev,
+                                      const void* count_dev, int cap_rows, int E, const int* plan, void* stream);
 
 int mmx_chain_matvec(const void* A_dev, const void* y_dev, const void* base_dev, void* out_dev, int B, int N, void* stream);
 size_t mmx_chain_vecmat_workspace_bytes(int B, int N);
diff --git a/transformer-mm-explainability_amd/_lib.py b/transformer-mm-explainability_amd/_lib.py
--- a/transformer-mm-explainability_amd/_lib.py
+++ b/transformer-mm-explainability_amd/_lib.py
@@ -90,6 +90,10 @@
     "mmx_gemm_rows_bias_f32": (_i, [_vp, _vp, _vp, _vp, _vp, _vp, _vp, _i, _i, _i, _vp]),
     "mmx_add_layernorm_fwd_rows": (_i, [_vp, _vp, _vp, _vp, _vp, _vp, _vp, _vp, _vp, _vp, _i, _i, _f, _vp]),
     "mmx_text_live_rows_fwd_enabled": (_i, []),
+    "mmx_gemm_rows_split_plan": (_i, [_i, _i, _vp]),
+    "mmx_gemm_rows_planes_f32": (_i, [_vp, _vp, _vp, _vp, _vp, _i, _i, _i, _vp, _vp]),
+    "mmx_add_layernorm_fwd_rows_planes": (_i, [_vp, _vp, _vp, _vp, _vp, _vp, _vp, _vp, _vp, _vp, _vp, _i, _i, _f, _vp, _vp]),
+    "mmx_layernorm_bwd_add_rows_planes": (_i, [_vp, _vp, _vp, _vp, _vp, _vp, _vp, _vp, _vp, _i, _i, _vp, _vp]),
     "mmx_chain_matvec": (_i, [_vp, _vp, _vp, _vp, _i, _i, _vp]),
     "mmx_chain_vecmat_workspace_bytes": (_sz, [_i, _i]),
     "mmx_chain_vecmat": (_i, [_vp, _vp, _vp, _vp, _i, _i, _vp, _sz, _vp]),
diff --git a/transformer-mm-explainability_amd/clip_model.py b/transformer-mm-explainability_amd/clip_model.py
--- a/transformer-mm-explainability_amd/clip_model.py
+++ b/transformer-mm-explainability_amd/clip_model.py
@@ -267,9 +267,11 @@
                 blk.attn_probs, blk.attn_grad = buffers.layer_probs(l), buffers.layer_grads(l)
                 return x1 + mlp_out, tape
             if live is not None:
-                x1, h2, mean2, rstd2 = ln(x, ops.linear_rows(o.view(Bx, N, E), at.out_proj.weight, at.out_proj.bias, live), blk.ln_2)
+                x1, h2, mean2, rstd2 = ln(x, ops.linear_rows(o.view(Bx, N, E), at.out_proj.weight, at.out_proj.bias, live,
+                                                             planes=ops.gemm_rows_split(E, E) > 1), blk.ln_2)
                 m, act = ops.linear_rows(h2, blk.mlp.c_fc.weight, blk.mlp.c_fc.bias, live, gelu=True)
-                mlp_out = ops.linear_rows(act, blk.mlp.c_proj.weight, blk.mlp.c_proj.bias, live)
+                mlp_out = ops.linear_rows(act, blk.mlp.c_proj.weight, blk.mlp.c_proj.bias, live,
+                                          planes=l + 1 < len(blocks) and ops.gemm_rows_split(E, act.shape[-1]) > 1)
             else:
                 x1, h2, mean2, rstd2 = ln(x, self._linear(o.view(Bx, N, E), at.out_proj.weight, at.out_proj.bias), blk.ln_2)
                 m = self._linear(h2, blk.mlp.c_fc.weight, blk.mlp.c_fc.bias)
@@ -385,7 +387,7 @@
             elif live is not None:
                 d_a = ops.gemm_rows(dx, blk.mlp.c_proj.weight, live)
                 d_m = ops.quick_gelu_bwd_rows(m, d_a, live)
-                d_h2 = ops.gemm_rows(d_m, blk.mlp.c_fc.weight, live)
+                d_h2 = ops.gemm_rows(d_m, blk.mlp.c_fc.weight, live, planes=ops.gemm_rows_split(E, d_m.shape[-1]) > 1)
                 d_x1 = ops.layernorm_bwd_add_rows(d_h2, x1, mean2, rstd2, blk.ln_2.weight, dx, live)
                 d_o = ops.gemm_rows(d_x1, at.out_proj.weight, live, out=d_o_dense)
             elif stream16:
@@ -422,7 +424,7 @@
                 d_h1 = ops.backward_gemm_bf16(dq_in if att16 else dq_in.to(torch.bfloat16), at.in_proj_weight)
                 dx, dx_h = ops.layernorm_bwd_add_bf16(d_h1, x, mean1, rstd1, blk.ln_1.weight, d_x1)
             elif live is not None:
-                d_h1 = ops.gemm_rows(dqkv.view(B, N, 3 * E), at.in_proj_weight, live)
+                d_h1 = ops.gemm_rows(dqkv.view(B, N, 3 * E), at.in_proj_weight, live, planes=ops.gemm_rows_split(E, 3 * E) > 1)
                 dx = ops.layernorm_bwd_add_rows(d_h1, x, mean1, rstd1, blk.ln_1.weight, d_x1, live)
             else:
                 d_h1 = self._gemm(dqkv.view(B, N, 3 * E), at.in_proj_weight)
diff --git a/transformer-mm-explainability_amd/csrc/elementwise_kernels.hip b/transformer-mm-explainability_amd/csrc/elementwise_kernels.hip
--- a/transformer-mm-explainability_amd/csrc/elementwise_kernels.hip
+++ b/transformer-mm-explainability_amd/csrc/elementwise_kernels.hip
@@ -174,6 +174,50 @@
     }
 }
 
+__global__ __launch_bounds__(256) void layernorm_bwd_add_planes_kernel(const float* __restrict__ dy, const float* __restrict__ x,
+                                                                       const float* __restrict__ mean, const float* __restrict__ rstd,
+                                                                       const float* __restrict__ gamma, const float* d_res,
+                                                                       float* __restrict__ dx, int64_t rows, int E,
+                                                                       const int* __restrict__ list, const int* __restrict__ count,
+                                                                       RowsSplit sp) {
+    int64_t r = static_cast<int64_t>(blockIdx.x) * 4 + (threadIdx.x >> 6);
+    if (r >= rows || r >= *count) return;
+    r = list[r];
+    if (r < 0 || r >= rows) return;
+    const int lane = threadIdx.x & 63, n4 = E >> 2;
+    const int S = rows_split_eff(*count, static_cast<int>(rows), sp);
+    const int64_t plane4 = rows * n4;
+    const f32x4* dyr = reinterpret_cast<const f32x4*>(dy + r * E);
+    const f32x4* xr = reinterpret_cast<const f32x4*>(x + r * E);
+    const f32x4* gm = reinterpret_cast<const f32x4*>(gamma);
+    const float mu = mean[r], rs = rstd[r];
+    auto dy_at = [&](int i) {
+        f32x4 d = dyr[i];
+        for (int z = 1; z < S; ++z) d = d + dyr[z * plane4 + i];
+        return d;
+    };
+    float a = 0.f, b = 0.f;
+    for (int i = lane; i < n4; i += 64) {
+        const f32x4 g = dy_at(i) * gm[i];
+        const f32x4 xh = (xr[i] - mu) * rs;
+        a += g[0] + g[1] + g[2] + g[3];
+        b += g[0] * xh[0] + g[1] * xh[1] + g[2] * xh[2] + g[3] * xh[3];
+    }
+#pragma unroll
+    for (int off = 32; off > 0; off >>= 1) { a += __shfl_xor(a, off); b += __shfl_xor(b, off); }
+    a /= static_cast<float>(E);
+    b /= static_cast<float>(E);
+    const f32x4* dr = d_res ? reinterpret_cast<const f32x4*>(d_res + r * E) : nullptr;
+    f32x4* out = reinterpret_cast<f32x4*>(dx + r * E);
+    for (int i = lane; i < n4; i += 64) {
+        const f32x4 g = dy_at(i) * gm[i];
+        const f32x4 xh = (xr[i] - mu) * rs;
+        f32x4 o = (g - a - xh * b) * rs;
+        if (dr) o = o + dr[i];
+        out[i] = o;
+    }
+}
+
 }
 
 extern "C" int mmx_layernorm_bwd_add(const void* dy_dev, const void* x_dev, const void* mean_dev, const void* rstd_dev,
@@ -204,15 +248,33 @@
     return MMX_OK;
 }
 
+extern "C" int mmx_layernorm_bwd_add_rows_planes(const void* planes_dev, const void* x_dev, const void* mean_dev, const void* rstd_dev,
+                                                 const void* gamma_dev, const void* d_res_dev, void* dx_dev, const void* rows_dev,
+                                                 const void* count_dev, int cap_rows, int E, const int* plan, void* stream) {
+    MMX_CHECK_ARG(planes_dev && x_dev && mean_dev && rstd_dev && gamma_dev && dx_dev && rows_dev && count_dev && plan,
+                  "mmx_layernorm_bwd_add_rows_planes: null pointer");
+    MMX_CHECK_ARG(cap_rows > 0 && E > 0 && E % 4 == 0, "mmx_layernorm_bwd_add_rows_planes: cap_rows=%d E=%d (E %% 4 must be 0)", cap_rows, E);
+    const mmx::RowsSplit sp = {plan[0], plan[1], plan[2], plan[3], plan[4]};
+    MMX_CHECK_ARG(sp.S >= 1 && sp.S <= 8 && sp.tm > 0 && sp.tiles_n > 0 && sp.dense_wgs >= 1, "mmx_layernorm_bwd_add_rows_planes: bad plan");
+    mmx::layernorm_bwd_add_planes_kernel<<<static_cast<unsigned>((cap_rows + 3) / 4), 256, 0, static_cast<hipStream_t>(stream)>>>(
+        static_cast<const float*>(planes_dev), static_cast<const float*>(x_dev), static_cast<const float*>(mean_dev),
+        static_cast<const float*>(rstd_dev), static_cast<const float*>(gamma_dev), static_cast<const float*>(d_res_dev),
+        static_cast<float*>(dx_dev), cap_rows, E, static_cast<const int*>(rows_dev), static_cast<const int*>(count_dev), sp);
+    MMX_LAUNCH_CHECK("layernorm_bwd_add_planes_kernel");
+    return MMX_OK;
+}
+
 namespace mmx {
 
-template <int NV, bool ROWS>
+template <int NV, bool ROWS, bool PLANES = false>
 __global__ __launch_bounds__(256) void add_layernorm_fwd_kernel(const float* __restrict__ x, const float* __restrict__ y,
                                                                 const float* __restrict__ gamma, const float* __restrict__ beta,
                                                                 float* __restrict__ sum_out, float* __restrict__ h_out,
                                                                 float* __restrict__ mean_out, float* __restrict__ rstd_out,
                                                                 int64_t rows, int E, float eps, unsigned short* __restrict__ h_bf16,
-                                                                const int* __restrict__ list, const int* __restrict__ count) {
+                                                                const int* __restrict__ list, const int* __restrict__ count,
+                                                                const float* __restrict__ bias = nullptr, RowsSplit sp = {1, 0, 0, 0, 0}) {
+    static_assert(ROWS || !PLANES, "the planes form is a row-list form");
     int64_t r = static_cast<int64_t>(blockIdx.x) * 4 + (threadIdx.x >> 6);
     if (r >= rows) return;
     if constexpr (ROWS) {
@@ -225,13 +287,19 @@
     const f32x4* yr = y ? reinterpret_cast<const f32x4*>(y + r * E) : nullptr;
     f32x4 v[NV];
     float s = 0.f;
+    int S = 1;
+    if constexpr (PLANES) S = rows_split_eff(*count, static_cast<int>(rows), sp);
 #pragma unroll
     for (int j = 0; j < NV; ++j) {
         const int i = lane + 64 * j;
         v[j] = f32x4{0.f, 0.f, 0.f, 0.f};
         if (i < n4) {
             v[j] = xr[i];
-            if (yr) v[j] = v[j] + yr[i];
+            if constexpr (PLANES) {
+                f32x4 t = reinterpret_cast<const f32x4*>(bias)[i] + yr[i];
+                for (int z = 1; z < S; ++z) t = t + yr[z * (rows * n4) + i];
+                v[j] = v[j] + t;
+            } else if (yr) v[j] = v[j] + yr[i];
             s += v[j][0] + v[j][1] + v[j][2] + v[j][3];
         }
     }
@@ -316,6 +384,32 @@
     else if (E <= 2048) mmx::add_layernorm_fwd_kernel<8, true><<<grid, 256, 0, s>>>(x, y, g, b, so, ho, mo, ro, cap_rows, E, eps, nullptr, list, count);
     else mmx::add_layernorm_fwd_kernel<16, true><<<grid, 256, 0, s>>>(x, y, g, b, so, ho, mo, ro, cap_rows, E, eps, nullptr, list, count);
     MMX_LAUNCH_CHECK("add_layernorm_fwd_kernel<rows>");
+    return MMX_OK;
+}
+
+extern "C" int mmx_add_layernorm_fwd_rows_planes(const void* x_dev, const void* planes_dev, const void* bias_dev, const void* gamma_dev,
+                                                 const void* beta_dev, void* sum_dev, void* h_dev, void* mean_dev, void* rstd_dev,
+                                                 const void* rows_dev, const void* count_dev, int cap_rows, int E, float eps,
+                                                 const int* plan, void* stream) {
+    MMX_CHECK_ARG(x_dev && planes_dev && bias_dev && gamma_dev && beta_dev && sum_dev && h_dev && mean_dev && rstd_dev && rows_dev &&
+                      count_dev && plan, "mmx_add_layernorm_fwd_rows_planes: null pointer");
+    MMX_CHECK_ARG(cap_rows > 0 && E > 0 && E % 4 == 0 && E <= 4096, "mmx_add_layernorm_fwd_rows_planes: cap_rows=%d E=%d (E %% 4 == 0, E <= 4096)",
+                  cap_rows, E);
+    const mmx::RowsSplit sp = {plan[0], plan[1], plan[2], plan[3], plan[4]};
+    MMX_CHECK_ARG(sp.S >= 1 && sp.S <= 8 && sp.tm > 0 && sp.tiles_n > 0 && sp.dense_wgs >= 1, "mmx_add_layernorm_fwd_rows_planes: bad plan");
+    const unsigned grid = static_cast<unsigned>((cap_rows + 3) / 4);
+    hipStream_t s = static_cast<hipStream_t>(stream);
+    const float *x = static_cast<const float*>(x_dev), *y = static_cast<const float*>(planes_dev), *bias = static_cast<const float*>(bias_dev);
+    const float *g = static_cast<const float*>(gamma_dev), *b = static_cast<const float*>(beta_dev);
+    float *so = static_cast<float*>(sum_dev), *ho = static_cast<float*>(h_dev);
+    float *mo = static_cast<float*>(mean_dev), *ro = static_cast<float*>(rstd_dev);
+    const int *list = static_cast<const int*>(rows_dev), *count = static_cast<const int*>(count_dev);
+    if (E <= 256) mmx::add_layernorm_fwd_kernel<1, true, true><<<grid, 256, 0, s>>>(x, y, g, b, so, ho, mo, ro, cap_rows, E, eps, nullptr, list, count, bias, sp);
+    else if (E <= 512) mmx::add_layernorm_fwd_kernel<2, true, true><<<grid, 256, 0, s>>>(x, y, g, b, so, ho, mo, ro, cap_rows, E, eps, nullptr, list, count, bias, sp);
+    else if (E <= 1024) mmx::add_layernorm_fwd_kernel<4, true, true><<<grid, 256, 0, s>>>(x, y, g, b, so, ho, mo, ro, cap_rows, E, eps, nullptr, list, count, bias, sp);
+    else if (E <= 2048) mmx::add_layernorm_fwd_kernel<8, true, true><<<grid, 256, 0, s>>>(x, y, g, b, so, ho, mo, ro, cap_rows, E, eps, nullptr, list, count, bias, sp);
+    else mmx::add_layernorm_fwd_kernel<16, true, true><<<grid, 256, 0, s>>>(x, y, g, b, so, ho, mo, ro, cap_rows, E, eps, nullptr, list, count, bias, sp);
+    MMX_LAUNCH_CHECK("add_layernorm_fwd_kernel<rows, planes>");
     return MMX_OK;
 }
 
diff --git a/transformer-mm-explainability_amd/csrc/gemm_rows_f32.hip b/transformer-mm-explainability_amd/csrc/gemm_rows_f32.hip
--- a/transformer-mm-explainability_amd/csrc/gemm_rows_f32.hip
+++ b/transformer-mm-explainability_amd/csrc/gemm_rows_f32.hip
@@ -8,11 +8,18 @@
 static int g_gemm_rows_tm = 32;
 static int g_gemm_rows_tn = 0;
 static int g_text_live_rows_fwd = 1;
+static int g_gemm_rows_split = 0;
+static int g_gemm_rows_split_dense = 512;
 bool text_live_rows_option(const char* key, int value) {
     if (strcmp(key, "text_live_rows") == 0 && value >= 0 && value <= 1) { g_text_live_rows = value; return true; }
     if (strcmp(key, "text_live_rows_fwd") == 0 && value >= 0 && value <= 1) { g_text_live_rows_fwd = value; return true; }
     if (strcmp(key, "gemm_rows_tm") == 0 && (value == 32 || value == 64)) { g_gemm_rows_tm = value; return true; }
     if (strcmp(key, "gemm_rows_tn") == 0 && (value == 0 || value == 32 || value == 64)) { g_gemm_rows_tn = value; return true; }
+    if (strcmp(key, "gemm_rows_split") == 0 && (value == 0 || value == 1 || value == 2 || value == 4 || value == 8)) {
+        g_gemm_rows_split = value;
+        return true;
+    }
+    if (strcmp(key, "gemm_rows_split_dense") == 0 && value >= 1 && value <= (1 << 20)) { g_gemm_rows_split_dense = value; return true; }
     return false;
 }
 
@@ -47,7 +54,7 @@
 __global__ __launch_bounds__(256, 2) void gemm_rows_f32_kernel(const float* __restrict__ A, const float* __restrict__ W,
                                                                float* __restrict__ C, const int* __restrict__ rows,
                                                                const int* __restrict__ count, int cap, int N, int K,
-                                                               const float* __restrict__ bias, float* __restrict__ C2) {
+                                                               const float* __restrict__ bias, float* __restrict__ C2, RowsSplit sp) {
     constexpr int WR = TM / 32, WC = TN / 32;
     constexpr int WK = 4 / (WR * WC);
     constexpr int NG = BK / 8 / WK;
@@ -65,9 +72,21 @@
     const int wc = wave % WC, wr = (wave / WC) % WR, wk = wave / (WC * WR);
     const int M = min(*count, cap);
     const int tiles_n = (N + TN - 1) / TN;
-    const int bx = blockIdx.x % tiles_n, by = blockIdx.x / tiles_n;
+    const int plane_wgs = tiles_n * ((cap + TM - 1) / TM);
+    const int z = blockIdx.x / plane_wgs, bz = blockIdx.x - z * plane_wgs;
+    const int bx = bz % tiles_n, by = bz / tiles_n;
     const int m0 = by * TM, n0 = bx * TN;
     if (m0 >= M) return;
+    int kbeg = 0, Kl = K;
+    if (sp.S > 1) {
+        if (rows_split_eff(M, cap, sp) > 1) {
+            kbeg = z * sp.per * BK;
+            Kl = min(K, kbeg + sp.per * BK) - kbeg;
+            C += static_cast<int64_t>(z) * cap * N;
+        } else if (z > 0) {
+            return;
+        }
+    }
 
     auto dense_row = [&](int gm) {
         const int r = gm < M ? rows[gm] : -1;
@@ -86,29 +105,29 @@
     for (int i = 0; i < CA; ++i) {
         const int arow = dense_row(m0 + ar + i * RA);
         oka[i] = arow >= 0;
-        pa[i] = A + static_cast<int64_t>(oka[i] ? arow : 0) * K;
+        pa[i] = A + static_cast<int64_t>(oka[i] ? arow : 0) * K + kbeg;
     }
     const int kb = tid / (TN / 4), nbl = (tid % (TN / 4)) * 4;
     const bool okb = n0 + nbl < N;
-    const float* pb = W + (okb ? n0 + nbl : 0);
+    const float* pb = W + static_cast<int64_t>(kbeg) * N + (okb ? n0 + nbl : 0);
     struct Slab { f32x4 a[CA], b[CB]; };
     Slab ring[PF];
     auto fetch = [&](int t, Slab& x) {
         const int k0 = t * BK;
 #pragma unroll
-        for (int i = 0; i < CA; ++i) x.a[i] = ldg4_u(pa[i] + min(k0 + ka, K - 4));
-#pragma unroll
-        for (int i = 0; i < CB; ++i) x.b[i] = ldg4_u(pb + static_cast<int64_t>(min(k0 + kb + i * RB, K - 1)) * N);
+        for (int i = 0; i < CA; ++i) x.a[i] = ldg4_u(pa[i] + min(k0 + ka, Kl - 4));
+#pragma unroll
+        for (int i = 0; i < CB; ++i) x.b[i] = ldg4_u(pb + static_cast<int64_t>(min(k0 + kb + i * RB, Kl - 1)) * N);
     };
     auto stash = [&](int stage, int t, const Slab& x) {
-        const f32x4 z = {0.f, 0.f, 0.f, 0.f};
+        const f32x4 zero = {0.f, 0.f, 0.f, 0.f};
         const int k0 = t * BK;
 #pragma unroll
         for (int i = 0; i < CA; ++i)
-            *reinterpret_cast<f32x4*>(&As[stage][(ar + i * RA) * LA + ka]) = (oka[i] && k0 + ka < K) ? x.a[i] : z;
+            *reinterpret_cast<f32x4*>(&As[stage][(ar + i * RA) * LA + ka]) = (oka[i] && k0 + ka < Kl) ? x.a[i] : zero;
 #pragma unroll
         for (int i = 0; i < CB; ++i)
-            *reinterpret_cast<f32x4*>(&Bs[stage][(kb + i * RB) * LB + nbl]) = (okb && k0 + kb + i * RB < K) ? x.b[i] : z;
+            *reinterpret_cast<f32x4*>(&Bs[stage][(kb + i * RB) * LB + nbl]) = (okb && k0 + kb + i * RB < Kl) ? x.b[i] : zero;
     };
 
     const int li = lane & 31, lg = lane >> 5;
@@ -131,7 +150,7 @@
             for (int t = 0; t < 4; ++t) acc = __builtin_amdgcn_mfma_f32_32x32x2f32(f.a[g][t], f.b[g][t], acc, 0, 0, 0);
     };
 
-    const int nslab = (K + BK - 1) / BK;
+    const int nslab = (Kl + BK - 1) / BK;
     fetch(0, ring[0]);
     stash(0, 0, ring[0]);
 #pragma unroll
@@ -200,16 +219,25 @@
     return static_cast<int64_t>((N + t.tn - 1) / t.tn) * ((cap_rows + t.tm - 1) / t.tm);
 }
 
+static RowsSplit rows_split(RowsTile t, int N, int K) {
+    const int bk = (t.tm == 32 && t.tn == 32) ? 64 : 32, nslab = (K + bk - 1) / bk;
+    int want = g_gemm_rows_split;
+    if (want == 0) want = 1;
+    const int per = (nslab + want - 1) / want;
+    return {(nslab + per - 1) / per, per, t.tm, (N + t.tn - 1) / t.tn, g_gemm_rows_split_dense};
+}
+
 template <int EPI>
 static void launch_gemm_rows(RowsTile t, int64_t wgs, hipStream_t s, const float* A, const float* W, float* C, const int* rows,
-                             const int* count, int cap_rows, int N, int K, const float* bias, float* C2) {
+                             const int* count, int cap_rows, int N, int K, const float* bias, float* C2,
+                             RowsSplit sp = {1, 0, 0, 0, 0}) {
     const unsigned g = static_cast<unsigned>(wgs);
     if (t.tm == 64)
-        gemm_rows_f32_kernel<64, 64, 32, 3, EPI><<<g, 256, 0, s>>>(A, W, C, rows, count, cap_rows, N, K, bias, C2);
+        gemm_rows_f32_kernel<64, 64, 32, 3, EPI><<<g, 256, 0, s>>>(A, W, C, rows, count, cap_rows, N, K, bias, C2, sp);
     else if (t.tn == 32)
-        gemm_rows_f32_kernel<32, 32, 64, 3, EPI><<<g, 256, 0, s>>>(A, W, C, rows, count, cap_rows, N, K, bias, C2);
+        gemm_rows_f32_kernel<32, 32, 64, 3, EPI><<<g, 256, 0, s>>>(A, W, C, rows, count, cap_rows, N, K, bias, C2, sp);
     else
-        gemm_rows_f32_kernel<32, 64, 32, 3, EPI><<<g, 256, 0, s>>>(A, W, C, rows, count, cap_rows, N, K, bias, C2);
+        gemm_rows_f32_kernel<32, 64, 32, 3, EPI><<<g, 256, 0, s>>>(A, W, C, rows, count, cap_rows, N, K, bias, C2, sp);
 }
 
 }
@@ -245,6 +273,35 @@
                         static_cast<float*>(c_dev), static_cast<const int*>(rows_dev), static_cast<const int*>(count_dev), cap_rows, N, K,
                         nullptr, nullptr);
     MMX_LAUNCH_CHECK("gemm_rows_f32_kernel");
+    return MMX_OK;
+}
+
+extern "C" int mmx_gemm_rows_split_plan(int N, int K, int* plan) {
+    MMX_CHECK_ARG(plan && N > 0 && K > 0, "mmx_gemm_rows_split_plan: N=%d K=%d", N, K);
+    const RowsSplit sp = rows_split(rows_tile(N, K), N, K);
+    plan[0] = sp.S; plan[1] = sp.per; plan[2] = sp.tm; plan[3] = sp.tiles_n; plan[4] = sp.dense_wgs;
+    return MMX_OK;
+}
+
+extern "C" int mmx_gemm_rows_planes_f32(const void* a_dev, const void* w_dev, void* planes_dev, const void* rows_dev,
+                                        const void* count_dev, int cap_rows, int N, int K, const int* plan, void* stream) {
+    MMX_CHECK_ARG(a_dev && w_dev && planes_dev && rows_dev && count_dev && plan, "mmx_gemm_rows_planes_f32: null pointer");
+    MMX_CHECK_ARG(cap_rows > 0 && N > 0 && K > 0, "mmx_gemm_rows_planes_f32: cap_rows=%d N=%d K=%d", cap_rows, N, K);
+    if (N % 4 || K % 4 ||
+        ((reinterpret_cast<uintptr_t>(a_dev) | reinterpret_cast<uintptr_t>(w_dev) | reinterpret_cast<uintptr_t>(planes_dev)) & 15u)) {
+        set_error("mmx_gemm_rows_planes_f32: N=%d and K=%d must be multiples of 4 and the operands 16-byte aligned", N, K);
+        return MMX_ENOTSUP;
+    }
+    const RowsTile tm = rows_tile(N, K);
+    const RowsSplit want = rows_split(tm, N, K), sp = {plan[0], plan[1], plan[2], plan[3], plan[4]};
+    MMX_CHECK_ARG(sp.S == want.S && sp.per == want.per && sp.tm == want.tm && sp.tiles_n == want.tiles_n && sp.dense_wgs >= 1,
+                  "mmx_gemm_rows_planes_f32: the plan is not mmx_gemm_rows_split_plan's for N=%d K=%d under the current options", N, K);
+    const int64_t wgs = rows_grid(tm, cap_rows, N) * sp.S;
+    MMX_CHECK_ARG(wgs < (1ll << 31), "mmx_gemm_rows_planes_f32: cap_rows=%d x N=%d x %d planes is too large a grid", cap_rows, N, sp.S);
+    launch_gemm_rows<0>(tm, wgs, static_cast<hipStream_t>(stream), static_cast<const float*>(a_dev), static_cast<const float*>(w_dev),
+                        static_cast<float*>(planes_dev), static_cast<const int*>(rows_dev), static_cast<const int*>(count_dev), cap_rows, N, K,
+                        nullptr, nullptr, sp);
+    MMX_LAUNCH_CHECK("gemm_rows_f32_kernel<planes>");
     return MMX_OK;
 }
 
diff --git a/transformer-mm-explainability_amd/csrc/mmx_common.h b/transformer-mm-explainability_amd/csrc/mmx_common.h
--- a/transformer-mm-explainability_amd/csrc/mmx_common.h
+++ b/transformer-mm-explainability_amd/csrc/mmx_common.h
@@ -166,6 +166,12 @@
 __device__ __forceinline__ float group16_sum(float x) {
     x += dpp_row<0x128>(x); x += dpp_row<0x124>(x); x += dpp_row<0x122>(x); x += dpp_row<0x121>(x);
     return x;
+}
+
+struct RowsSplit { int S, per, tm, tiles_n, dense_wgs; };
+__host__ __device__ __forceinline__ int rows_split_eff(int count, int cap, RowsSplit sp) {
+    const int m = count < cap ? count : cap;
+    return ((m + sp.tm - 1) / sp.tm) * sp.tiles_n >= sp.dense_wgs ? 1 : sp.S;
 }
 
 __device__ __forceinline__ int xcd_contiguous_id(int w, int total) {
diff --git a/transformer-mm-explainability_amd/ops.py b/transformer-mm-explainability_amd/ops.py
--- a/transformer-mm-explainability_amd/ops.py
+++ b/transformer-mm-explainability_amd/ops.py
@@ -538,6 +538,12 @@
             return torch.full(shape, float("nan"), dtype=torch.float32, device=like.device)
         return torch.empty(shape, dtype=torch.float32, device=like.device)
 
+    def _planes(self, like, width, count):
+        shape = (count,) + tuple(like.shape[:-1]) + (width,)
+        if LiveRows.poison:
+            return torch.full(shape, float("nan"), dtype=torch.float32, device=like.device)
+        return torch.empty(shape, dtype=torch.float32, device=like.device)
+
     def _check(self, what, *tensors):
         for t in tensors:
             if t.dtype != torch.float32 or not t.is_contiguous() or t.numel() // t.shape[-1] != self.cap:
@@ -561,9 +567,49 @@
                and w.data_ptr() % 16 == 0 for w in weights)
 
 
-def gemm_rows(x, weight, live, out=None):
+class RowPlanes:
+
+    def __init__(self, planes, plan, bias):
+        self.planes, self.plan, self.bias = planes, plan, bias
+
+    @property
+    def S(self):
+        return int(self.plan[0])
+
+
+def _rows_plan(M, K):
+    plan = (C.c_int * 5)()
+    check(lib().mmx_gemm_rows_split_plan(M, K, plan), "mmx_gemm_rows_split_plan")
+    return plan
+
+
+def gemm_rows_split(M, K):
+    return int(_rows_plan(M, K)[0])
+
+
+def _gemm_rows_planes(what, x, w_kn, bias, live, planes):
+    K, M = w_kn.shape
+    live._check(what, x)
+    if x.shape[-1] != K:
+        raise MMXError("%s: x %s against K = %d" % (what, tuple(x.shape), K))
+    plan = _rows_plan(M, K)
+    shape = (plan[0],) + tuple(x.shape[:-1]) + (M,)
+    if planes is None:
+        planes = live._planes(x, M, plan[0])
+    elif tuple(planes.shape) != shape or planes.dtype != torch.float32 or not planes.is_contiguous():
+        raise MMXError("%s: the planes of this product are fp32 contiguous %s, got %s" % (what, shape, tuple(planes.shape)))
+    check(lib().mmx_gemm_rows_planes_f32(_p(x), _p(w_kn), _p(planes), _p(live.rows), _p(live.count), live.cap, M, K, plan, _stream()),
+          "mmx_gemm_rows_planes_f32")
+    return RowPlanes(planes, plan, bias)
+
+
+def gemm_rows(x, weight, live, out=None, planes=False):
     _dev(x, weight, out)
     K, M = weight.shape
+    if planes:
+        if not gemm_rows_eligible(weight):
+            raise MMXError("gemm_rows: x %s @ weight %s" % (tuple(x.shape), tuple(weight.shape)))
+        return _gemm_rows_planes("gemm_rows", x, weight, None, live, out)
     if out is None:
         out = live._out(x, M)
     live._check("gemm_rows", x, out)
@@ -578,9 +624,13 @@
     return bool(lib().mmx_text_live_rows_fwd_enabled())
 
 
-def linear_rows(x, weight, bias, live, out=None, gelu=False, act_out=None):
+def linear_rows(x, weight, bias, live, out=None, gelu=False, act_out=None, planes=False):
     _dev(x, weight, bias, out, act_out)
     M, K = weight.shape
+    if planes:
+        if gelu or not gemm_rows_eligible(weight) or bias is None or bias.numel() != M:
+            raise MMXError("linear_rows: planes need an eligible weight with a bias and no QuickGELU")
+        return _gemm_rows_planes("linear_rows", x, transposed_weight(weight), _f32c(bias.detach()), live, out)
     if out is None:
         out = live._out(x, M)
     live._check("linear_rows", x, out)
@@ -597,6 +647,12 @@
 
 
 def add_layernorm_rows(x, y, gamma, beta, eps, live, out=None):
+    yp = y if isinstance(y, RowPlanes) else None
+    if yp is not None:
+        y = yp.planes[0]
+        if yp.bias is None or yp.bias.numel() != x.shape[-1] or y.shape != x.shape:
+            raise MMXError("add_layernorm_rows: planes %s with a bias expected for x %s" % (tuple(yp.planes.shape), tuple(x.shape)))
+        _dev(yp.planes, yp.bias)
     _dev(x, y, gamma, beta)
     live._check("add_layernorm_rows", x, *([y] if y is not None else []))
     E = x.shape[-1]
@@ -612,6 +668,11 @@
         s = live._out(x, E) if y is not None else x
         h = live._out(x, E)
         mean, rstd = live._out(x, 1).view(-1), live._out(x, 1).view(-1)
+    if yp is not None:
+        check(lib().mmx_add_layernorm_fwd_rows_planes(_p(x), _p(yp.planes), _p(yp.bias), _p(_f32c(gamma)), _p(_f32c(beta)), _p(s), _p(h),
+                                                      _p(mean), _p(rstd), _p(live.rows), _p(live.count), live.cap, E, float(eps), yp.plan,
+                                                      _stream()), "mmx_add_layernorm_fwd_rows_planes")
+        return s, h, mean, rstd
     check(lib().mmx_add_layernorm_fwd_rows(_p(x), _p(y), _p(_f32c(gamma)), _p(_f32c(beta)), _p(s) if y is not None else _p(None), _p(h),
                                            _p(mean), _p(rstd), _p(live.rows), _p(live.count), live.cap, E, float(eps), _stream()),
           "mmx_add_layernorm_fwd_rows")
@@ -628,12 +689,23 @@
 
 
 def layernorm_bwd_add_rows(dy, x, mean, rstd, gamma, d_res, live):
+    dyp = dy if isinstance(dy, RowPlanes) else None
+    if dyp is not None:
+        dy = dyp.planes[0]
+        if dyp.bias is not None or dy.shape != x.shape:
+            raise MMXError("layernorm_bwd_add_rows: planes %s without a bias expected for x %s" % (tuple(dyp.planes.shape), tuple(x.shape)))
+        _dev(dyp.planes)
     _dev(dy, x, mean, rstd, gamma, d_res)
     live._check("layernorm_bwd_add_rows", dy, x, *([d_res] if d_res is not None else []))
     mean, rstd = _f32c(mean), _f32c(rstd)
     if mean.numel() != live.cap or rstd.numel() != live.cap:
         raise MMXError("layernorm_bwd_add_rows: %d statistics for %d rows" % (mean.numel(), live.cap))
     dx = live._out(dy, dy.shape[-1])
+    if dyp is not None:
+        check(lib().mmx_layernorm_bwd_add_rows_planes(_p(dyp.planes), _p(x), _p(mean), _p(rstd), _p(_f32c(gamma)), _p(d_res), _p(dx),
+                                                      _p(live.rows), _p(live.count), live.cap, dy.shape[-1], dyp.plan, _stream()),
+              "mmx_layernorm_bwd_add_rows_planes")
+        return dx
     check(lib().mmx_layernorm_bwd_add_rows(_p(dy), _p(x), _p(mean), _p(rstd), _p(_f32c(gamma)), _p(d_res), _p(dx), _p(live.rows),
                                            _p(live.count), live.cap, dy.shape[-1], _stream()), "mmx_layernorm_bwd_add_rows")
     return dx
```

Result: slower. 8045 (-1.0%).
